# utiasSTARS/pyslam

Hardware: AMD Instinct MI355X
Metric: ms/LM-iter (Jac build + J^T J + Schur solve), stereo BA @ 500k residuals (lower is better)
Workload: dtype f64

## Files before the change

### include/pyslam_hip.h

```cpp
#ifndef PYSLAM_HIP_H
#define PYSLAM_HIP_H

#include <stdint.h>

#ifdef __cplusplus
extern "C" {
#endif

typedef struct ps_problem ps_problem;

typedef struct ps_problem_desc {
    int32_t dof;
    int32_t num_poses;
    const double*  poses;
    const int32_t* pose_rid;
    int32_t num_points;
    const double*  points;
    const int32_t* point_vid;

    int64_t num_obs;
    const int32_t* obs_pose;
    const int32_t* obs_point;
    const double*  obs_uvd;
    const int32_t* obs_grp;
// ... 81 lines not shown
int ps_step_norm2(ps_problem* h, double* norm2);

int ps_apply_update(ps_problem* h, double step);

int ps_snapshot_params(ps_problem* h);
int ps_restore_params(ps_problem* h);

int ps_get_params(ps_problem* h, double* poses, double* points);
int ps_set_params(ps_problem* h, const double* poses, const double* points);

int ps_gn_iteration(ps_problem* h, double lambda, double pcg_tol, int pcg_max_iters,
                    int linesearch, double* cost_out, double* dx_norm_out,
                    int* pcg_iters_out, double* pcg_relres_out);

typedef struct ps_solve_options {
    int32_t max_iters, allow_nondecreasing_steps, max_nondecreasing_steps, linesearch;
    double min_update_norm, min_cost, min_cost_decrease, lm_lambda;
} ps_solve_options;
int ps_motion_only_solve(ps_problem* h, const ps_solve_options* options, double* cost_history, int32_t cap,
                         int32_t* n_history, int32_t* iterations, double* last_dx_norm, double* pose12_out);

int ps_reset_solver_state(ps_problem* h);

const char* ps_build_sha(void);

int ps_solve(ps_problem* h, const ps_solve_options* options, double pcg_tol, int pcg_max_iters, double* cost_history,
             int32_t cap, int32_t* n_history, int32_t* iterations, double* last_dx_norm, int32_t* pcg_iters,
             double* pcg_relres, double* iter_ms);

int ps_lm_iteration(ps_problem* h, double lambda, double pcg_tol, int pcg_max_iters, int linesearch, double* cost_out,
                    double* dx_norm_out, double* model_decrease_out, int* pcg_iters_out, double* pcg_relres_out);

typedef struct ps_lm_options {
    int32_t max_iters, allow_nondecreasing_steps, max_nondecreasing_steps, linesearch;
    double min_update_norm, min_cost, min_cost_decrease, lm_lambda;
    double lambda0, lambda_min, lambda_max;
} ps_lm_options;
int ps_solve_lm(ps_problem* h, const ps_lm_options* options, double pcg_tol, int pcg_max_iters, double* cost_history,
                int32_t cap, int32_t* n_history, int32_t* iterations, double* last_dx_norm, int32_t* pcg_iters,
                double* pcg_relres, double* iter_ms, double* lm_rows);

int ps_gn_finish(ps_problem* h, int linesearch, double* cost_out, double* dx_pose_norm2,
                 double* dx_point_norm2);

int ps_gn_solve_finish(ps_problem* h, double pcg_tol, int pcg_max_iters, int linesearch, double* cost_out,
                       double* dx_pose_norm2, double* dx_point_norm2, int* pcg_iters_out,
                       double* pcg_relres_out);

int ps_shard_buffer(ps_problem* h, void** dev_ptr);

int ps_set_collective(ps_problem* h, void* nccl_all_reduce_fn, void* nccl_comm);
int ps_set_segment_exchange(ps_problem* h, void* nccl_all_gather_fn, int32_t world, int32_t rank, int64_t maxlen,
                            int64_t n_mine, const int64_t* mine, int64_t n_dst, const int64_t* dst, const int64_t* src_ptr,
                            const int64_t* src_off);
int ps_gn_solve_finish_enqueue(ps_problem* h, double pcg_tol, int pcg_max_iters, int linesearch, int first);
int ps_gn_result(ps_problem* h, int* done, double* shard2, double* dx_pose_norm2,
                 int* pcg_iters_out, double* pcg_relres_out);

int ps_covariance_begin(ps_problem* h);
int ps_covariance_column(ps_problem* h, int kind, int index, int comp, double tol, int max_iters,
                         int* iters_out, double* relres_out);

#define PS_COV_DENSE_MAX_UNKNOWNS 12288
int ps_covariance_marginals(ps_problem* h, double* pose_blocks ,
                            double* point_blocks );
int ps_covariance_pose_blocks(ps_problem* h, int64_t n, const int32_t* a, const int32_t* b,
                              double* out );
int ps_covariance_cross_blocks(ps_problem* h, int64_t n, const int32_t* kind_a, const int32_t* a,
                               const int32_t* kind_b, const int32_t* b, double* out );

int ps_triangulate(ps_problem* h, int64_t n, const int32_t* vids , int refine_iters, double min_parallax_deg,
                   int write_back, double* points_out , int32_t* status_out );

int ps_get_reduced_system(ps_problem* h, int32_t* row_ptr, int32_t* col_idx,
                          double* vals, double* g);
int ps_get_landmark_factors(ps_problem* h, double* cinv , double* c );
int ps_debug_reproj_blocks(ps_problem* h, double* r , double* jpose ,
                           double* jpoint );
int ps_debug_factor_blocks(ps_problem* h, double* r, double* j1, double* j2);
int ps_debug_table_checksums(ps_problem* h, uint64_t* out, int capacity, int* count);
int ps_debug_packed_runs(ps_problem* h, int32_t* nwaves, int32_t capacity_waves, int32_t* run, int32_t* first, int32_t* lm_ptr,
                         double* sq_part);
int ps_debug_pose_items(ps_problem* h, int32_t* nitems, int32_t capacity_items, int32_t* items, double* partial);

int ps_set_option(ps_problem* h, const char* name, double value);
int ps_get_option(ps_problem* h, const char* name, double* value);

int ps_set_profiling(ps_problem* h, int enabled);
int ps_get_stage_times(ps_problem* h, double* ms , int64_t* counts, int reset);

int ps_dense_normal_solve(const double* J, const double* r, int32_t m, int32_t n,
                          double* dx, double* covariance );

int ps_sparse_normal_solve(int32_t m, int32_t n, const int32_t* j_row_ptr, const int32_t* j_col, const double* j_val,
                           const int32_t* jt_row_ptr, const int32_t* jt_col, const double* jt_val,
                           const double* r, const double* rhs, double tol, int32_t max_iters,
                           double* dx, int32_t* iters_out, double* relres_out);

int ps_sparse_normal_direct(int32_t m, int32_t n, const int32_t* j_row_ptr, const int32_t* j_col, const double* j_val,
                            const int32_t* jt_row_ptr, const int32_t* jt_col, const double* jt_val,
                            const double* r, const double* rhs, int32_t refine_steps, double* dx, double* relres_out);

int ps_debug_band_inverse(const double* a, int32_t ncb, int32_t dof, int32_t bw, int32_t chunk_nodes, float* ainv_out,
                          double* elapsed_us);
int ps_debug_coarse_chol(const double* a, int32_t ncb, int32_t dof, int32_t bw, int32_t variant, double* Li, double* LiT,
                         int32_t* status, double* elapsed_us);
int ps_debug_coarse_chol_clocks(const double* a, int32_t ncb, int32_t dof, int32_t bw, int32_t variant, double* clocks);
int ps_debug_dense_factor(const double* a, int32_t n, int32_t flags, double* l_out, double* tinv_out, double* li_out, double* lit_out,
                          float* ainv_out, int32_t* diag_fail, double* elapsed_us);
int ps_debug_bchol_slab(int32_t m, int32_t w, int32_t block, int32_t* row_lo, int32_t* row_hi, int32_t* entries, int32_t* grid);
enum { PS_LDI_READ_STATE = 0, PS_LDI_READ_S32 = 1, PS_LDI_READ_X32 = 2, PS_LDI_READ_XU = 3, PS_LDI_READ_XT = 4, PS_LDI_READ_LINV = 5,
       PS_LDI_READ_COEF = 6, PS_LDI_READ_FRO = 7, PS_LDI_READ_R = 8, PS_LDI_READ_Z = 9 };
int ps_debug_ldi_gemm(int32_t M, int32_t N, int32_t K, float alpha, const float* A, int32_t lda, const float* B, int32_t ldb, float beta,
                      const float* Dm, int32_t ldd, float gamma, float* C, int32_t ldc, const int32_t* krange, int32_t upper_only,
                      const float* dev_scale, double fro_sentinel, double* fro_part);
int ps_debug_ldi_ritz(const double* rz, const double* alpha, int32_t m, float* out3);
int ps_debug_ldi_read(ps_problem* h, int32_t what, double* out, int64_t capacity);
int ps_debug_factor_stress(const double* a, int32_t ncb, int32_t dof, int32_t bw, int32_t mode, int32_t launches, int32_t lowprio,
                           int32_t aggressor, int32_t* n_diff, int32_t* n_pivot);

int ps_ransac_transforms(const double* pts_1, const double* pts_2, int32_t batch, int32_t n, double* T_out);
int ps_ransac_cost(const double* T, int32_t num_hyp, const double* pts_1, const double* obs_2, int32_t num_pts,
                   const double* cam5, double thresh, uint8_t* masks, int32_t* counts);
int ps_ransac_frame_to_frame(const double* pts_1, const double* pts_2, const double* obs_2, int32_t num_pts,
                             const int32_t* sample_idx, int32_t num_hyp, int32_t set_size, const double* cam5,
                             double thresh, double* T_all, int32_t* counts, int32_t* best_index,
                             int32_t* best_count, double* T_best, uint8_t* best_mask);

int ps_twoview_hypotheses(const double* obs_1, const double* obs_2, int32_t num_pts, const int32_t* sample_idx, int32_t num_hyp,
                          const double* cam5, double thresh, double* E_all, int32_t* counts, uint8_t* degenerate);
int ps_twoview_score(const double* E, int32_t num_hyp, const double* obs_1, const double* obs_2, int32_t num_pts,
                     const double* cam5, double thresh, uint8_t* masks, int32_t* counts);
int ps_twoview_ransac(const double* obs_1, const double* obs_2, int32_t num_pts, const int32_t* sample_idx, int32_t num_hyp,
                      const double* cam5, double thresh, int32_t refit, double* T_21, double* E_out, uint8_t* mask,
                      int32_t* info, double* parallax_deg);

int ps_pnp_hypotheses(const double* pts_w, const double* obs, int32_t num_pts, const int32_t* sample_idx, int32_t num_hyp,
                      const double* cam5, double thresh, double* T_all, int32_t* counts, uint8_t* empty);
int ps_pnp_score(const double* T, int32_t num_T, const double* pts_w, const double* obs, int32_t num_pts, const double* cam5,
                 double thresh, uint8_t* masks, int32_t* counts);
int ps_pnp_ransac(const double* pts_w, const double* obs, int32_t num_pts, const int32_t* sample_idx, int32_t num_hyp,
                  const double* cam5, double thresh, int32_t refine_iters, double* T_cw, uint8_t* mask, int32_t* info,
                  double* sq_err, double* cost_history);

int ps_sim3_hypotheses(const double* pts_1, const double* pts_2, const double* obs_1, const double* obs_2, int32_t num_pts,
                       const int32_t* sample_idx, int32_t num_hyp, const double* cam5, double thresh, int32_t fixed_scale,
                       double* S_all, double* scales, int32_t* counts, uint8_t* flags);
int ps_sim3_score(const double* S, int32_t num_S, const double* pts_1, const double* pts_2, const double* obs_1, const double* obs_2,
                  int32_t num_pts, const double* cam5, double thresh, uint8_t* masks, int32_t* counts);
int ps_sim3_ransac(const double* pts_1, const double* pts_2, const double* obs_1, const double* obs_2, int32_t num_pts,
                   const int32_t* sample_idx, int32_t num_hyp, const double* cam5, double thresh, int32_t fixed_scale,
                   int32_t refit_iters, double* S_21, double* scale, uint8_t* mask, int32_t* info, double* sq_err);

typedef struct ps_sim3pg ps_sim3pg;
int ps_sim3pg_create(int32_t num_vertices, const double* vertices13, const uint8_t* held, int32_t num_edges, const int32_t* edge_i,
                     const int32_t* edge_j, const double* edge_obs13, const double* edge_stiffness49, int32_t loss_id, double loss_k,
                     void* stream, ps_sim3pg** out);
int ps_sim3pg_destroy(ps_sim3pg* h);
int ps_sim3pg_set_vertices(ps_sim3pg* h, const double* vertices13);
int ps_sim3pg_get_vertices(ps_sim3pg* h, double* vertices13);
int ps_sim3pg_eval_cost(ps_sim3pg* h, double* cost);
int ps_sim3pg_linearize(ps_sim3pg* h, double lambda, double* H_out, double* g_out, double* cost);
int ps_sim3pg_iteration(ps_sim3pg* h, double lambda, double* cost_after, double* dx_norm, double* relres);
int ps_sim3pg_solve(ps_sim3pg* h, const ps_solve_options* options, double* cost_history, int32_t cap, int32_t* n_history,
                    int32_t* iterations, double* last_dx_norm);
int ps_sim3pg_debug_edges(ps_sim3pg* h, double* tap105);
// ... 81 lines not shown
```

### pyslam_amd/_native.py

```python
import ctypes as C
import os

import numpy as np

_HERE = os.path.dirname(os.path.abspath(__file__))
LIB_PATH = os.path.join(_HERE, 'lib', 'libpyslam_hip.so')
if os.environ.get('PYSLAM_AMD_MEASURE') == '1':
    LIB_PATH = os.path.join(_HERE, 'lib', 'libpyslam_hip_measure.so')

c_i32p = C.POINTER(C.c_int32)
c_f64p = C.POINTER(C.c_double)
c_u8p = C.POINTER(C.c_uint8)
PS_NUM_STAGES = 12
STAGE_NAMES = ['landmark_pass', 'pose_pass', 'schur_pairs', 'pose_factors', 'pcg',
               'backsub', 'update', 'cost', 'iteration_total', 'cg_kernel', 'allreduce', 'pack_unpack']


class ProblemDesc(C.Structure):
    _fields_ = [
        ('dof', C.c_int32), ('num_poses', C.c_int32), ('poses', c_f64p), ('pose_rid', c_i32p),
        ('num_points', C.c_int32), ('points', c_f64p), ('point_vid', c_i32p),
        ('num_obs', C.c_int64), ('obs_pose', c_i32p), ('obs_point', c_i32p), ('obs_uvd', c_f64p),
        ('obs_grp', c_i32p),
        ('num_cams', C.c_int32), ('cams', c_f64p), ('num_stiff3', C.c_int32), ('stiff3', c_f64p),
# ... 30 lines not shown
        ('num_obs', C.c_int64), ('num_edges', C.c_int64), ('num_priors', C.c_int64),
        ('reduced_nnzb', C.c_int64), ('num_pairs', C.c_int64), ('reduce_count', C.c_int64),
        ('device_bytes', C.c_int64), ('cg_restarts', C.c_int64), ('cg_kernel_launches', C.c_int64),
        ('ldi_solves', C.c_int64), ('ldi_fallbacks', C.c_int64), ('ldi_seeds', C.c_int64),
        ('xcg_fused_solves', C.c_int64), ('xcg_fused_fallbacks', C.c_int64),
        ('cg_persist_solves', C.c_int64), ('cg_persist_failures', C.c_int64), ('cg_persist_refused', C.c_int64),
        ('persist_cus', C.c_int32), ('persist_cus_needed', C.c_int32), ('landmark_passes_taken_over', C.c_int64),
    ]


class PhotoDesc(C.Structure):
    _fields_ = [
        ('num_pixels', C.c_int32), ('pt_ref', c_f64p), ('im_ref', c_f64p), ('im_jac', c_f64p), ('tri_jac_d', c_f64p),
        ('height', C.c_int32), ('width', C.c_int32), ('im_track', c_f64p),
        ('cam', C.c_double * 5), ('cam_type', C.c_int32), ('cam_w', C.c_int32), ('cam_h', C.c_int32),
        ('intensity_covar', C.c_double), ('depth_covar', C.c_double), ('loss_id', C.c_int32), ('loss_k', C.c_double),
    ]


class FeatParams(C.Structure):
    _fields_ = [('response_threshold', C.c_int64), ('nms_n', C.c_int32), ('max_features', C.c_int32),
                ('match_radius_u', C.c_int32), ('match_radius_v', C.c_int32), ('disp_max', C.c_int32),
                ('match_cost_max', C.c_int32), ('refinement', C.c_int32), ('reserved', C.c_int32)]


H = C.c_void_p
SIGNATURES = {
    'ps_last_error': (C.c_char_p, []),
    'ps_device_count': (C.c_int, []),
    'ps_warm_up': (C.c_int, []),
    'ps_problem_create': (C.c_int, [C.POINTER(ProblemDesc), C.c_void_p, C.POINTER(H)]),
    'ps_problem_create_hybrid': (C.c_int, [C.POINTER(ProblemDesc), C.POINTER(HostRowsDesc), C.c_void_p, C.POINTER(H)]),
    'ps_set_host_rows': (C.c_int, [H, c_f64p, C.c_int64, C.c_double]),
    'ps_problem_destroy': (C.c_int, [H]),
    'ps_get_info': (C.c_int, [H, C.POINTER(ProblemInfo)]),
    'ps_eval_cost': (C.c_int, [H, C.c_int, c_f64p]),
    'ps_linearize': (C.c_int, [H, C.c_double]),
    'ps_reduce_buffer': (C.c_int, [H, C.POINTER(C.c_void_p), C.POINTER(C.c_int64)]),
    'ps_shard_pack': (C.c_int, [H]),
    'ps_shard_unpack': (C.c_int, [H]),
    'ps_solve_reduced': (C.c_int, [H, C.c_double, C.c_int, C.POINTER(C.c_int), c_f64p]),
    'ps_backsub': (C.c_int, [H]),
    'ps_get_dx': (C.c_int, [H, c_f64p, c_f64p]),
    'ps_step_norm2': (C.c_int, [H, c_f64p]),
    'ps_apply_update': (C.c_int, [H, C.c_double]),
    'ps_snapshot_params': (C.c_int, [H]),
    'ps_restore_params': (C.c_int, [H]),
    'ps_reset_solver_state': (C.c_int, [H]),
    'ps_build_sha': (C.c_char_p, []),
    'ps_get_params': (C.c_int, [H, c_f64p, c_f64p]),
    'ps_set_params': (C.c_int, [H, c_f64p, c_f64p]),
    'ps_motion_only_solve': (C.c_int, [H, C.POINTER(SolveOptions), c_f64p, C.c_int32, C.POINTER(C.c_int32), C.POINTER(C.c_int32),
                                       C.POINTER(C.c_double), c_f64p]),
    'ps_solve': (C.c_int, [H, C.POINTER(SolveOptions), C.c_double, C.c_int, c_f64p, C.c_int32, C.POINTER(C.c_int32),
                           C.POINTER(C.c_int32), C.POINTER(C.c_double), c_i32p, c_f64p, c_f64p]),
    'ps_gn_iteration': (C.c_int, [H, C.c_double, C.c_double, C.c_int, C.c_int, c_f64p, c_f64p,
                                  C.POINTER(C.c_int), c_f64p]),
    'ps_lm_iteration': (C.c_int, [H, C.c_double, C.c_double, C.c_int, C.c_int, c_f64p, c_f64p, c_f64p,
                                  C.POINTER(C.c_int), c_f64p]),
    'ps_solve_lm': (C.c_int, [H, C.POINTER(LmOptions), C.c_double, C.c_int, c_f64p, C.c_int32, C.POINTER(C.c_int32),
                              C.POINTER(C.c_int32), C.POINTER(C.c_double), c_i32p, c_f64p, c_f64p, c_f64p]),
    'ps_gn_finish': (C.c_int, [H, C.c_int, c_f64p, c_f64p, c_f64p]),
    'ps_gn_solve_finish': (C.c_int, [H, C.c_double, C.c_int, C.c_int, c_f64p, c_f64p, c_f64p,
                                     C.POINTER(C.c_int), c_f64p]),
    'ps_set_collective': (C.c_int, [H, C.c_void_p, C.c_void_p]),
    'ps_set_segment_exchange': (C.c_int, [H, C.c_void_p, C.c_int32, C.c_int32, C.c_int64, C.c_int64, C.POINTER(C.c_int64), C.c_int64,
                                         C.POINTER(C.c_int64), C.POINTER(C.c_int64), C.POINTER(C.c_int64)]),
    'ps_shard_buffer': (C.c_int, [H, C.POINTER(C.c_void_p)]),
    'ps_gn_solve_finish_enqueue': (C.c_int, [H, C.c_double, C.c_int, C.c_int, C.c_int]),
    'ps_gn_result': (C.c_int, [H, C.POINTER(C.c_int), c_f64p, c_f64p, C.POINTER(C.c_int), c_f64p]),
    'ps_covariance_begin': (C.c_int, [H]),
    'ps_covariance_column': (C.c_int, [H, C.c_int, C.c_int, C.c_int, C.c_double, C.c_int, C.POINTER(C.c_int), c_f64p]),
    'ps_covariance_marginals': (C.c_int, [H, c_f64p, c_f64p]),
    'ps_covariance_pose_blocks': (C.c_int, [H, C.c_int64, c_i32p, c_i32p, c_f64p]),
    'ps_covariance_cross_blocks': (C.c_int, [H, C.c_int64, c_i32p, c_i32p, c_i32p, c_i32p, c_f64p]),
    'ps_triangulate': (C.c_int, [H, C.c_int64, c_i32p, C.c_int, C.c_double, C.c_int, c_f64p, c_i32p]),
    'ps_get_reduced_system': (C.c_int, [H, c_i32p, c_i32p, c_f64p, c_f64p]),
    'ps_get_landmark_factors': (C.c_int, [H, c_f64p, c_f64p]),
    'ps_debug_reproj_blocks': (C.c_int, [H, c_f64p, c_f64p, c_f64p]),
    'ps_debug_factor_blocks': (C.c_int, [H, c_f64p, c_f64p, c_f64p]),
    'ps_debug_table_checksums': (C.c_int, [H, C.POINTER(C.c_uint64), C.c_int, C.POINTER(C.c_int)]),
    'ps_debug_packed_runs': (C.c_int, [H, c_i32p, C.c_int32, c_i32p, c_i32p, c_i32p, c_f64p]),
    'ps_debug_pose_items': (C.c_int, [H, c_i32p, C.c_int32, c_i32p, c_f64p]),
    'ps_set_option': (C.c_int, [H, C.c_char_p, C.c_double]),
    'ps_get_option': (C.c_int, [H, C.c_char_p, c_f64p]),
    'ps_set_profiling': (C.c_int, [H, C.c_int]),
    'ps_get_stage_times': (C.c_int, [H, c_f64p, C.POINTER(C.c_int64), C.c_int]),
    'ps_ransac_transforms': (C.c_int, [c_f64p, c_f64p, C.c_int32, C.c_int32, c_f64p]),
    'ps_ransac_cost': (C.c_int, [c_f64p, C.c_int32, c_f64p, c_f64p, C.c_int32, c_f64p, C.c_double, c_u8p, c_i32p]),
    'ps_ransac_frame_to_frame': (C.c_int, [c_f64p, c_f64p, c_f64p, C.c_int32, c_i32p, C.c_int32, C.c_int32, c_f64p,
                                           C.c_double, c_f64p, c_i32p, c_i32p, c_i32p, c_f64p, c_u8p]),
    'ps_twoview_hypotheses': (C.c_int, [c_f64p, c_f64p, C.c_int32, c_i32p, C.c_int32, c_f64p, C.c_double, c_f64p, c_i32p, c_u8p]),
    'ps_twoview_score': (C.c_int, [c_f64p, C.c_int32, c_f64p, c_f64p, C.c_int32, c_f64p, C.c_double, c_u8p, c_i32p]),
    'ps_twoview_ransac': (C.c_int, [c_f64p, c_f64p, C.c_int32, c_i32p, C.c_int32, c_f64p, C.c_double, C.c_int32, c_f64p, c_f64p,
                                    c_u8p, c_i32p, c_f64p]),
    'ps_pnp_hypotheses': (C.c_int, [c_f64p, c_f64p, C.c_int32, c_i32p, C.c_int32, c_f64p, C.c_double, c_f64p, c_i32p, c_u8p]),
    'ps_pnp_score': (C.c_int, [c_f64p, C.c_int32, c_f64p, c_f64p, C.c_int32, c_f64p, C.c_double, c_u8p, c_i32p]),
    'ps_pnp_ransac': (C.c_int, [c_f64p, c_f64p, C.c_int32, c_i32p, C.c_int32, c_f64p, C.c_double, C.c_int32, c_f64p, c_u8p, c_i32p,
                                c_f64p, c_f64p]),
    'ps_sim3_hypotheses': (C.c_int, [c_f64p, c_f64p, c_f64p, c_f64p, C.c_int32, c_i32p, C.c_int32, c_f64p, C.c_double, C.c_int32,
                                     c_f64p, c_f64p, c_i32p, c_u8p]),
    'ps_sim3_score': (C.c_int, [c_f64p, C.c_int32, c_f64p, c_f64p, c_f64p, c_f64p, C.c_int32, c_f64p, C.c_double, c_u8p, c_i32p]),
    'ps_sim3_ransac': (C.c_int, [c_f64p, c_f64p, c_f64p, c_f64p, C.c_int32, c_i32p, C.c_int32, c_f64p, C.c_double, C.c_int32, C.c_int32,
                                 c_f64p, c_f64p, c_u8p, c_i32p, c_f64p]),
    'ps_sim3pg_create': (C.c_int, [C.c_int32, c_f64p, c_u8p, C.c_int32, c_i32p, c_i32p, c_f64p, c_f64p, C.c_int32, C.c_double, C.c_void_p,
                                   C.POINTER(H)]),
    'ps_sim3pg_destroy': (C.c_int, [H]),
    'ps_sim3pg_set_vertices': (C.c_int, [H, c_f64p]),
    'ps_sim3pg_get_vertices': (C.c_int, [H, c_f64p]),
    'ps_sim3pg_eval_cost': (C.c_int, [H, c_f64p]),
    'ps_sim3pg_linearize': (C.c_int, [H, C.c_double, c_f64p, c_f64p, c_f64p]),
    'ps_sim3pg_iteration': (C.c_int, [H, C.c_double, c_f64p, c_f64p, c_f64p]),
    'ps_sim3pg_solve': (C.c_int, [H, C.POINTER(SolveOptions), c_f64p, C.c_int32, C.POINTER(C.c_int32), C.POINTER(C.c_int32),
                                  C.POINTER(C.c_double)]),
    'ps_sim3pg_debug_edges': (C.c_int, [H, c_f64p]),
    'ps_sim3pg_debug_explog': (C.c_int, [C.c_int32, c_f64p, c_f64p, c_f64p, c_f64p]),
    'ps_sim3pg_profile': (C.c_int, [H, C.c_int32, c_f64p]),
    'ps_photometric_create': (C.c_int, [C.POINTER(PhotoDesc), C.c_void_p, C.POINTER(H)]),
    'ps_photometric_destroy': (C.c_int, [H]),
    'ps_photometric_set_pose': (C.c_int, [H, c_f64p]),
    'ps_photometric_get_pose': (C.c_int, [H, c_f64p]),
    'ps_photometric_eval_cost': (C.c_int, [H, c_f64p, C.POINTER(C.c_int64)]),
    'ps_photometric_normal_equations': (C.c_int, [H, c_f64p, c_f64p, c_f64p, C.POINTER(C.c_int64)]),
    'ps_photometric_iteration': (C.c_int, [H, C.c_int32, C.c_int32, c_f64p, c_f64p]),
    'ps_dense_create': (C.c_int, [C.c_int32, C.c_int32, C.c_int32, C.c_int32, C.c_void_p, C.POINTER(H)]),
    'ps_dense_destroy': (C.c_int, [H]),
    'ps_dense_upload': (C.c_int, [H, C.c_int32, C.c_int32, C.c_int32, C.c_int32, C.c_void_p, c_f64p]),
    'ps_dense_make_tables': (C.c_int, [H, C.c_int32, C.c_int32, c_i32p, c_f64p, C.c_double, C.c_double, C.c_double]),
    'ps_dense_track': (C.c_int, [H, C.c_int32, C.c_int32, C.c_int32, c_i32p, c_i32p, C.POINTER(SolveOptions), C.c_int32,
                                 C.c_double, c_f64p, c_f64p, c_i32p, c_f64p, C.c_int32]),
    'ps_dense_level_shape': (C.c_int, [H, C.c_int32, c_i32p, c_i32p]),
    'ps_dense_read_level': (C.c_int, [H, C.c_int32, C.c_int32, C.c_int32, c_f64p]),
    'ps_dense_num_pixels': (C.c_int, [H, C.c_int32, C.c_int32, c_i32p]),
    'ps_dense_read_tables': (C.c_int, [H, C.c_int32, C.c_int32, C.c_int32, c_f64p, c_f64p, c_f64p, c_f64p]),
    'ps_dense_device_bytes': (C.c_int, [H, C.POINTER(C.c_int64)]),
    'ps_feat_create': (C.c_int, [C.c_int32, C.c_int32, C.c_int32, C.c_void_p, C.POINTER(H)]),
    'ps_feat_destroy': (C.c_int, [H]),
    'ps_feat_push': (C.c_int, [H, C.c_int32, C.c_int32, c_u8p, c_u8p]),
    'ps_feat_match': (C.c_int, [H, C.c_int32, C.POINTER(FeatParams), c_i32p]),
    'ps_feat_read_matches': (C.c_int, [H, C.c_int32, c_f64p, c_i32p]),
    'ps_feat_read_features': (C.c_int, [H, C.c_int32, C.c_int32, c_i32p, c_i32p, C.POINTER(C.c_int64), c_u8p]),
    'ps_feat_set_map': (C.c_int, [H, C.c_int32, c_f64p, c_u8p]),
    'ps_feat_match_map': (C.c_int, [H, c_f64p, c_f64p, C.c_int32, C.POINTER(FeatParams), c_i32p]),
    'ps_feat_read_map_matches': (C.c_int, [H, C.c_int32, c_i32p, c_i32p, c_i32p, c_f64p]),
    'ps_feat_match_map_global': (C.c_int, [H, C.c_int32, C.c_int32, C.POINTER(FeatParams), c_i32p]),
    'ps_feat_read_map_second': (C.c_int, [H, C.c_int32, c_i32p]),
    'ps_feat_db_add': (C.c_int, [H, C.c_int32, c_u8p, c_i32p]),
    'ps_feat_db_clear': (C.c_int, [H]),
    'ps_feat_db_size': (C.c_int, [H, c_i32p, C.POINTER(C.c_int64)]),
    'ps_feat_db_query': (C.c_int, [H, C.c_int32, C.c_int32, C.c_int32, C.c_int32, C.POINTER(FeatParams), c_i32p]),
    'ps_feat_feature_passes': (C.c_int, [H, C.POINTER(C.c_int64)]),
    'ps_feat_device_bytes': (C.c_int, [H, C.POINTER(C.c_int64)]),
    'ps_dense_normal_solve': (C.c_int, [c_f64p, c_f64p, C.c_int32, C.c_int32, c_f64p, c_f64p]),
    'ps_sparse_normal_solve': (C.c_int, [C.c_int32, C.c_int32, c_i32p, c_i32p, c_f64p, c_i32p, c_i32p, c_f64p, c_f64p, c_f64p,
                                         C.c_double, C.c_int32, c_f64p, c_i32p, c_f64p]),
    'ps_sparse_normal_direct': (C.c_int, [C.c_int32, C.c_int32, c_i32p, c_i32p, c_f64p, c_i32p, c_i32p, c_f64p, c_f64p, c_f64p,
                                          C.c_int32, c_f64p, c_f64p]),
    'ps_debug_band_inverse': (C.c_int, [c_f64p, C.c_int32, C.c_int32, C.c_int32, C.c_int32, C.POINTER(C.c_float), c_f64p]),
    'ps_debug_coarse_chol': (C.c_int, [c_f64p, C.c_int32, C.c_int32, C.c_int32, C.c_int32, c_f64p, c_f64p, c_i32p, c_f64p]),
    'ps_debug_coarse_chol_clocks': (C.c_int, [c_f64p, C.c_int32, C.c_int32, C.c_int32, C.c_int32, c_f64p]),
    'ps_debug_dense_factor': (C.c_int, [c_f64p, C.c_int32, C.c_int32, c_f64p, c_f64p, c_f64p, c_f64p, C.POINTER(C.c_float), c_i32p, c_f64p]),
    'ps_debug_bchol_slab': (C.c_int, [C.c_int32, C.c_int32, C.c_int32, c_i32p, c_i32p, c_i32p, c_i32p]),
    'ps_debug_ldi_gemm': (C.c_int, [C.c_int32, C.c_int32, C.c_int32, C.c_float, C.POINTER(C.c_float), C.c_int32, C.POINTER(C.c_float), C.c_int32,
                                    C.c_float, C.POINTER(C.c_float), C.c_int32, C.c_float, C.POINTER(C.c_float), C.c_int32, c_i32p, C.c_int32,
                                    C.POINTER(C.c_float), C.c_double, c_f64p]),
    'ps_debug_ldi_ritz': (C.c_int, [c_f64p, c_f64p, C.c_int32, C.POINTER(C.c_float)]),
# ... 100 lines not shown
```

### pyslam_amd/csrc/ps_abi_solver.h

```cpp

int ps_get_info(ps_problem* h, ps_problem_info* info) {
    if (!h || !info) return fail("null argument");
    info->dof = h->D; info->num_poses = h->P; info->num_reduced = h->nr; info->num_points = h->L;
    info->num_var_points = h->nv; info->num_obs = h->N; info->num_edges = h->F; info->num_priors = 0;
    info->reduced_nnzb = h->nnzb; info->num_pairs = h->npairs;
    info->reduce_count = ((long)h->nnzb + h->nr) / 2 * h->D * h->D + (long)h->nr * h->D + 3;
    info->device_bytes = (int64_t)h->dev_bytes;
    info->cg_restarts = h->cg_fallbacks;
    info->cg_kernel_launches = h->cg_kernel_launches;
    info->ldi_solves = h->ldi_solves; info->ldi_fallbacks = h->ldi_fallbacks; info->ldi_seeds = h->ldi_seeds;
    info->xcg_fused_solves = h->xf_solves; info->xcg_fused_fallbacks = h->xf_fallbacks;
    info->cg_persist_solves = h->cp_launches; info->cg_persist_failures = h->cp_failures;
    info->cg_persist_refused = h->cp_refused; info->persist_cus = h->persist_cus;
    info->persist_cus_needed = h->cp_ok ? h->cp_cus_needed : (h->xp_ok ? h->xp_cus_needed : 0);
    info->landmark_passes_taken_over = h->prelm_used;
    return 0;
}

int ps_eval_cost(ps_problem* h, int include_all_constant, double* cost) {
    if (!h || !cost) return fail("null argument");
    if (include_all_constant && h->fuse_cost == 1 && lm_cost_possible(h)) { if (lm_cost_pass(h, h->lin_lambda, SC_COST)) return -1; }
    else if (cost_pass(h, include_all_constant, SC_COST)) return -1;
    if (read_scalars(h)) return -1;
    *cost = h->h_scalars[SC_COST];
// ... 751 lines not shown
    hipMemcpyAsync(jpoint, djl, (size_t)h->N * 9 * sizeof(double), hipMemcpyDeviceToHost, h->stream);
    const int rc = sync(h);
    hipFree(dr); hipFree(djp); hipFree(djl);
    return rc;
}

int ps_debug_factor_blocks(ps_problem* h, double* r, double* j1, double* j2) {
    if (!h || !r || !j1 || !j2) return fail("null argument");
    if (h->F == 0) return 0;
    const int D = h->D, DD = D * D, ROW = D + 2 * DD;
    double* dbg;
    HIP_OK(hipMalloc((void**)&dbg, (size_t)h->F * ROW * sizeof(double)));
    const int rc0 = D == 6 ? launch_factor_pass<6>(h, 0.0, dbg) : launch_factor_pass<3>(h, 0.0, dbg);
    std::vector<double> t((size_t)h->F * ROW);
    hipMemcpyAsync(t.data(), dbg, t.size() * sizeof(double), hipMemcpyDeviceToHost, h->stream);
    const int rc = sync(h);
    hipFree(dbg);
    if (rc0 || rc) return -1;
    for (long f = 0; f < h->F; ++f) {
        std::memcpy(r + f * D, &t[(size_t)f * ROW], D * sizeof(double));
        std::memcpy(j1 + f * DD, &t[(size_t)f * ROW + D], DD * sizeof(double));
        std::memcpy(j2 + f * DD, &t[(size_t)f * ROW + D + DD], DD * sizeof(double));
    }
    return 0;
}

int ps_debug_table_checksums(ps_problem* h, uint64_t* out, int capacity, int* count) {
    if (!h || !out || !count) return fail("null argument");
    if (sync(h)) return -1;
    struct Tab { const void* p; size_t bytes; };
    const bool tiled = h->schur_tiles > 1 && h->npair_items > 0;
    const Tab tabs[16] = {
        {h->point_vid, (size_t)h->L * 4}, {h->lobs, (size_t)h->N * sizeof(LObs)}, {h->lorig, (size_t)h->N * 4},
        {h->lm_ptr, ((size_t)h->nv + 1) * 4}, {h->lm_point, (size_t)h->nv * 4}, {h->pose_of_rid, (size_t)std::max(h->nr, 1) * 4},
        {h->pitems, (size_t)h->npitems * sizeof(PItem)}, {h->pitem_ptr, ((size_t)h->nr + 1) * 4}, {h->pobs, (size_t)h->Np * sizeof(LObs)},
        {h->pairs, (size_t)h->npairs * 8}, {h->pair_xitems, (size_t)8 * h->pair_per_xcd * sizeof(PairItem)},
        {tiled ? h->comb_items : nullptr, (size_t)h->ncomb * sizeof(PairItem)}, {tiled ? h->comb_tasks : nullptr, (size_t)h->npair_items * 4},
        {h->row_ptr, ((size_t)h->nr + 1) * 4}, {h->col_idx, (size_t)h->nnzb * 4}, {h->diag_slot, (size_t)h->nr * 4}};
    *count = 16;
    std::vector<unsigned char> buf;
    for (int t = 0; t < 16 && t < capacity; ++t) {
        uint64_t hsh = 0;
        if (tabs[t].p && tabs[t].bytes) {
            buf.resize(tabs[t].bytes);
            HIP_OK(hipMemcpy(buf.data(), tabs[t].p, tabs[t].bytes, hipMemcpyDeviceToHost));
            hsh = 1469598103934665603ull;
            size_t i = 0;
            for (; i + 8 <= buf.size(); i += 8) { uint64_t w; std::memcpy(&w, &buf[i], 8); hsh = (hsh ^ w) * 1099511628211ull; }
            for (; i < buf.size(); ++i) hsh = (hsh ^ buf[i]) * 1099511628211ull;
        }
        out[t] = hsh;
    }
    return 0;
}

int ps_debug_packed_runs(ps_problem* h, int32_t* nwaves, int32_t capacity_waves, int32_t* run, int32_t* first, int32_t* lm_ptr, double* sq_part) {
    if (!h || !nwaves) return fail("null argument");
    if (sync(h)) return -1;
    const int nw = h->lmw_nwaves;
    *nwaves = nw;
    if ((run || first || sq_part) && capacity_waves < nw) return fail("ps_debug_packed_runs: capacity too small");
    if (sq_part && nw) HIP_OK(hipMemcpy(sq_part, h->sq_part_l, (size_t)cdiv(nw, 4) * 8, hipMemcpyDeviceToHost));
    if (run && nw) HIP_OK(hipMemcpy(run, h->lmw_run, (size_t)nw * sizeof(LmwRun), hipMemcpyDeviceToHost));
    if (first && nw) HIP_OK(hipMemcpy(first, h->lmw_first, ((size_t)nw + 1) * 4, hipMemcpyDeviceToHost));
    if (lm_ptr && h->nv > 0) HIP_OK(hipMemcpy(lm_ptr, h->lm_ptr, ((size_t)h->nv + 1) * 4, hipMemcpyDeviceToHost));
    return 0;
}

int ps_debug_pose_items(ps_problem* h, int32_t* nitems, int32_t capacity_items, int32_t* items, double* partial) {
    if (!h || !nitems) return fail("null argument");
    if (sync(h)) return -1;
    const int ni = h->npitems;
    *nitems = ni;
    if ((items || partial) && capacity_items < ni) return fail("ps_debug_pose_items: capacity too small");
    if (items && ni) {
        std::vector<PItem> tab(ni);
        HIP_OK(hipMemcpy(tab.data(), h->pitems, (size_t)ni * sizeof(PItem), hipMemcpyDeviceToHost));
        for (int k = 0; k < ni; ++k) { items[3 * k] = tab[k].rid; items[3 * k + 1] = tab[k].start; items[3 * k + 2] = tab[k].end; }
    }
    if (partial && ni) HIP_OK(hipMemcpy(partial, h->ppartial, (size_t)ni * PS_NPOSE_ACC * sizeof(double), hipMemcpyDeviceToHost));
    return 0;
}

int ps_debug_ldi_read(ps_problem* h, int32_t what, double* out, int64_t capacity) {
    if (!h || !out) return fail("null argument");
    if (what == PS_LDI_READ_STATE) {
        if (capacity < 12) return fail("ps_debug_ldi_read: state record needs 12 doubles");
        const double rec[12] = {(double)h->ldi_state, (double)h->ldi_cur, (double)h->ldi_n, (double)h->ldi_np, (double)h->ldi_kp,
                                h->ldi_direct ? 1.0 : 0.0, h->ldi_fro_limit, (double)h->ldi_last_its, (double)h->ldi_seed_steps,
                                (double)h->nr, (double)h->D, h->ldi_ready ? 1.0 : 0.0};
        std::memcpy(out, rec, sizeof(rec));
        return 0;
    }
    if (!h->ldi_ready || h->ldi_seeds < 1) return fail("ps_debug_ldi_read: the lagged inverse has never been set up on this handle");
    HIP_OK(hipStreamSynchronize(h->stream));
    if (h->side) HIP_OK(hipStreamSynchronize(h->side));
    if (h->ldi_stream) HIP_OK(hipStreamSynchronize(h->ldi_stream));
    if (h->ev_ldi) HIP_OK(hipEventSynchronize(h->ev_ldi));
    const size_t n = (size_t)h->ldi_n, np = (size_t)h->ldi_np, kp = (size_t)h->ldi_kp;
    const void* src = nullptr; size_t count = 0; bool f32 = true;
    const bool seed_item = what == PS_LDI_READ_S32 || what == PS_LDI_READ_X32 || what == PS_LDI_READ_XT || what == PS_LDI_READ_LINV ||
                           what == PS_LDI_READ_COEF;
    if (seed_item && h->ldi_direct) return fail("ps_debug_ldi_read: the direct seed keeps no Newton-Schulz operands");
    const bool use_item = what == PS_LDI_READ_XU || what == PS_LDI_READ_R || what == PS_LDI_READ_Z;
    if (use_item && h->ldi_cur < 0) return fail("ps_debug_ldi_read: no inverse is in use");
    switch (what) {
        case PS_LDI_READ_S32: src = h->ldi_S32; count = np * np; break;
        case PS_LDI_READ_X32: src = h->ldi_X32; count = np * np; break;
        case PS_LDI_READ_XU: src = h->ldi_Xu[h->ldi_cur]; count = np * np; break;
        case PS_LDI_READ_XT: src = h->ldi_Xt; count = np * kp; break;
        case PS_LDI_READ_LINV: src = h->ldi_Linv; count = (size_t)h->nr * h->D * h->D; f32 = false; break;
        case PS_LDI_READ_COEF: src = h->ldi_coef; count = 3; break;
        case PS_LDI_READ_FRO: if (capacity < 1) return fail("ps_debug_ldi_read: capacity"); out[0] = *h->h_ldi_fro; return 0;
        case PS_LDI_READ_R: src = h->ldi_r[h->ldi_last_its & 1]; count = n; f32 = false; break;
        case PS_LDI_READ_Z: src = h->z; count = n; f32 = false; break;
        default: return fail("ps_debug_ldi_read: unknown item");
    }
    if ((size_t)capacity < count) return fail("ps_debug_ldi_read: capacity too small");
    if (!f32) { HIP_OK(hipMemcpy(out, src, count * 8, hipMemcpyDeviceToHost)); return 0; }
    std::vector<float> tmp(count);
    HIP_OK(hipMemcpy(tmp.data(), src, count * 4, hipMemcpyDeviceToHost));
    for (size_t i = 0; i < count; ++i) out[i] = (double)tmp[i];
    return 0;
}

static void relook_path(ps_problem* h) {
    const bool possible = ps_ldi_possible(*h, (long)h->nr * h->D);
    if (h->coarse_built && possible != h->xmin_auto_ldi && h->cg_explicit_min_rows < 0) h->coarse_built = false;
}

int ps_set_option(ps_problem* h, const char* name, double value) {
    if (!h || !name) return fail("null argument");
    if (!std::strcmp(name, "expect_next")) { h->expect_next = value != 0 && !h->hybrid; return 0; }
    if (!std::strcmp(name, "solve_horizon")) { h->solve_horizon = value < 0 ? -1 : (int)std::min(value, 1e6); return 0; }
    if (!std::strcmp(name, "setup_ride")) {
        h->setup_ride = value != 0 ? 1 : 0;
        h->prelin_valid = h->prelm_valid = false;
        relook_launch_gates(h);
        return 0;
    }
    if (!std::strcmp(name, "rows_regs")) {
        h->rows_regs = value != 0 ? 1 : 0;
        h->prelin_valid = h->prelm_valid = h->ride_valid = false;
        return 0;
    }
    if (!std::strcmp(name, "cg_persist_recover")) {
        h->cg_persist_recover = value != 0 ? 1 : 0;
        h->prelin_valid = h->prelm_valid = h->ride_valid = false;
        return 0;
    }
    if (!std::strcmp(name, "cg_persist_recover_lds")) {
        if (!(value >= 0 && value <= PS_CP_RECOVER_LDS_CAP)) return fail("cg_persist_recover_lds out of range (0 .. 146432 bytes)");
        h->cg_persist_recover_lds = (int)value;
        h->prelin_valid = h->prelm_valid = h->ride_valid = false;
        return 0;
    }
    if (!std::strcmp(name, "packed_prefetch")) {
        h->packed_prefetch = value != 0 ? 1 : 0;
        h->prelin_valid = h->prelm_valid = h->ride_valid = false;
        return 0;
    }
    if (!std::strcmp(name, "pose_prefetch")) {
        h->pose_prefetch = value != 0 ? 1 : 0;
        h->prelin_valid = h->prelm_valid = h->ride_valid = false;
        return 0;
    }
    if (!std::strcmp(name, "coarse_chol_band")) { h->coarse_chol_band = value != 0 ? 1 : 0; return 0; }
    if (std::strcmp(name, "cg_force_breakdown")) h->prelin_valid = h->prelm_valid = h->ride_valid = false;
    const char* refusal = nullptr;
    const int fx = ps_option_apply(*h, name, value, &refusal);
    if (fx == PS_OPT_UNKNOWN) return fail(std::string("unknown option: ") + name);
    if (fx == PS_OPT_REFUSED) return fail(refusal);
    if (fx & PS_FX_COARSE_REBUILD) h->coarse_built = false;
    if (fx & PS_FX_DROP_FACTOR) h->lci_next = -1;
    if (fx & PS_FX_DROP_SIDE) h->side_todo = false;
    if ((fx & PS_FX_LDI_OFF) && !h->ldi_enable) { h->ldi_cur = -1; if (h->ldi_state != 1) h->ldi_state = 0; }
    if (fx & PS_FX_RELOOK_PATH) relook_path(h);
    relook_launch_gates(h);
    return 0;
}

int ps_get_option(ps_problem* h, const char* name, double* value) {
    if (!h || !name || !value) return fail("null argument");
    const std::string n(name);
    if (n == "lin_zero_list") *value = h->lin_zero_gate ? 1.0 : 0.0;
    else if (n == "lin_fills") *value = (double)h->lin_fills;
    else if (n == "lin_zero_launches") *value = (double)h->lin_zero_launches;
    else if (n == "setup_ride") *value = h->ride_gate ? 1.0 : 0.0;
    else if (n == "factor_launches") *value = (double)h->bjf_launches;
    else if (n == "factors_ridden") *value = (double)h->bjf_ridden;
    else if (n == "factor_plan_mismatches") *value = (double)h->bjf_mismatches;
    else if (n == "rows_regs") *value = (double)h->rows_regs;
    else if (n == "rows_setups") *value = (double)h->rows_setups;
    else if (n == "exact_row_setups") *value = (double)h->exact_row_setups;
    else if (n == "rows_lci_in_lds") *value = h->coarse_built && h->lagx_ok && h->rows_lci_lds ? 1.0 : 0.0;
    else if (n == "packed_prefetch") *value = (double)h->packed_prefetch;
    else if (n == "pose_prefetch") *value = (double)h->pose_prefetch;
    else if (n == "cg_persist_recover") *value = (double)h->cg_persist_recover;
    else if (n == "cg_persist_recover_lds") *value = (double)h->cg_persist_recover_lds;
    else if (n == "cg_persist_recover_need") *value = h->coarse_built && h->cp_ok ? (double)h->cp_rec_lds : 0.0;
    else if (n == "cg_persist_recovered") *value = (double)h->cp_rec_inside;
    else if (n == "cg_persist_recover_fallbacks") *value = (double)h->cp_rec_behind;
    else if (n == "coarse_chol_band") *value = (double)h->coarse_chol_band;
    else if (n == "coarse_nodes") *value = h->coarse_built ? (double)h->ncb : 0.0;
    else if (n == "coarse_chol_bw") *value = h->coarse_built && h->ncb > 0 ? (double)std::min(std::max(h->coarse_chol_bw, 0), h->ncb - 1) : -1.0;
    else if (n == "cg_force_breakdown") *value = (double)h->cg_force_breakdown;
    else return fail("ps_get_option: no read-back for option: " + n);
    return 0;
}

int ps_reset_solver_state(ps_problem* h) {
    if (!h) return fail("null argument");
    h->prelin_valid = h->prelm_valid = h->ride_valid = false;
    if (!h->solver_touched) {
        static_cast<PsCostHistory&>(*h) = PsCostHistory{};
        return 0;
    }
    h->solver_touched = false;
    HIP_OK(hipStreamSynchronize(h->stream));
    if (h->side) HIP_OK(hipStreamSynchronize(h->side));
    if (h->ldi_stream) HIP_OK(hipStreamSynchronize(h->ldi_stream));
    drain_timers(h);
    static_cast<PsCarried&>(*h) = PsCarried{};
    static_cast<PsCostHistory&>(*h) = PsCostHistory{};
    if (h->lag_status) HIP_OK(hipMemsetAsync(h->lag_status, 0, ST_NWORDS * sizeof(int32_t), h->stream));
    if (h->ldi_ready && !(h->ldi_direct_ok && h->N == 0 && h->F > 0)) h->ldi_direct = false;
    h->cov_ready = false;
    return 0;
}

#ifndef PS_BUILD_SHA
#define PS_BUILD_SHA "unknown"
#endif
const char* ps_build_sha(void) { return PS_BUILD_SHA; }

int ps_set_profiling(ps_problem* h, int enabled) {
    if (!h) return fail("null argument");
    h->profiling = enabled < 0 ? 0 : (enabled > 2 ? 2 : enabled);
    return 0;
}

int ps_get_stage_times(ps_problem* h, double* ms, int64_t* counts, int reset) {
    if (!h) return fail("null argument");
    if (!h->pending.empty() && sync(h)) return -1;
    for (int i = 0; i < PS_NUM_STAGES; ++i) {
        if (ms) ms[i] = h->stage_ms[i];
        if (counts) counts[i] = h->stage_n[i];
        if (reset) { h->stage_ms[i] = 0.0; h->stage_n[i] = 0; }
    }
    return 0;
}

int ps_dense_normal_solve(const double* J, const double* r, int32_t m, int32_t n, double* dx, double* covariance) {
    if (!J || !r || !dx || m <= 0 || n <= 0) return fail("bad argument");
    if (n > 2048) return fail("generic (host-evaluated) path supports at most 2048 unknowns");
    if (need_device()) return -1;
    const int nrhs = covariance ? n + 1 : 1;
    DevBuf bJ, br, bH, bB, bst, bg;
    if (bJ.put(J, (size_t)m * n) || br.put(r, (size_t)m) || bH.get((size_t)n * n * sizeof(double)) ||
        bst.get(ST_NWORDS * sizeof(int32_t)) || bg.get((size_t)n * sizeof(double))) return -1;
    HIP_OK(hipMemset(bst.p, 0, ST_NWORDS * sizeof(int32_t)));
    hipLaunchKernelGGL(k_dense_normal, dim3(cdiv((long)n * n, 256)), dim3(256), 0, 0, m, n, bJ.as<double>(), br.as<double>(), bH.as<double>(),
                       bg.as<double>());
    std::vector<double> B((size_t)n * nrhs, 0.0), gh(n);
    if (bg.fetch(gh.data(), gh.size())) return -1;
    for (int i = 0; i < n; ++i) { B[(size_t)i * nrhs] = gh[i]; if (covariance) B[(size_t)i * nrhs + 1 + i] = 1.0; }
    if (bB.put(B.data(), B.size())) return -1;
    hipLaunchKernelGGL(k_dense_chol_solve, dim3(1), dim3(256), 0, 0, n, nrhs, bH.as<double>(), bB.as<double>(), bst.as<int32_t>());
    int32_t st[ST_NWORDS];
    if (bB.fetch(B.data(), B.size()) || bst.fetch(st, (size_t)ST_NWORDS)) return -1;
    if (st[ST_DIAG_FAIL]) return fail("normal matrix is not positive definite");
    for (int i = 0; i < n; ++i) {
        dx[i] = B[(size_t)i * nrhs];
        if (covariance) for (int j = 0; j < n; ++j) covariance[(size_t)i * n + j] = B[(size_t)i * nrhs + 1 + j];
    }
    return 0;
}
```

### pyslam_amd/csrc/ps_core.hip

```cpp
#include <hip/hip_runtime.h>

#include <algorithm>
#include <array>
#include <map>
#include <atomic>
#include <chrono>
#include <thread>
#include <climits>
#include <cmath>
#include <cstdio>
#include <cstring>
#include <memory>
#include <mutex>
#include <string>
#include <vector>

#include "pyslam_hip.h"
#include "ps_kernels.h"
#include "ps_ransac_core.h"
#include "ps_ransac.h"
#include "ps_k_twoview.h"
#include "ps_k_pnp.h"
#include "ps_k_sim3.h"
#include "ps_k_sim3pg.h"
// ... 287 lines not shown
    int cg_persist_recover = 1;
    int cg_persist_recover_lds = PS_CP_RECOVER_LDS_CAP;
    int cp_rec_pp = 0, cp_rec_cols = 0;
    size_t cp_rec_lds = 0;
    long cp_rec_inside = 0, cp_rec_behind = 0;
    int persist_dev = 0, persist_cus = 0;
    bool persist_masked = false;
    int cp_cus_needed = 0, xp_cus_needed = 0;
    int persist_held = 0;
    bool params_moved_since_lin = false;
    bool z_foreign = false;
    bool no_repeat = false;
    long cp_refused = 0;
    void persist_release() { if (persist_held) { ps_persist_ledger().release(persist_dev, persist_held); persist_held = 0; } }
    int persist_capacity() const { return persist_masked ? persist_cus / 2 : persist_cus; }
    bool persist_reserve(int need) {
        if (need <= 0 || persist_cus <= 0) return false;
        if (persist_held) return true;
        if (!ps_persist_ledger().reserve(persist_dev, need, persist_capacity())) { ++cp_refused; return false; }
        persist_held = need; return true;
    }
    bool xp_ok = false;
    int32_t* xf_cnt = nullptr;
    unsigned long long* xp_exch = nullptr;
    size_t xp_words = 0;
    unsigned xp_salt = 0;
    bool xp_defer = false;
    long long* cp_dbg = nullptr;
    long long* xp_dbg = nullptr;
    long prof_tick = 0;
    int cg_fallbacks = 0;
    bool cg_two_level_reduce = false, cg_short_rows = false;
    double* cg_tot = nullptr;
    bool cg_split = false;
    bool xmin_auto_ldi = false;
    double *cg_U = nullptr, *cg_cgd[2] = {}, *cg_ab = nullptr;
    int cg_launched = 0;
    long cg_kernel_launches = 0;
    bool cov_ready = false;
    std::vector<int32_t> h_slot_of_vid;
    double* cov_buf = nullptr;
    double* cov_xbuf = nullptr;
    long long cov_epoch = 0, cov_sigma_epoch = -1;
    double* tri_buf = nullptr;
    size_t tri_cap = 0;
    int ell_wf = 0, ell_wc = 0;
    double *cost_partials = nullptr, *scalars = nullptr, *h_scalars = nullptr;
    int32_t *status = nullptr, *h_status = nullptr;
    double* h_scalars_dev = nullptr;
    int32_t* h_status_dev = nullptr;
    double *h_shard = nullptr, *h_shard_dev = nullptr;
    long long *h_seq = nullptr, *h_seq_dev = nullptr;
    long long seq = 0;
    long long *h_setup = nullptr, *h_setup_dev = nullptr;
    long long setup_seq = 0;
    int32_t* arrivals = nullptr;
    double *h_mo_hist = nullptr, *h_mo_hist_dev = nullptr;
    int ncost_obs = 0, ncost_fac = 0;
    typedef int (*allreduce_fn)(const void*, void*, size_t, int, int, void*, hipStream_t);
    allreduce_fn nccl_allreduce = nullptr;
    void* nccl_comm = nullptr;
    typedef int (*allgather_fn)(const void*, void*, size_t, int, void*, hipStream_t);
    allgather_fn seg_allgather = nullptr;
    int seg_world = 0;
    long seg_maxlen = 0, seg_nmine = 0, seg_ndst = 0;
    int32_t *seg_mine = nullptr, *seg_dst = nullptr, *seg_src_off = nullptr, *seg_src_ptr = nullptr;
    double *seg_in = nullptr, *seg_all = nullptr;
    double* shard_pack = nullptr;
    int32_t *up_slot = nullptr, *upT_slot = nullptr;
    long nup = 0, pack_count = 0;
    double* shard_buf = nullptr;
    bool shard_out = false;
    double *sq_part_l = nullptr, *sq_part_p = nullptr;
    bool lm_md = false;
    double *md_part_p = nullptr, *md_part_l = nullptr;
    int nmd_p = 0;
    int nsq_l = 0 , nsq_l16 = 0 , nsq_p = 0;
    int32_t* lmw_first = nullptr;
    int lmw_nwaves = 0;
    LmwRun* lmw_run = nullptr;
    int packed_prefetch = 1;
    int pose_prefetch = 1;
    int pose_chunk = 256;
    int coarse_chol_band = 1;
    int coarse_chol_bw = 0;
    bool ldi_ready = false;
    int ldi_n = 0, ldi_np = 0, ldi_kp = 0;
    float *ldi_S32 = nullptr, *ldi_X32 = nullptr, *ldi_R32 = nullptr, *ldi_T32 = nullptr, *ldi_Xt = nullptr, *ldi_XtT = nullptr;
    float* ldi_Xu[2] = {};
    double *ldi_x64 = nullptr, *ldi_Linv = nullptr, *ldi_r[2] = {}, *ldi_part = nullptr, *ldi_fro_part = nullptr;
    double *h_ldi_fro = nullptr, *h_ldi_fro_dev = nullptr;
    double ldi_fro_limit = 0.1;
    int2* ldi_krange = nullptr;
    bool side_poolable = false;
    hipStream_t ldi_stream = nullptr;
    double *ldi_A64 = nullptr, *ldi_Li = nullptr, *ldi_LiT = nullptr, *ldi_Tinv = nullptr; int32_t* ldi_stat = nullptr;
    float* ldi_coef = nullptr;
    long ldi_solves = 0, ldi_fallbacks = 0, ldi_seeds = 0;
    hipEvent_t ev_ldi = nullptr, ev_ldi_sread = nullptr;
    bool snap_valid = false;
    long long *h_early = nullptr, *h_early_dev = nullptr;
    long long early_seq = 0;
    bool spec_next = false, spec_enqueued = false, early_armed = false, prelin_valid = false;
    double prelin_lambda = 0.0;
    bool prelm_pending = false, prelm_valid = false;
    double prelm_lambda = 0.0;
    long long prelm_tag = 0, prelm_seq = 0, lmfail_check = 0, lin_lmfail_tag = 0;
    long long *h_lmfail = nullptr, *h_lmfail_dev = nullptr;
    long prelm_used = 0;
    bool start_cost_pending = false;
    bool solver_touched = false;
    int profiling = 0;
    std::vector<std::pair<int, int>> pending;
    double stage_ms[PS_NUM_STAGES] = {};
    int64_t stage_n[PS_NUM_STAGES] = {};
    std::vector<hipEvent_t> ev_pool;
    size_t ev_used = 0;

    char *arena_dev = nullptr, *arena_host = nullptr;
    void* words_host = nullptr;
    size_t arena_used = 0;
    bool arena_open = false, arena_poisoned = false;

    template <typename T>
    int alloc(T** out, size_t n, bool device_written = false ) {
        *out = nullptr;
        const size_t bytes = std::max<size_t>(n, 1) * sizeof(T);
        if (arena_open && bytes <= PS_ARENA_SMALL && !device_written) {
            const size_t off = (arena_used + 255) & ~(size_t)255;
            if (off + bytes <= PS_ARENA_BYTES) {
                std::memset(arena_host + off, 0, bytes);
                arena_used = off + bytes;
                dev_bytes += bytes;
                *out = (T*)(arena_dev + off);
                return 0;
            }
        }
        void* p = nullptr;
        static const bool guard_on = ps_env("PS_ALLOC_GUARD") != nullptr;
        const size_t padded = (bytes + 255) & ~(size_t)255;
        if (slab_left >= padded) {
            *out = (T*)slab; slab += padded; slab_left -= padded; dev_bytes += bytes;
            return 0;
        }
        hipError_t e = hipMalloc(&p, guard_on ? padded + 4096 : bytes);
        if (e != hipSuccess) return fail(std::string("hipMalloc: ") + hipGetErrorString(e));
        if (guard_on) {
            if (hipMemset((char*)p + bytes, 0xA5, padded - bytes + 4096) != hipSuccess) return fail("hipMemset (guard) failed");
            guards.push_back({(char*)p + padded, bytes, (int)guards.size()});
            fprintf(stderr, "GUARD %p table #%d = %zu bytes (%s)\n", (void*)this, (int)guards.size() - 1, bytes, __PRETTY_FUNCTION__);
        }
        static const bool poison_all = ps_env("PS_ARENA_POISON") != nullptr;
        if (poison_all && hipMemset(p, 0xFF, bytes) != hipSuccess) return fail("hipMemset (poison) failed");
        allocs.push_back(p);
        dev_bytes += bytes;
        *out = (T*)p;
        return 0;
    }
    char* slab = nullptr; size_t slab_left = 0;
    int slab_reserve(size_t bytes) {
        if (ps_env("PS_ALLOC_GUARD")) return 0;
        void* p = nullptr;
        hipError_t e = hipMalloc(&p, bytes);
        if (e != hipSuccess) return fail(std::string("hipMalloc: ") + hipGetErrorString(e));
        if (ps_env("PS_ARENA_POISON") && hipMemset(p, 0xFF, bytes) != hipSuccess) return fail("hipMemset (poison) failed");
        allocs.push_back(p);
// ... 101 lines not shown
```

### pyslam_amd/csrc/ps_host_cg.h

```cpp

namespace {

struct StageTimer {
    ps_problem* h;
    int stage;
    hipEvent_t a = nullptr, b = nullptr;
    int slot = -1;
    StageTimer(ps_problem* h_, int st, int level = 2) : h(h_), stage(st) {
        if (h->profiling < level) return;
        if (h->profiling == 1 && h->prof_every > 1 &&
            h->prof_tick % h->prof_every != (st == PS_ST_CG_KERNEL ? h->prof_every / 2 : 0)) return;
        if (h->ev_used + 2 > h->ev_pool.size()) {
            for (int i = 0; i < 64; ++i) { hipEvent_t e; hipEventCreate(&e); h->ev_pool.push_back(e); }
        }
        slot = (int)h->ev_used;
        a = h->ev_pool[h->ev_used++];
        b = h->ev_pool[h->ev_used++];
        hipEventRecord(a, h->stream);
    }
    void stop() {
        if (!a) return;
        hipEventRecord(b, h->stream);
        h->pending.push_back({stage, slot});
        a = nullptr;
    }
    ~StageTimer() { stop(); }
};

void drain_timers(ps_problem* h) {
    for (auto& pr : h->pending) {
        float ms = 0.f;
        if (hipEventElapsedTime(&ms, h->ev_pool[pr.second], h->ev_pool[pr.second + 1]) == hipSuccess) {
            h->stage_ms[pr.first] += ms;
            h->stage_n[pr.first] += 1;
        }
    }
    h->pending.clear();
    h->ev_used = 0;
}

int side_kick(ps_problem* h);
int ldi_side_kick(ps_problem* h);
int linearize(ps_problem* h, double lambda, bool allow_prelm = false);
bool use_direct(const ps_problem* h);

void drain_timers_ready(ps_problem* h) {
    std::vector<std::pair<int, int>> keep;
    for (auto& pr : h->pending) {
        float ms = 0.f;
        if (hipEventQuery(h->ev_pool[pr.second + 1]) != hipSuccess) { keep.push_back(pr); continue; }
        if (hipEventElapsedTime(&ms, h->ev_pool[pr.second], h->ev_pool[pr.second + 1]) == hipSuccess) {
            h->stage_ms[pr.first] += ms;
            h->stage_n[pr.first] += 1;
        }
    }
    h->pending.swap(keep);
    if (h->pending.empty()) h->ev_used = 0;
}

int sync(ps_problem* h) {
    HIP_OK(hipStreamSynchronize(h->stream));
    h->persist_release();
    drain_timers(h);
    if (h->side_todo) h->side_ready = true;
    return 0;
}

int wait_published(ps_problem* h) {
    volatile long long* w = h->h_seq;
    struct WaitClock {
        ps_problem* h; std::chrono::steady_clock::time_point t0 = std::chrono::steady_clock::now();
        ~WaitClock() { h->host_wait_ns += std::chrono::duration<double, std::nano>(std::chrono::steady_clock::now() - t0).count(); ++h->host_waits; }
    } wc{h};
    static const int kick_mode = ps_env("PS_SIDE_KICK") ? atoi(ps_env("PS_SIDE_KICK")) : 2;
    volatile long long* ws = h->h_setup;
    for (long spins = 0; spins < 400000000L; ++spins) {
        if (kick_mode == 2 && h->side_todo && !h->side_ready && *ws == h->setup_seq) { h->side_ready = true; if (side_kick(h)) return -1; }
        if (h->ldi_side_todo && *ws == h->setup_seq) { if (ldi_side_kick(h)) return -1; }
        if (h->early_armed && *reinterpret_cast<volatile long long*>(h->h_early) == h->early_seq) {
            h->early_armed = false; h->spec_enqueued = true;
            if (h->prelm_pending) { h->prelm_pending = false; h->prelm_valid = true; }
            if (linearize(h, h->lin_lambda, true)) return -1;
        }
        if (*w == h->seq) {
            h->persist_release();
            if (h->lmfail_check && *reinterpret_cast<volatile long long*>(h->h_lmfail + (h->lmfail_check & 1)) == h->lmfail_check) h->h_status[ST_LM_FAIL] += 1;
            if (h->h_status[ST_PERSIST_FAIL] && (h->cg_persist || h->xcg_persist)) { h->cg_persist = 0; h->xcg_persist = 0; ++h->cp_failures; }
            if (h->start_cost_pending) {
                h->start_cost_pending = false;
                h->last_cost = h->ldi_call_start_cost = h->h_scalars[SC_STARTCOST];
            }
            if (h->side_todo) { h->side_ready = true; if (kick_mode >= 1 && side_kick(h)) return -1; }
            if (h->ldi_side_todo) { if (h->spec_enqueued) h->ldi_side_todo = false; else if (ldi_side_kick(h)) return -1; }
            h->early_armed = false;
            if (h->pending.empty()) return 0;
            if (h->spec_enqueued) { drain_timers_ready(h); return 0; }
            HIP_OK(hipEventSynchronize(h->ev_pool[h->pending.back().second + 1]));
            drain_timers(h);
            return 0;
        }
        __builtin_ia32_pause();
    }
    return sync(h);
}

int read_scalars(ps_problem* h) {
    HIP_OK(hipMemcpyAsync(h->h_scalars, h->scalars, SC_NWORDS * sizeof(double), hipMemcpyDeviceToHost, h->stream));
    HIP_OK(hipMemcpyAsync(h->h_status, h->status, ST_NWORDS * sizeof(int32_t), hipMemcpyDeviceToHost, h->stream));
    return sync(h);
}

template <int D>
int launch_factor_pass(ps_problem* h, double lambda, double* dbg = nullptr) {
    if (h->F == 0 && h->FH == 0) return 0;
    if (h->F > 0)
        hipLaunchKernelGGL(k_factor_pass<D>, dim3(cdiv(h->F, PS_FP_FACTORS)), dim3(256), 0, h->stream, (int)h->F, h->f_i,
                           h->f_j, h->f_Tinv, h->f_grp, h->fgroups, h->poses, h->fscratch, dbg);
    if (dbg) return 0;
    const long threads = (long)h->nes * D * D + (long)h->nr * D;
    hipLaunchKernelGGL(k_factor_assemble<D>, dim3(cdiv(threads, 256)), dim3(256), 0, h->stream, h->nes,
                       h->eslots, h->eptr, h->eitems, h->eslot_diag, h->nr, h->gptr, h->gitems,
                       h->fscratch, lambda, h->S, h->g);
    return 0;
}

template <int D>
int pcg_run(ps_problem* h, double tol, int max_iters, int* iters_out, double* relres_out) {
    const int nr = h->nr;
    if (max_iters + 2 > h->hist_cap) return fail("pcg max_iters exceeds the history buffer (4096)");
    hipLaunchKernelGGL(k_block_jacobi<D>, dim3(cdiv(nr, 256)), dim3(256), 0, h->stream, nr, h->diag_slot,
                       h->S, h->Minv, h->status);
    hipLaunchKernelGGL(k_pcg_init<D>, dim3(h->npartB), dim3(256), 0, h->stream, nr, h->g, h->Minv, h->x,
                       h->r, h->z, h->rz_part, h->rr_part, h->status);
    const double tol2 = tol * tol;
    int k = 0;
    int chunk = std::max(4, h->last_pcg_iters + 1);
    bool done = false;
    while (!done) {
        const int n = std::min(chunk, max_iters + 1 - k);
        h->cg_kernel_launches += 2L * n;
        for (int i = 0; i < n; ++i, ++k) {
            double* pold = (k & 1) ? h->p1 : h->p0;
            double* pnew = (k & 1) ? h->p0 : h->p1;
            hipLaunchKernelGGL(k_pcg_spmv<D>, dim3(h->npartA), dim3(256), 0, h->stream, nr, h->row_ptr,
                               h->col_idx, h->S, h->z, pold, pnew, h->q, h->rz_part, h->rr_part, h->npartB,
                               h->pq_part, h->hist, k, tol2, h->status, h->scalars);
            if (k < max_iters)
                hipLaunchKernelGGL(k_pcg_update<D>, dim3(h->npartB), dim3(256), 0, h->stream, nr, h->Minv,
                                   pnew, h->q, h->x, h->r, h->z, h->pq_part, h->npartA, h->hist, k,
                                   h->rz_part, h->rr_part, h->status);
        }
        HIP_OK(hipMemcpyAsync(h->h_status, h->status, ST_NWORDS * sizeof(int32_t), hipMemcpyDeviceToHost, h->stream));
        HIP_OK(hipMemcpyAsync(h->h_scalars, h->scalars, SC_NWORDS * sizeof(double), hipMemcpyDeviceToHost, h->stream));
        HIP_OK(hipStreamSynchronize(h->stream));
        done = h->h_status[ST_PCG_DONE] != 0 || k > max_iters;
        chunk = 8;
    }
    h->last_pcg_iters = h->h_status[ST_PCG_ITERS];
    if (iters_out) *iters_out = h->h_status[ST_PCG_ITERS];
    const double rr0 = h->h_scalars[SC_RR0], rrf = h->h_scalars[SC_RRFINAL];
    if (relres_out) *relres_out = rr0 > 0.0 ? std::sqrt(rrf / rr0) : 0.0;
// ... 705 lines not shown
        if (cg_fused_setup<D>(h, max_iters, false, rhs)) return -1;
        int chunk = std::max(h->pcg_chunk, h->last_pcg_iters + 2);
        bool done = false;
        while (!done) {
            const int m = std::min(chunk, max_iters + 2 - h->cg_launched);
            cg_fused_launch<D>(h, tol_pass, m);
            HIP_OK(hipMemcpyAsync(h->h_status, h->status, ST_NWORDS * sizeof(int32_t), hipMemcpyDeviceToHost, h->stream));
            HIP_OK(hipMemcpyAsync(h->h_scalars, h->scalars, SC_NWORDS * sizeof(double), hipMemcpyDeviceToHost, h->stream));
            HIP_OK(hipStreamSynchronize(h->stream));
            h->persist_release();
            if (h->h_status[ST_PERSIST_FAIL] && h->cg_persist) { h->cg_persist = 0; ++h->cp_failures; }
            done = h->h_status[ST_PCG_DONE] != 0 || h->cg_launched >= max_iters + 2;
            chunk = h->pcg_chunk;
        }
        total_its += h->h_status[ST_PCG_ITERS];
        const bool pretend = forced && h->h_status[ST_PCG_DONE] == 1 && tol_pass > tol;
        if ((h->h_status[ST_PCG_DONE] != 2 && !pretend) || h->h_status[ST_DIAG_FAIL] || h->h_status[ST_LM_FAIL]) break;
        const double rr0 = h->h_scalars[SC_RR0], rrf = h->h_scalars[SC_RRFINAL];
        const double rho = rr0 > 0.0 ? std::sqrt(rrf / rr0) : 1.0;
        ++h->cg_fallbacks;
        if (restarts == 3 || !(rho < 0.5)) {
            if (restarts) copy_doubles(h->stream, h->g, gsaved, (size_t)nvec);
            return pcg_run<D>(h, tol, max_iters, iters_out, relres_out);
        }
        cg_fused_recover<D>(h, nullptr);
        if (restarts == 0) copy_doubles(h->stream, gsaved, h->g, (size_t)nvec);
        hipLaunchKernelGGL(k_vec_accumulate, dim3(cdiv(nvec, 256)), dim3(256), 0, h->stream, nvec, (const double*)h->x, xacc, restarts == 0);
        hipLaunchKernelGGL(k_bsr_residual<D>, dim3(cdiv(nvec, 256)), dim3(256), 0, h->stream, h->nr, h->row_ptr, h->col_idx, h->S,
                           (const double*)xacc, (const double*)gsaved, h->g);
        reduced *= rho;
        rhs = true;
        ++restarts;
    }
    cg_fused_recover<D>(h, nullptr);
    if (restarts) {
        hipLaunchKernelGGL(k_vec_accumulate, dim3(cdiv(nvec, 256)), dim3(256), 0, h->stream, nvec, (const double*)xacc, h->x, 0);
        copy_doubles(h->stream, h->g, gsaved, (size_t)nvec);
    }
    int its = 0; double rel = 0.0;
    const int rc = cg_report(h, &its, &rel);
    if (iters_out) *iters_out = total_its;
    if (relres_out) *relres_out = rel * reduced;
    h->last_pcg_iters = total_its;
    return rc;
}

int linearize(ps_problem* h, double lambda, bool allow_prelm) {
    h->solver_touched = true;
    h->prelin_valid = false;
    const bool lm_done = allow_prelm && h->prelm_valid && h->prelm_lambda == lambda && h->nv > 0;
    h->prelm_valid = false;
    h->lin_lmfail_tag = lm_done ? h->prelm_tag : 0;
    if (lm_done) ++h->prelm_used;
    h->lin_lambda = lambda;
    h->params_moved_since_lin = false; h->z_foreign = false;
    ++h->prof_tick;
    h->cov_ready = false;
    cov_release(h);
    h->status_clean = false;
    if (h->ldi_sread_pending) {
        HIP_OK(hipStreamWaitEvent(h->stream, h->ev_ldi_sread, 0));
        h->ldi_sread_pending = false;
    }
    const bool zero_by_list = h->lin_zero_gate;
    const bool lm_here = h->nv > 0 && !lm_done;
    BjFactorOut ride{};
    h->ride_valid = false;
    if (h->ride_gate && h->nr > 0 && h->pcg_variant == 1 && !use_direct(h)) {
        if (!h->coarse_built && build_coarse(h)) return -1;
        if (h->cg_explicit) h->ride_gate = false;
        else {
            const int lci = (h->side_todo && h->side_ready) ? h->side_buf : h->lci_next;
            const CgSetupPlan plan = cg_setup_plan(h, allow_prelm, lci);
            const CgSetupPlan lag = cg_setup_plan(h, true, lci);
            const bool held = plan.basis_out && ((lag.lagged && plan.basis_out == h->Bmat2[lag.use]) ||
                                                 (h->side_todo && plan.basis_out == h->Bmat2[h->side_buf]));
            if (!held) {
                ride = BjFactorOut{h->Linv, h->status, h->cg_r[0], h->cg_w[0], h->cg_s[0], h->cg_p, h->cg_xh, h->poses, h->pose_of_rid,
                                   h->coarse_basis, plan.basis_out, h->bgv};
                h->ride_lagged = plan.lagged; h->ride_use = plan.use; h->ride_basis = plan.basis_out;
            }
        }
    }
    if (!zero_by_list) {
        HIP_OK(hipMemsetAsync(h->red, 0, h->red_count * sizeof(double) + ST_NWORDS * sizeof(int32_t), h->stream));
        ++h->lin_fills;
    } else {
        if (lm_here) HIP_OK(hipMemsetAsync(h->status, 0, ST_NWORDS * sizeof(int32_t), h->stream));
        ++h->lin_zero_launches;
    }
    if (lm_here) {
        StageTimer t(h, PS_ST_LANDMARK);
        const ObsWide wl{h->sidx_l, h->stiff_tab};
#define PS_LM_LAUNCH(W) hipLaunchKernelGGL(k_landmark_pass<W>, dim3(cdiv(h->nv, 256 / PS_LM_GROUP)), dim3(256), 0, h->stream, h->nv, h->lm_ptr, \
                           h->lm_point, h->lobs, h->poses, h->points, h->pose_rid, h->ogroups, lambda, h->Z,                       \
                           h->Cinv, h->cvec, h->status, h->lm_ablate, wl)
#define PS_LMP_LAUNCH(W, PF) hipLaunchKernelGGL((k_landmark_pass_packed<W, false, PF>), dim3(cdiv(h->lmw_nwaves, 4)), dim3(256), 0, h->stream, h->lmw_nwaves, \
                           h->lmw_first, h->lmw_run, h->lm_ptr, h->lm_point, h->lobs, h->poses, h->points, h->pose_rid, h->ogroups, lambda, h->Z,      \
                           h->Cinv, h->cvec, h->status, wl, (const int32_t*)nullptr, (double*)nullptr, (long long*)nullptr, 0LL)
        if (h->lm_packed && h->lmw_nwaves > 0 && !h->lm_ablate) {
            if (h->packed_prefetch) { if (h->wide_obs) PS_LMP_LAUNCH(true, true); else PS_LMP_LAUNCH(false, true); }
            else if (h->wide_obs) PS_LMP_LAUNCH(true, false); else PS_LMP_LAUNCH(false, false);
        }
        else if (h->wide_obs) PS_LM_LAUNCH(true); else PS_LM_LAUNCH(false);
#undef PS_LMP_LAUNCH
#undef PS_LM_LAUNCH
    }
    bool fin_in_combine = false, fin_in_pairs = false;
    static const bool schur_split_env = ps_env("PS_SCHUR_SPLIT") != nullptr;
    if (h->npitems > 0) {
        StageTimer t(h, PS_ST_POSE);
        const ObsWide wp{h->sidx_p, h->stiff_tab};
        const int per_xcd = h->pose_xcd ? cdiv(h->npitems, 8) : 0;
        const int nblk = per_xcd ? 8 * per_xcd : h->npitems;
        static_assert(ST_NWORDS % 2 == 0, "the status words are cleared as doubles");
        const int ntail = zero_by_list ? h->nr * 6 + 2 + (lm_here ? 0 : ST_NWORDS / 2) : 0;
        const int nzs = zero_by_list ? h->nzero_slots : 0;
        const int nzblk = zero_by_list ? cdiv((long)nzs * 36 + ntail, 256) : 0;
#define PS_PPF_LAUNCH(W, D) hipLaunchKernelGGL((k_pose_pass_pf<W, D>), dim3(nblk + nzblk), dim3(256), 0, h->stream, h->pitems, h->pobs,       \
                               h->poses, h->points, h->ogroups, h->Cinv, h->cvec, h->ppartial, wp, h->npitems, per_xcd,                  \
                               nblk, (const int32_t*)h->zero_slots, nzs, h->S, h->g, ntail)
        if (h->pose_prefetch && h->pose_chunk <= PS_POSE_PF_OBS) {
            if (h->wide_obs) { if (lambda != 0.0) PS_PPF_LAUNCH(true, true); else PS_PPF_LAUNCH(true, false); }
            else if (lambda != 0.0) PS_PPF_LAUNCH(false, true); else PS_PPF_LAUNCH(false, false);
        }
        else if (h->wide_obs)
            hipLaunchKernelGGL(k_pose_pass<true>, dim3(nblk + nzblk), dim3(256), 0, h->stream, h->pitems, h->pobs,
                               h->poses, h->points, h->ogroups, h->Cinv, h->cvec, h->ppartial, lambda != 0.0 ? 1 : 0, wp, h->npitems, per_xcd,
                               nblk, (const int32_t*)h->zero_slots, nzs, h->S, h->g, ntail);
        else
            hipLaunchKernelGGL(k_pose_pass<false>, dim3(nblk + nzblk), dim3(256), 0, h->stream, h->pitems, h->pobs,
                               h->poses, h->points, h->ogroups, h->Cinv, h->cvec, h->ppartial, lambda != 0.0 ? 1 : 0, wp, h->npitems, per_xcd,
                               nblk, (const int32_t*)h->zero_slots, nzs, h->S, h->g, ntail);
#undef PS_PPF_LAUNCH
        fin_in_combine = h->Spart && h->npair_items > 0 && !h->has_diag_tasks && h->D == 6;
        fin_in_pairs = !h->Spart && h->schur_pipeline && h->npair_items > 0 && !h->has_diag_tasks && h->D == 6 && !schur_split_env;
        if (!fin_in_combine && !fin_in_pairs)
            hipLaunchKernelGGL(k_pose_finalize, dim3(h->nr), dim3(64), 0, h->stream, h->nr, h->pitem_ptr,
                               h->ppartial, h->diag_slot, lambda, h->S, h->g);
    }
    if (h->npair_items > 0) {
        StageTimer t(h, PS_ST_SCHUR, 1);
        const bool split2 = schur_split_env;
        const int halfp = split2 ? (h->pair_per_xcd / 2 + 3) / 4 * 4 : h->pair_per_xcd;
        static const int lds_pad = ps_env("PS_SCHUR_LDS_PAD") ? atoi(ps_env("PS_SCHUR_LDS_PAD")) : 0;
        auto launch_pairs = [&](int nblk, int lds, int from, int to) {
            if (!h->schur_pipeline)
                hipLaunchKernelGGL(k_schur_pairs, dim3(nblk), dim3(256), lds, h->stream, h->pair_per_xcd, h->pair_xitems, h->pairs,
                                   h->Z, h->S, h->Spart, h->schur_ablate, from, to);
            else {
#ifdef PS_MEASURE
                auto k = h->schur_ablate == 0 ? k_schur_pairs_db<0> : h->schur_ablate == 1 ? k_schur_pairs_db<1> :
                         h->schur_ablate == 2 ? k_schur_pairs_db<2> : h->schur_ablate == 3 ? k_schur_pairs_db<3> :
                         h->schur_ablate == 4 ? k_schur_pairs_db<4> : k_schur_pairs_db<5>;
#else
                auto k = k_schur_pairs_db<0>;
#endif
                const int nfin = fin_in_pairs ? cdiv(h->nr, 4) : 0;
                const int lead = (fin_in_pairs && ride.Linv) ? (nfin + 7) / 8 * 8 : 0;
                hipLaunchKernelGGL(k, dim3(nblk + (lead ? lead : nfin)), dim3(256), lds, h->stream, h->pair_per_xcd,
                                   h->pair_xitems, h->pairs, h->Z, h->S, h->Spart, from, to, nblk, fin_in_pairs ? h->nr : 0,
                                   h->pitem_ptr, h->ppartial, h->diag_slot, lambda, h->g, fin_in_pairs ? ride : BjFactorOut{}, lead);
                if (fin_in_pairs && ride.Linv) { h->ride_valid = true; ++h->bjf_ridden; }
            }
        };
        launch_pairs(8 * (halfp / 4), lds_pad, 0, halfp);
        if (split2 && halfp < h->pair_per_xcd) launch_pairs(8 * ((h->pair_per_xcd - halfp + 3) / 4), 0, halfp, h->pair_per_xcd);
        if (h->Spart)
            hipLaunchKernelGGL(k_schur_combine, dim3(cdiv(h->ncomb, 4) + (fin_in_combine ? cdiv(h->nr, 4) : 0)), dim3(256), 0,
                               h->stream, h->ncomb, h->comb_items, h->comb_tasks, h->Spart, h->S,
                               fin_in_combine ? h->nr : 0, h->pitem_ptr, h->ppartial, h->diag_slot, lambda, h->g);
    }
    if ((h->F > 0 || h->FH > 0) && h->nr > 0) {
        StageTimer t(h, PS_ST_EDGES);
        if (h->D == 6) launch_factor_pass<6>(h, lambda); else launch_factor_pass<3>(h, lambda);
    }
    return side_kick(h);
}

inline bool cost_packed_possible(const ps_problem* h) {
    return h->fuse_cost != 0 && h->lm_packed && h->lmw_nwaves > 0 && !h->lm_ablate && h->Nl == h->N && h->nv > 0 && h->D == 6;
}
int cost_partials_pass(ps_problem* h, int include_all, const int32_t* gate) {
    int n = 0;
    if (h->N > 0 && include_all && cost_packed_possible(h)) {
        const ObsWide wl{h->sidx_l, h->stiff_tab};
        const int nbl = cdiv(h->lmw_nwaves, 4);
#define PS_CSP_LAUNCH(W, PF) hipLaunchKernelGGL((k_cost_packed<W, PF>), dim3(nbl), dim3(256), 0, h->stream, h->lmw_nwaves, h->lmw_first, h->lmw_run, \
                           h->lm_ptr, h->lm_point, h->lobs, h->poses, h->points, h->ogroups, h->cost_partials, gate, wl)
        if (h->packed_prefetch) { if (h->wide_obs) PS_CSP_LAUNCH(true, true); else PS_CSP_LAUNCH(false, true); }
        else if (h->wide_obs) PS_CSP_LAUNCH(true, false); else PS_CSP_LAUNCH(false, false);
#undef PS_CSP_LAUNCH
        n += nbl;
    } else if (h->N > 0) {
        const ObsWide wl{h->sidx_l, h->stiff_tab};
        if (h->wide_obs)
            hipLaunchKernelGGL(k_cost_reproj<true>, dim3(h->ncost_obs), dim3(256), 0, h->stream, h->N, h->lobs, h->poses,
                               h->points, h->pose_rid, h->point_vid, h->ogroups, include_all, h->cost_partials, gate, wl);
        else
            hipLaunchKernelGGL(k_cost_reproj<false>, dim3(h->ncost_obs), dim3(256), 0, h->stream, h->N, h->lobs, h->poses,
                               h->points, h->pose_rid, h->point_vid, h->ogroups, include_all, h->cost_partials, gate, wl);
        n += h->ncost_obs;
    }
    if (h->F > 0) {
        if (h->D == 6)
            hipLaunchKernelGGL(k_cost_factors<6>, dim3(h->ncost_fac), dim3(256), 0, h->stream, (int)h->F, h->f_i,
                               h->f_j, h->f_Tinv, h->f_grp, h->fgroups, h->poses, h->pose_rid, include_all,
                               h->cost_partials + n, gate);
        else
            hipLaunchKernelGGL(k_cost_factors<3>, dim3(h->ncost_fac), dim3(256), 0, h->stream, (int)h->F, h->f_i,
                               h->f_j, h->f_Tinv, h->f_grp, h->fgroups, h->poses, h->pose_rid, include_all,
                               h->cost_partials + n, gate);
        n += h->ncost_fac;
    }
    return n;
}
// ... 49 lines not shown
}

int lm_md_enqueue(ps_problem* h, const int32_t* gate) {
    const int32_t* pip = h->npitems > 0 ? h->pitem_ptr : nullptr;
#define PS_LMP_SUMS(DD) hipLaunchKernelGGL(k_lm_pose_sums<DD>, dim3(h->nmd_p), dim3(256), 0, h->stream, h->nr, h->x, h->g, pip, h->ppartial, h->nes,   \
                               h->eslots, h->eptr, h->eitems, h->eslot_diag, h->brow_of, h->fscratch, h->lin_lambda, gate, h->md_part_p)
    if (h->D == 6) PS_LMP_SUMS(6); else PS_LMP_SUMS(3);
#undef PS_LMP_SUMS
    hipLaunchKernelGGL(k_lm_total, dim3(1), dim3(256), 0, h->stream, h->nmd_p, h->md_part_p, h->nv > 0 ? nsq_l_now(h) : 0, h->md_part_l, gate,
                       h->scalars + SC_MODELDEC);
    return 0;
}

int step_norm(ps_problem* h) {
    double* part = h->cost_partials;
    HIP_OK(hipMemsetAsync(h->scalars + SC_DXP2, 0, sizeof(double), h->stream));
    HIP_OK(hipMemsetAsync(h->scalars + SC_DXL2, 0, sizeof(double), h->stream));
    if (h->nr > 0) {
        const int b = std::min(256, cdiv((long)h->nr * h->D, 256));
        hipLaunchKernelGGL(k_sumsq_partials, dim3(b), dim3(256), 0, h->stream, (long)h->nr * h->D, h->x, 1.0, part);
        hipLaunchKernelGGL(k_reduce_partials, dim3(1), dim3(256), 0, h->stream, b, part, h->scalars + SC_DXP2);
    }
    if (h->nv > 0) {
        const int b = std::min(256, cdiv((long)h->nv * 3, 256));
        hipLaunchKernelGGL(k_sumsq_partials, dim3(b), dim3(256), 0, h->stream, (long)h->nv * 3, h->dxl, 1.0, part + 256);
        hipLaunchKernelGGL(k_reduce_partials, dim3(1), dim3(256), 0, h->stream, b, part + 256, h->scalars + SC_DXL2);
    }
    return 0;
}

int apply_update(ps_problem* h, double step, const int32_t* gate = nullptr, bool with_norm = false, long long* hearly = nullptr, long long eseq = 0) {
    h->params_moved_since_lin = true;
    h->prelin_valid = h->prelm_valid = h->ride_valid = false;
    StageTimer t(h, PS_ST_UPDATE);
    if (h->nr > 0) {
        double* sq = with_norm ? h->sq_part_p : nullptr;
        if (h->D == 6)
            hipLaunchKernelGGL(k_update_poses<6>, dim3(cdiv(h->P, 256)), dim3(256), 0, h->stream, h->P, h->pose_rid, h->x, step, h->poses, sq, gate, hearly, eseq);
        else
            hipLaunchKernelGGL(k_update_poses<3>, dim3(cdiv(h->P, 256)), dim3(256), 0, h->stream, h->P, h->pose_rid, h->x, step, h->poses, sq, gate, hearly, eseq);
    }
    if (h->nv > 0)
        hipLaunchKernelGGL(k_update_points, dim3(cdiv((long)h->nv * 3, 256)), dim3(256), 0, h->stream, h->nv,
                           h->lm_point, h->dxl, step, h->points, gate);
    return 0;
}

inline bool lm_cost_possible(const ps_problem* h) {
    return cost_packed_possible(h) && (!h->shard_out || (h->nccl_allreduce && h->nccl_comm));
}
int lm_cost_enqueue(ps_problem* h, double lambda, const int32_t* gate) {
    const int nbl = cdiv(h->lmw_nwaves, 4);
    if (h->params_moved_since_lin || lambda != h->lin_lambda) h->z_foreign = true;
    h->prelm_tag = ++h->prelm_seq;
    {
        StageTimer t(h, PS_ST_LANDMARK);
        const ObsWide wl{h->sidx_l, h->stiff_tab};
#define PS_LMC_LAUNCH(W, PF) hipLaunchKernelGGL((k_landmark_pass_packed<W, true, PF>), dim3(nbl), dim3(256), 0, h->stream, h->lmw_nwaves, h->lmw_first,    \
                           h->lmw_run, h->lm_ptr, h->lm_point, h->lobs, h->poses, h->points, h->pose_rid, h->ogroups, lambda, h->Z, h->Cinv, h->cvec,        \
                           h->status, wl, gate, h->cost_partials, h->h_lmfail_dev + (h->prelm_tag & 1), h->prelm_tag)
        if (h->packed_prefetch) { if (h->wide_obs) PS_LMC_LAUNCH(true, true); else PS_LMC_LAUNCH(false, true); }
        else if (h->wide_obs) PS_LMC_LAUNCH(true, false); else PS_LMC_LAUNCH(false, false);
#undef PS_LMC_LAUNCH
    }
    int n = nbl;
    if (h->F > 0) {
        StageTimer t(h, PS_ST_COST);
        hipLaunchKernelGGL(k_cost_factors<6>, dim3(h->ncost_fac), dim3(256), 0, h->stream, (int)h->F, h->f_i, h->f_j, h->f_Tinv, h->f_grp,
                           h->fgroups, h->poses, h->pose_rid, 1, h->cost_partials + nbl, gate);
        n += h->ncost_fac;
    }
    h->prelm_lambda = lambda;
    return n;
}
int lm_cost_pass(ps_problem* h, double lambda, int scalar_slot) {
    h->prelin_valid = h->ride_valid = false;
    const int n = lm_cost_enqueue(h, lambda, nullptr);
    hipLaunchKernelGGL(k_reduce_partials, dim3(1), dim3(256), 0, h->stream, n, h->cost_partials, h->scalars + scalar_slot);
    h->prelm_pending = false; h->prelm_valid = true;
    return 0;
}

int gn_tail(ps_problem* h, int linesearch, const int32_t* gate, bool publish = false) {
    h->params_moved_since_lin = true;
    h->prelin_valid = h->prelm_valid = h->ride_valid = false;
    h->prelm_pending = false;
    const bool fused = linesearch && h->nv > 0 && h->nr > 0 && h->D == 6;
    long long* const hearly = (publish && h->spec_next && !h->spec_enqueued && gate) ? h->h_early_dev : nullptr;
    const long long eseq = hearly ? ++h->early_seq : 0;
    h->early_armed = hearly != nullptr;
    const bool stamp_in_backsub = h->nv > 0;
    if (h->lm_md && lm_md_ensure(h)) return -1;
    if (backsub(h, gate, fused, stamp_in_backsub ? hearly : nullptr, eseq)) return -1;
    if (h->lm_md && lm_md_enqueue(h, gate)) return -1;
    int ncost = 0;
    if (!linesearch) { StageTimer t(h, PS_ST_COST); ncost = cost_partials_pass(h, 0, gate); }
    if (!fused && apply_update(h, 1.0, gate, true, stamp_in_backsub ? nullptr : hearly, eseq)) return -1;
    if (!stamp_in_backsub && (fused || h->nr == 0)) h->early_armed = false;
    const bool lm_cost = fused && (publish || (h->shard_out && h->nccl_allreduce && h->nccl_comm)) && h->expect_next && lm_cost_possible(h);
    if (lm_cost) {
        ncost = lm_cost_enqueue(h, h->lin_lambda, gate);
        h->prelm_pending = true;
    } else if (linesearch) { StageTimer t(h, PS_ST_COST); ncost = cost_partials_pass(h, 1, gate); }
    double* o_cost = h->shard_out ? h->shard_buf : h->scalars + (linesearch ? SC_COST : SC_LINCOST);
    double* o_dxl = h->shard_out ? h->shard_buf + 1 : h->scalars + SC_DXL2;
    hipLaunchKernelGGL(k_reduce3, dim3(3), dim3(256), 0, h->stream,
                       ncost, h->cost_partials, o_cost,
                       h->nsq_p, h->sq_part_p, h->nr > 0 ? h->scalars + SC_DXP2 : nullptr,
                       nsq_l_now(h), h->sq_part_l, (h->nv > 0 || h->shard_out) ? o_dxl : nullptr, gate,
                       h->status, h->scalars, publish ? h->h_status_dev : nullptr, publish ? h->h_scalars_dev : nullptr,
                       h->arrivals, publish ? h->h_seq_dev : nullptr, publish ? ++h->seq : 0LL);
    return 0;
}

}
```

### pyslam_amd/csrc/ps_k_linearize.h

```cpp
#pragma once

#define PS_LM_GROUP 16

PS_DEV double group16_sum(double v) {
    v = dpp_shift_add<0x111, 0xf, 0xf>(v);
    v = dpp_shift_add<0x112, 0xf, 0xf>(v);
    v = dpp_shift_add<0x114, 0xf, 0xe>(v);
    v = dpp_shift_add<0x118, 0xf, 0xc>(v);
    return __shfl(v, (int)(threadIdx.x & 63) | 15, 64);
}

#define PS_ZROW 16

PS_DEV void lm_emit_m(const ReprojEval& ev, double M00, double M10, double M11, double M20, double M21,
                      double M22, double* __restrict__ m) {
#pragma unroll
    for (int a = 0; a < 3; ++a) {
        const double w0 = ev.Jp[a] * ev.Jl[0] + ev.Jp[6 + a] * ev.Jl[3] + ev.Jp[12 + a] * ev.Jl[6];
        const double w1 = ev.Jp[a] * ev.Jl[1] + ev.Jp[6 + a] * ev.Jl[4] + ev.Jp[12 + a] * ev.Jl[7];
        const double w2 = ev.Jp[a] * ev.Jl[2] + ev.Jp[6 + a] * ev.Jl[5] + ev.Jp[12 + a] * ev.Jl[8];
        m[3 * a] = w0 * M00;
        m[3 * a + 1] = w0 * M10 + w1 * M11;
        m[3 * a + 2] = w0 * M20 + w1 * M21 + w2 * M22;
    }
}

PS_DEV void zrow_cross(const double* __restrict__ m, const double* __restrict__ pc, double* __restrict__ l) {
#pragma unroll
    for (int k = 0; k < 3; ++k) {
        l[k] = pc[1] * m[6 + k] - pc[2] * m[3 + k];
        l[3 + k] = pc[2] * m[k] - pc[0] * m[6 + k];
        l[6 + k] = pc[0] * m[3 + k] - pc[1] * m[k];
    }
}

PS_DEV void zrow_expand(const double* __restrict__ m, const double* __restrict__ pc, double* __restrict__ z) {
#pragma unroll
    for (int k = 0; k < 9; ++k) z[k] = m[k];
    zrow_cross(m, pc, z + 9);
}

#ifndef PS_LM_WAVES
#define PS_LM_WAVES 3
#endif
template <bool WIDE>
__global__ __launch_bounds__(256) __attribute__((amdgpu_waves_per_eu(PS_LM_WAVES, 8))) void k_landmark_pass(
    int nv, const int32_t* __restrict__ lm_ptr, const int32_t* __restrict__ lm_point,
    const LObs* __restrict__ lobs, const double* __restrict__ poses,
    const double* __restrict__ points, const int32_t* __restrict__ pose_rid,
    const ObsGroup* __restrict__ groups, double lambda,
    double* __restrict__ Z, double* __restrict__ Cinv, double* __restrict__ cvec,
    int32_t* __restrict__ status, int ablate, ObsWide wide)
{
    const int v = blockIdx.x * (blockDim.x / PS_LM_GROUP) + threadIdx.x / PS_LM_GROUP;
    const int sub = threadIdx.x & (PS_LM_GROUP - 1);
    const bool live = v < nv;
    int b = 0, e = 0;
    double pw[3] = {0.0, 0.0, 0.0};
    if (live) {
        b = lm_ptr[v]; e = lm_ptr[v + 1];
        const int pt = lm_point[v];
        pw[0] = points[3 * pt]; pw[1] = points[3 * pt + 1]; pw[2] = points[3 * pt + 2];
    }
    const bool single = (e - b) <= PS_LM_GROUP;

    double H00 = 0, H10 = 0, H11 = 0, H20 = 0, H21 = 0, H22 = 0, b0 = 0, b1 = 0, b2 = 0;
    ReprojEval ev;
    bool have = false, variable_pose = false;
    int rid_of_obs = -1;
    for (int i = b + sub; i < e; i += PS_LM_GROUP) {
        const LObs o = lobs[i];
        const int pose = PS_POSE_OF(o);
        const Se3 T = se3_load(poses + 12 * pose);
        rid_of_obs = pose_rid[pose];
        variable_pose = rid_of_obs >= 0;
        reproj_eval_obs<true, true, WIDE>(T, pw, &o.u, groups, PS_GRP_OF(o), wide, i, ev);
        have = true;
        const double* J = ev.Jl;
#pragma unroll
        for (int k = 0; k < 3; ++k) {
            H00 += J[3 * k] * J[3 * k];
            H10 += J[3 * k + 1] * J[3 * k];
            H11 += J[3 * k + 1] * J[3 * k + 1];
            H20 += J[3 * k + 2] * J[3 * k];
            H21 += J[3 * k + 2] * J[3 * k + 1];
            H22 += J[3 * k + 2] * J[3 * k + 2];
            b0 -= J[3 * k] * ev.r[k];
            b1 -= J[3 * k + 1] * ev.r[k];
            b2 -= J[3 * k + 2] * ev.r[k];
        }
    }
    H00 = group16_sum(H00); H10 = group16_sum(H10); H11 = group16_sum(H11);
    H20 = group16_sum(H20); H21 = group16_sum(H21); H22 = group16_sum(H22);
    b0 = group16_sum(b0); b1 = group16_sum(b1); b2 = group16_sum(b2);

    const double damp = 1.0 + lambda;
    H00 *= damp; H11 *= damp; H22 *= damp;
    const double M00 = ps_rsqrt(H00);
    const double l10 = H10 * M00, l20 = H20 * M00;
    const double d1 = H11 - l10 * l10;
    const double M11 = ps_rsqrt(d1);
    const double l21 = (H21 - l20 * l10) * M11;
    const double d2 = H22 - l20 * l20 - l21 * l21;
    const double M22 = ps_rsqrt(d2);
    const double M10 = -l10 * M00 * M11;
    const double M21 = -l21 * M11 * M22;
    const double M20 = -(l20 * M00 + l21 * M10) * M22;
    if (live && sub == 0) {
        if (!(H00 > 0.0) || !(d1 > 0.0) || !(d2 > 0.0)) atomicAdd(&status[ST_LM_FAIL], 1);
        double* ci = Cinv + 6 * (size_t)v;
        ci[0] = M00; ci[1] = M10; ci[2] = M11; ci[3] = M20; ci[4] = M21; ci[5] = M22;
        double* cv = cvec + 3 * (size_t)v;
        cv[0] = M00 * b0;
        cv[1] = M10 * b0 + M11 * b1;
        cv[2] = M20 * b0 + M21 * b1 + M22 * b2;
    }
    __shared__ __attribute__((aligned(16))) double zst[4][64 * PS_ZROW];
    const int lane = threadIdx.x & 63, wv = threadIdx.x >> 6;
    if (__ballot(single || !live) == ~0ull && !(ablate & 2)) {
        const int row0 = __shfl(b, 0, 64);
        const int eend = max(max(__shfl(e, 0, 64), __shfl(e, 16, 64)), max(__shfl(e, 32, 64), __shfl(e, 48, 64)));
        const int nrows = eend - row0;
        if (have) {
            double z[PS_ZROW];
#pragma unroll
            for (int k = 0; k < PS_ZROW; ++k) z[k] = 0.0;
            z[12] = -1.0;
            if (variable_pose) {
                lm_emit_m(ev, M00, M10, M11, M20, M21, M22, z);
                z[9] = ev.pc[0]; z[10] = ev.pc[1]; z[11] = ev.pc[2];
                z[12] = (double)rid_of_obs;
            }
            double2* dst = reinterpret_cast<double2*>(&zst[wv][PS_ZROW * (b + sub - row0)]);
#pragma unroll
            for (int k = 0; k < PS_ZROW / 2; ++k) dst[k] = make_double2(z[2 * k], z[2 * k + 1]);
        }
        __builtin_amdgcn_wave_barrier();
        if (!(ablate & 1)) {
            const double2* src = reinterpret_cast<const double2*>(zst[wv]);
            double2* out = reinterpret_cast<double2*>(Z + PS_ZROW * (size_t)row0);
            for (int k = lane; k < nrows * (PS_ZROW / 2); k += 64) out[k] = src[k];
        }
        return;
    }
    if (!live) return;
    for (int i = b + sub; i < e; i += PS_LM_GROUP) {
        const LObs o = lobs[i];
        const int pose = PS_POSE_OF(o);
        double* z = Z + PS_ZROW * (size_t)i;
        const int rid = pose_rid[pose];
        z[12] = (double)rid;
        if (rid < 0 || (ablate & 1)) continue;
        if (!single) {
            const Se3 T = se3_load(poses + 12 * pose);
            reproj_eval_obs<true, true, WIDE>(T, pw, &o.u, groups, PS_GRP_OF(o), wide, i, ev);
        }
        lm_emit_m(ev, M00, M10, M11, M20, M21, M22, z);
        z[9] = ev.pc[0]; z[10] = ev.pc[1]; z[11] = ev.pc[2];
    }
}

PS_DEV void pose_sandwich(const double* __restrict__ e, const double* __restrict__ pc, double* __restrict__ acc) {
    const double x = pc[0], y = pc[1], z = pc[2];
    const double E[3][3] = {{e[0], e[1], e[2]}, {e[1], e[3], e[4]}, {e[2], e[4], e[5]}};
    double F[3][3];
#pragma unroll
    for (int i = 0; i < 3; ++i) {
        F[i][0] = E[i][2] * y - E[i][1] * z;
        F[i][1] = E[i][0] * z - E[i][2] * x;
        F[i][2] = E[i][1] * x - E[i][0] * y;
    }
    acc[0] += e[0]; acc[1] += e[1]; acc[2] += e[2]; acc[3] += F[0][0]; acc[4] += F[0][1]; acc[5] += F[0][2];
    acc[6] += e[3]; acc[7] += e[4]; acc[8] += F[1][0]; acc[9] += F[1][1]; acc[10] += F[1][2];
    acc[11] += e[5]; acc[12] += F[2][0]; acc[13] += F[2][1]; acc[14] += F[2][2];
    acc[15] += y * F[2][0] - z * F[1][0];
    acc[16] += y * F[2][1] - z * F[1][1];
    acc[17] += y * F[2][2] - z * F[1][2];
    acc[18] += z * F[0][1] - x * F[2][1];
    acc[19] += z * F[0][2] - x * F[2][2];
    acc[20] += x * F[1][2] - y * F[0][2];
}

#define PS_NPOSE_ACC 33
#ifndef PS_POSE_TRANSPOSE
#define PS_POSE_TRANSPOSE 1
#endif
typedef const __attribute__((address_space(1))) void* ps_gptr_t;
typedef __attribute__((address_space(3))) void* ps_lptr_t;

#ifndef PS_POSE_WAVES
#define PS_POSE_WAVES 3
#endif
template <bool WIDE>
__global__ __launch_bounds__(256) __attribute__((amdgpu_waves_per_eu(PS_POSE_WAVES, 8))) void k_pose_pass(
    const PItem* __restrict__ items,
    const LObs* __restrict__ pobs ,
    const double* __restrict__ poses, const double* __restrict__ points,
    const ObsGroup* __restrict__ groups, const double* __restrict__ Cinv,
    const double* __restrict__ cvec, double* __restrict__ partial, int want_diag ,
    ObsWide wide, int nitems, int per_xcd ,
    int zero_first, const int32_t* __restrict__ zero_slots, int nzero_slots, double* __restrict__ S, double* __restrict__ ztail, int ntail)
{
    __shared__ double red[4][PS_NPOSE_ACC];
#if PS_POSE_TRANSPOSE
    __shared__ double tr[4][64 * 17];
#endif
    if ((int)blockIdx.x >= zero_first) {
        const int e = ((int)blockIdx.x - zero_first) * 256 + (int)threadIdx.x, ns = 36 * nzero_slots;
        if (e < ns) { const int k = e / 36; S[(size_t)zero_slots[k] * 36 + (e - 36 * k)] = 0.0; }
        else if (e - ns < ntail) ztail[e - ns] = 0.0;
        return;
    }
    const int item = per_xcd > 0 ? (int)(blockIdx.x & 7) * per_xcd + (int)(blockIdx.x >> 3) : (int)blockIdx.x;
    if (item >= nitems) return;
    const PItem it = items[item];
    const int w = threadIdx.x >> 6, lane = threadIdx.x & 63;
    const Se3 T = se3_load(poses + 12 * (size_t)it.pad);
    double acc[PS_NPOSE_ACC];
#pragma unroll
    for (int k = 0; k < PS_NPOSE_ACC; ++k) acc[k] = 0.0;
    for (int i = it.start + threadIdx.x; i < it.end; i += 256) {
        const LObs o = pobs[i];
        const int v = PS_POSE_OF(o) - 1;
        const double pw[3] = {points[3 * (size_t)o.point], points[3 * (size_t)o.point + 1], points[3 * (size_t)o.point + 2]};
        double m[6] = {0, 0, 0, 0, 0, 0}, c0 = 0.0, c1 = 0.0, c2 = 0.0;
        if (v >= 0) {
            const double* ci = Cinv + 6 * (size_t)v;
#pragma unroll
            for (int k = 0; k < 6; ++k) m[k] = ci[k];
            c0 = cvec[3 * (size_t)v]; c1 = cvec[3 * (size_t)v + 1]; c2 = cvec[3 * (size_t)v + 2];
        }
        ReprojEval ev;
        reproj_eval_obs<true, true, WIDE>(T, pw, &o.u, groups, PS_GRP_OF(o), wide, i, ev);
        double G[6], t3[3];
        {
            const double* J = ev.Jp;
            G[0] = J[0] * J[0] + J[6] * J[6] + J[12] * J[12];
            G[1] = J[0] * J[1] + J[6] * J[7] + J[12] * J[13];
            G[2] = J[0] * J[2] + J[6] * J[8] + J[12] * J[14];
            G[3] = J[1] * J[1] + J[7] * J[7] + J[13] * J[13];
            G[4] = J[1] * J[2] + J[7] * J[8] + J[13] * J[14];
            G[5] = J[2] * J[2] + J[8] * J[8] + J[14] * J[14];
#pragma unroll
            for (int a = 0; a < 3; ++a) t3[a] = J[a] * ev.r[0] + J[6 + a] * ev.r[1] + J[12 + a] * ev.r[2];
        }
        if (want_diag) {
            double d21[21];
#pragma unroll
            for (int k = 0; k < 21; ++k) d21[k] = 0.0;
            pose_sandwich(G, ev.pc, d21);
            acc[27] += d21[0]; acc[28] += d21[6]; acc[29] += d21[11]; acc[30] += d21[15]; acc[31] += d21[18]; acc[32] += d21[20];
        }
        if (v >= 0) {
            double m9[9];
            lm_emit_m(ev, m[0], m[1], m[2], m[3], m[4], m[5], m9);
            G[0] -= m9[0] * m9[0] + m9[1] * m9[1] + m9[2] * m9[2];
            G[1] -= m9[0] * m9[3] + m9[1] * m9[4] + m9[2] * m9[5];
            G[2] -= m9[0] * m9[6] + m9[1] * m9[7] + m9[2] * m9[8];
            G[3] -= m9[3] * m9[3] + m9[4] * m9[4] + m9[5] * m9[5];
            G[4] -= m9[3] * m9[6] + m9[4] * m9[7] + m9[5] * m9[8];
            G[5] -= m9[6] * m9[6] + m9[7] * m9[7] + m9[8] * m9[8];
#pragma unroll
            for (int a = 0; a < 3; ++a) t3[a] += m9[3 * a] * c0 + m9[3 * a + 1] * c1 + m9[3 * a + 2] * c2;
        }
        pose_sandwich(G, ev.pc, acc);
        acc[21] -= t3[0]; acc[22] -= t3[1]; acc[23] -= t3[2];
        acc[24] -= ev.pc[1] * t3[2] - ev.pc[2] * t3[1];
        acc[25] -= ev.pc[2] * t3[0] - ev.pc[0] * t3[2];
        acc[26] -= ev.pc[0] * t3[1] - ev.pc[1] * t3[0];
    }
#if PS_POSE_TRANSPOSE
    {
        double* trw = tr[w];
#pragma unroll
        for (int h2 = 0; h2 < 2; ++h2) {
            const int k0 = 17 * h2, nk = h2 ? PS_NPOSE_ACC - 17 : 17;
#pragma unroll
            for (int k = 0; k < 17; ++k) if (k < nk) trw[lane * 17 + k] = acc[k0 + k];
            __builtin_amdgcn_wave_barrier();
            if (lane < nk) {
                double s = 0.0;
#pragma unroll 8
                for (int l = 0; l < 64; ++l) s += trw[l * 17 + lane];
                red[w][k0 + lane] = s;
            }
            __builtin_amdgcn_wave_barrier();
        }
    }
#else
#pragma unroll
    for (int k = 0; k < PS_NPOSE_ACC; ++k) {
        const double s = wave_sum(acc[k]);
        if (lane == 0) red[w][k] = s;
    }
#endif
    __syncthreads();
// ... 3 lines not shown
}

template <bool WIDE, bool DIAG>
PS_DEV void pose_obs_compact(const Se3& T, const LObs& o, const double* __restrict__ pw, const double* __restrict__ m,
                             double c0, double c1, double c2, int v, const ObsGroup* __restrict__ groups, int gfirst_id,
                             const ObsGroup& gfirst, const double* __restrict__ Sl,
                             double* __restrict__ G, double* __restrict__ t3, double* __restrict__ pc, double* __restrict__ dg) {
    ReprojEval ev;
    reproj_eval_obs_fetched<true, true, WIDE>(T, pw, &o.u, groups, PS_GRP_OF(o), gfirst_id, gfirst, Sl, ev);
    {
        const double* J = ev.Jp;
        G[0] = J[0] * J[0] + J[6] * J[6] + J[12] * J[12];
        G[1] = J[0] * J[1] + J[6] * J[7] + J[12] * J[13];
        G[2] = J[0] * J[2] + J[6] * J[8] + J[12] * J[14];
        G[3] = J[1] * J[1] + J[7] * J[7] + J[13] * J[13];
        G[4] = J[1] * J[2] + J[7] * J[8] + J[13] * J[14];
        G[5] = J[2] * J[2] + J[8] * J[8] + J[14] * J[14];
#pragma unroll
        for (int a = 0; a < 3; ++a) t3[a] = J[a] * ev.r[0] + J[6 + a] * ev.r[1] + J[12 + a] * ev.r[2];
    }
    if (DIAG) {
        double d21[21];
#pragma unroll
        for (int k = 0; k < 21; ++k) d21[k] = 0.0;
        pose_sandwich(G, ev.pc, d21);
        dg[0] = d21[0]; dg[1] = d21[6]; dg[2] = d21[11]; dg[3] = d21[15]; dg[4] = d21[18]; dg[5] = d21[20];
    }
    if (v >= 0) {
        double m9[9];
        lm_emit_m(ev, m[0], m[1], m[2], m[3], m[4], m[5], m9);
        G[0] -= m9[0] * m9[0] + m9[1] * m9[1] + m9[2] * m9[2];
        G[1] -= m9[0] * m9[3] + m9[1] * m9[4] + m9[2] * m9[5];
        G[2] -= m9[0] * m9[6] + m9[1] * m9[7] + m9[2] * m9[8];
        G[3] -= m9[3] * m9[3] + m9[4] * m9[4] + m9[5] * m9[5];
        G[4] -= m9[3] * m9[6] + m9[4] * m9[7] + m9[5] * m9[8];
        G[5] -= m9[6] * m9[6] + m9[7] * m9[7] + m9[8] * m9[8];
#pragma unroll
        for (int a = 0; a < 3; ++a) t3[a] += m9[3 * a] * c0 + m9[3 * a + 1] * c1 + m9[3 * a + 2] * c2;
    }
    pc[0] = ev.pc[0]; pc[1] = ev.pc[1]; pc[2] = ev.pc[2];
}

PS_DEV double pose_cross_sub(double acc, double a, double b, double c, double d) {
#pragma clang fp contract(off)
    return acc - __builtin_fma(a, b, -(c * d));
}

template <bool DIAG>
PS_DEV void pose_acc_add(const double* __restrict__ G, const double* __restrict__ t3, const double* __restrict__ pc,
                         const double* __restrict__ dg, double* __restrict__ acc) {
    if (DIAG) { acc[27] += dg[0]; acc[28] += dg[1]; acc[29] += dg[2]; acc[30] += dg[3]; acc[31] += dg[4]; acc[32] += dg[5]; }
    pose_sandwich(G, pc, acc);
    acc[21] -= t3[0]; acc[22] -= t3[1]; acc[23] -= t3[2];
    acc[24] = pose_cross_sub(acc[24], pc[1], t3[2], pc[2], t3[1]);
    acc[25] = pose_cross_sub(acc[25], pc[2], t3[0], pc[0], t3[2]);
    acc[26] = pose_cross_sub(acc[26], pc[0], t3[1], pc[1], t3[0]);
}

template <bool WIDE>
PS_DEV void pose_obs_gather(const LObs& o, int si, const double* __restrict__ points, const double* __restrict__ Cinv,
                            const double* __restrict__ cvec, const ObsWide& wide, double* __restrict__ pw, double* __restrict__ m,
                            double* __restrict__ c, double* __restrict__ Sl) {
    const int v = PS_POSE_OF(o) - 1;
    pw[0] = points[3 * (size_t)o.point]; pw[1] = points[3 * (size_t)o.point + 1]; pw[2] = points[3 * (size_t)o.point + 2];
    if (v >= 0) {
        const double* ci = Cinv + 6 * (size_t)v;
#pragma unroll
        for (int k = 0; k < 6; ++k) m[k] = ci[k];
        c[0] = cvec[3 * (size_t)v]; c[1] = cvec[3 * (size_t)v + 1]; c[2] = cvec[3 * (size_t)v + 2];
    }
    if (WIDE) {
        const double* sp = wide.stiff + 9 * (size_t)si;
#pragma unroll
        for (int k = 0; k < 9; ++k) Sl[k] = sp[k];
    }
}

#define PS_POSE_PF_OBS 512
template <bool WIDE, bool DIAG>
__global__ __launch_bounds__(256) __attribute__((amdgpu_waves_per_eu((WIDE || DIAG) ? 3 : 4, 8))) void k_pose_pass_pf(
    const PItem* __restrict__ items, const LObs* __restrict__ pobs, const double* __restrict__ poses,
    const double* __restrict__ points, const ObsGroup* __restrict__ groups, const double* __restrict__ Cinv,
    const double* __restrict__ cvec, double* __restrict__ partial, ObsWide wide, int nitems, int per_xcd,
    int zero_first, const int32_t* __restrict__ zero_slots, int nzero_slots, double* __restrict__ S, double* __restrict__ ztail, int ntail)
{
    __shared__ double red[4][PS_NPOSE_ACC];
    __shared__ double tr[4][64 * 17];
    if ((int)blockIdx.x >= zero_first) {
        const int e = ((int)blockIdx.x - zero_first) * 256 + (int)threadIdx.x, ns = 36 * nzero_slots;
        if (e < ns) { const int k = e / 36; S[(size_t)zero_slots[k] * 36 + (e - 36 * k)] = 0.0; }
        else if (e - ns < ntail) ztail[e - ns] = 0.0;
        return;
    }
    const int item = per_xcd > 0 ? (int)(blockIdx.x & 7) * per_xcd + (int)(blockIdx.x >> 3) : (int)blockIdx.x;
    if (item >= nitems) return;
    const PItem it = items[item];
    const int w = threadIdx.x >> 6, lane = threadIdx.x & 63;
    const int ia = it.start + (int)threadIdx.x, ib = ia + 256;
    const bool ha = ia < it.end, hb = ib < it.end;
    const Se3 T = se3_load(poses + 12 * (size_t)it.pad);
    LObs oa = {0.0, 0.0, 0.0, 0, 0}, ob = {0.0, 0.0, 0.0, 0, 0};
    int sa = 0, sb = 0;
    if (ha) { oa = pobs[ia]; if (WIDE) sa = wide.sidx[ia]; }
    if (hb) { ob = pobs[ib]; if (WIDE) sb = wide.sidx[ib]; }
    double pwa[3], ma[6] = {0, 0, 0, 0, 0, 0}, ca[3] = {0.0, 0.0, 0.0}, Sla[9];
    double pwb[3], mb[6] = {0, 0, 0, 0, 0, 0}, cb[3] = {0.0, 0.0, 0.0}, Slb[9];
    double Ga[6], ta[3], pca[3], da[6], Gb[6], tb[3], pcb[3], db[6];
    if (ha) {
        pose_obs_gather<WIDE>(oa, sa, points, Cinv, cvec, wide, pwa, ma, ca, Sla);
        if (hb) pose_obs_gather<WIDE>(ob, sb, points, Cinv, cvec, wide, pwb, mb, cb, Slb);
        const int g0 = __builtin_amdgcn_readfirstlane((int)PS_GRP_OF(oa));
        const ObsGroup g = obs_group_fetch(groups, g0);
        pose_obs_compact<WIDE, DIAG>(T, oa, pwa, ma, ca[0], ca[1], ca[2], PS_POSE_OF(oa) - 1, groups, g0, g, Sla, Ga, ta, pca, da);
        if (hb) pose_obs_compact<WIDE, DIAG>(T, ob, pwb, mb, cb[0], cb[1], cb[2], PS_POSE_OF(ob) - 1, groups, g0, g, Slb, Gb, tb, pcb, db);
    }
    double acc[PS_NPOSE_ACC];
#pragma unroll
    for (int k = 0; k < PS_NPOSE_ACC; ++k) acc[k] = 0.0;
    if (ha) pose_acc_add<DIAG>(Ga, ta, pca, da, acc);
    if (hb) pose_acc_add<DIAG>(Gb, tb, pcb, db, acc);
    {
        double* trw = tr[w];
#pragma unroll
        for (int h2 = 0; h2 < 2; ++h2) {
            const int k0 = 17 * h2, nk = h2 ? PS_NPOSE_ACC - 17 : 17;
#pragma unroll
            for (int k = 0; k < 17; ++k) if (k < nk) trw[lane * 17 + k] = acc[k0 + k];
            __builtin_amdgcn_wave_barrier();
            if (lane < nk) {
                double s = 0.0;
#pragma unroll 8
                for (int l = 0; l < 64; ++l) s += trw[l * 17 + lane];
                red[w][k0 + lane] = s;
            }
            __builtin_amdgcn_wave_barrier();
        }
    }
    __syncthreads();
    if (threadIdx.x < PS_NPOSE_ACC)
        partial[(size_t)item * PS_NPOSE_ACC + threadIdx.x] =
            ((red[0][threadIdx.x] + red[1][threadIdx.x]) + red[2][threadIdx.x]) + red[3][threadIdx.x];
}

PS_DEV void pose_finalize_wave(int rid, int lane, const int32_t* __restrict__ pitem_ptr,
                               const double* __restrict__ partial, const int32_t* __restrict__ diag_slot,
                               double lambda, double* __restrict__ S, double* __restrict__ g, double* v ,
                               double* s_new = nullptr, double* g_new = nullptr)
{
    if (lane < PS_NPOSE_ACC) {
        double s = 0.0;
        for (int it = pitem_ptr[rid]; it < pitem_ptr[rid + 1]; ++it) s += partial[(size_t)it * PS_NPOSE_ACC + lane];
        v[lane] = s;
    }
    __builtin_amdgcn_wave_barrier();
    double sn = 0.0, gn = 0.0;
    if (lane < 36) {
        const int r = lane / 6, c = lane % 6;
        const int a = r < c ? r : c, b = r < c ? c : r;
        const int idx = a * 6 - (a * (a - 1)) / 2 + (b - a);
        double val = v[idx];
        if (r == c) val += lambda * v[27 + r];
        const size_t o = (size_t)diag_slot[rid] * 36 + lane;
        sn = S[o] + val;
        S[o] = sn;
    }
    if (lane < 6) { const size_t o = (size_t)rid * 6 + lane; gn = g[o] + v[21 + lane]; g[o] = gn; }
    if (s_new) *s_new = sn;
    if (g_new) *g_new = gn;
}

__global__ __launch_bounds__(64) void k_pose_finalize(
    int nr, const int32_t* __restrict__ pitem_ptr, const double* __restrict__ partial,
    const int32_t* __restrict__ diag_slot, double lambda,
    double* __restrict__ S, double* __restrict__ g)
{
    __shared__ double v[PS_NPOSE_ACC];
    pose_finalize_wave(blockIdx.x, threadIdx.x, pitem_ptr, partial, diag_slot, lambda, S, g, v);
// ... 261 lines not shown
```

### pyslam_amd/csrc/ps_k_packed.h

```cpp
#pragma once

#define PS_LMW_MAXOBS 16

__global__ __launch_bounds__(256) void k_lmw_maxobs(int nv, const int32_t* __restrict__ lm_ptr, int32_t* __restrict__ out) {
    const int v = blockIdx.x * blockDim.x + threadIdx.x;
    const int n = v < nv ? lm_ptr[v + 1] - lm_ptr[v] : -1;
    int mx = n, mn = n < 0 ? INT_MAX : n;
    for (int off = 32; off; off >>= 1) { mx = max(mx, __shfl_xor(mx, off, 64)); mn = min(mn, __shfl_xor(mn, off, 64)); }
    if ((threadIdx.x & 63) == 0 && mx >= 0) { atomicMax(out, mx); atomicMin(out + 1, mn); }
}

struct __attribute__((aligned(16))) LmwRun { int32_t v0, v1, row0, nrows; };

PS_DEV int lmw_first_landmark(int nv, int target, const int32_t* __restrict__ lm_ptr) {
    int lo = 0, hi = nv;
    while (lo < hi) { const int mid = (lo + hi) >> 1; if (lm_ptr[mid] < target) lo = mid + 1; else hi = mid; }
    return lo;
}

__global__ __launch_bounds__(256) void k_lmw_items(int nv, int nwaves, int W, const int32_t* __restrict__ lm_ptr, int32_t* __restrict__ first,
                                                   LmwRun* __restrict__ run) {
    const int w = blockIdx.x * blockDim.x + threadIdx.x;
    if (w > nwaves) return;
    if (w == nwaves) { first[w] = nv; return; }
    const int v0 = lmw_first_landmark(nv, W * w, lm_ptr);
    const int v1 = w + 1 == nwaves ? nv : lmw_first_landmark(nv, W * (w + 1), lm_ptr);
    first[w] = v0;
    const int row0 = lm_ptr[v0];
    run[w] = LmwRun{v0, v1, row0, lm_ptr[v1] - row0};
}

struct LmwSeg { int v, lane0, lane1, nrows, row0; bool valid, head; };
PS_DEV LmwSeg lmw_segment_of(int v0, int nlm, int row0, int nrows, int start, int lane, volatile int32_t* flags ) {
    LmwSeg s;
    s.row0 = row0;
    s.nrows = nrows;
    flags[lane] = 0;
    __builtin_amdgcn_wave_barrier();
    if (lane < nlm) flags[start - s.row0] = 1;
    __builtin_amdgcn_wave_barrier();
    const unsigned long long hm = __ballot(flags[lane] != 0);
    const unsigned long long le = (lane == 63) ? ~0ull : ((2ull << lane) - 1ull);
    const unsigned long long below = hm & le, above = hm & ~le;
    s.valid = lane < s.nrows;
    s.v = v0 + __popcll(below) - 1;
    s.lane0 = below ? 63 - __clzll(below) : 0;
    s.lane1 = above ? __ffsll((long long)above) - 1 : s.nrows;
    s.lane1 = min(s.lane1, s.nrows);
    s.head = s.valid && lane == s.lane0;
    return s;
}
PS_DEV LmwSeg lmw_segment(int v0, int v1, const int32_t* __restrict__ lm_ptr, int lane, volatile int32_t* flags ) {
    const int nlm = v1 - v0;
    const int start = (lane < nlm) ? lm_ptr[v0 + lane] : 0;
    const int row0 = lm_ptr[v0];
    return lmw_segment_of(v0, nlm, row0, lm_ptr[v1] - row0, start, lane, flags);
}

PS_DEV LmwRun lmw_run_and_gate(const LmwRun* __restrict__ lmw_run, int nwaves, int gw , const int32_t* __restrict__ gate,
                               int& gate_word) {
    int4 r = make_int4(0, 0, 0, 0);
    if (gw < nwaves) r = reinterpret_cast<const int4*>(lmw_run)[gw];
    int g = 1;
    if (gate) g = gate[ST_PCG_DONE];
    asm volatile("" : "+s"(r.x), "+s"(r.y), "+s"(r.z), "+s"(r.w), "+s"(g));
    gate_word = g;
    return LmwRun{r.x, r.y, r.z, r.w};
}

template <bool WIDE, bool COST, bool PF>
__global__ __launch_bounds__(256) __attribute__((amdgpu_waves_per_eu(PS_LM_WAVES, 8))) void k_landmark_pass_packed(
    int nwaves, const int32_t* __restrict__ lmw_first, const LmwRun* __restrict__ lmw_run, const int32_t* __restrict__ lm_ptr,
    const int32_t* __restrict__ lm_point,
    const LObs* __restrict__ lobs, const double* __restrict__ poses,
    const double* __restrict__ points, const int32_t* __restrict__ pose_rid,
    const ObsGroup* __restrict__ groups, double lambda,
    double* __restrict__ Z, double* __restrict__ Cinv, double* __restrict__ cvec,
    int32_t* __restrict__ status, ObsWide wide,
    const int32_t* __restrict__ gate = nullptr, double* __restrict__ cost_part = nullptr,
    long long* __restrict__ fail_word = nullptr, long long fail_tag = 0)
{
    __shared__ __attribute__((aligned(16))) double zst[4][64 * PS_ZROW];
    __shared__ int32_t flags[4][64];
    __shared__ double csum[16];
    const int lane = threadIdx.x & 63;
    int wv, v0, v1;
    LmwRun rn = {0, 0, 0, 0};
    if (PF) {
        wv = __builtin_amdgcn_readfirstlane(threadIdx.x >> 6);
        int gate_word;
        rn = lmw_run_and_gate(lmw_run, nwaves, blockIdx.x * 4 + wv, COST ? gate : nullptr, gate_word);
        if (COST && gate_word != 1) return;
        v0 = rn.v0; v1 = rn.v1;
    } else {
        if (COST && gate && gate[ST_PCG_DONE] != 1) return;
        wv = threadIdx.x >> 6;
        const int gw = blockIdx.x * 4 + wv;
        v0 = gw < nwaves ? lmw_first[gw] : 0; v1 = gw < nwaves ? lmw_first[gw + 1] : 0;
    }
    double obs_cost = 0.0;
    if (v1 > v0) {
    double* sm = zst[wv];
    ReprojEval ev;
    bool variable_pose = false;
    int rid_of_obs = -1;
    double hb[9] = {0, 0, 0, 0, 0, 0, 0, 0, 0};
    LmwSeg sg;
    if (PF) {
        const int nlm = v1 - v0, i = rn.row0 + lane;
        const int start = (lane < nlm) ? lm_ptr[v0 + lane] : 0;
        if (lane < rn.nrows) {
            const LObs o = lobs[i];
            const int si = WIDE ? wide.sidx[i] : 0;
            const int pose = PS_POSE_OF(o), grp = PS_GRP_OF(o);
            const Se3 T = se3_load(poses + 12 * pose);
            const double pw[3] = {points[3 * (size_t)o.point], points[3 * (size_t)o.point + 1], points[3 * (size_t)o.point + 2]};
            rid_of_obs = pose_rid[pose];
            double Sl[9];
            if (WIDE) {
                const double* sp = wide.stiff + 9 * (size_t)si;
#pragma unroll
                for (int k = 0; k < 9; ++k) Sl[k] = sp[k];
            }
            const int g0 = __builtin_amdgcn_readfirstlane(grp);
            const ObsGroup g = obs_group_fetch(groups, g0);
            reproj_eval_obs_fetched<true, true, WIDE>(T, pw, &o.u, groups, grp, g0, g, Sl, ev);
        }
        sg = lmw_segment_of(v0, nlm, rn.row0, rn.nrows, start, lane, flags[wv]);
    } else {
        sg = lmw_segment(v0, v1, lm_ptr, lane, flags[wv]);
        const int i = sg.row0 + lane;
        if (sg.valid) {
            const int pt = lm_point[sg.v];
            const double pw[3] = {points[3 * (size_t)pt], points[3 * (size_t)pt + 1], points[3 * (size_t)pt + 2]};
            const LObs o = lobs[i];
            const int pose = PS_POSE_OF(o);
            const Se3 T = se3_load(poses + 12 * pose);
            rid_of_obs = pose_rid[pose];
            reproj_eval_obs<true, true, WIDE>(T, pw, &o.u, groups, PS_GRP_OF(o), wide, i, ev);
        }
    }
    if (sg.valid) {
        variable_pose = rid_of_obs >= 0;
        if (COST) obs_cost = ev.cost;
        const double* J = ev.Jl;
#pragma unroll
        for (int k = 0; k < 3; ++k) {
            hb[0] += J[3 * k] * J[3 * k];
            hb[1] += J[3 * k + 1] * J[3 * k];
            hb[2] += J[3 * k + 1] * J[3 * k + 1];
            hb[3] += J[3 * k + 2] * J[3 * k];
            hb[4] += J[3 * k + 2] * J[3 * k + 1];
            hb[5] += J[3 * k + 2] * J[3 * k + 2];
            hb[6] -= J[3 * k] * ev.r[k];
            hb[7] -= J[3 * k + 1] * ev.r[k];
            hb[8] -= J[3 * k + 2] * ev.r[k];
        }
    }
#pragma unroll
    for (int k = 0; k < 9; ++k) sm[9 * lane + k] = hb[k];
    __builtin_amdgcn_wave_barrier();
    {
        const int jpos = lane - sg.lane0, nseg = sg.lane1 - sg.lane0;
        double part[9];
#pragma unroll
        for (int it = 0; it < 9; ++it) {
            const int q = jpos + it * nseg;
            part[it] = 0.0;
            if (sg.valid && q < 9) {
                double acc = 0.0;
                for (int l = sg.lane0; l < sg.lane1; ++l) acc += sm[9 * l + q];
                part[it] = acc;
            }
        }
        __builtin_amdgcn_wave_barrier();
#pragma unroll
        for (int it = 0; it < 9; ++it) {
            const int q = jpos + it * nseg;
            if (sg.valid && q < 9) sm[9 * sg.lane0 + q] = part[it];
        }
        __builtin_amdgcn_wave_barrier();
    }
    if (sg.head) {
        double a[9];
#pragma unroll
        for (int k = 0; k < 9; ++k) a[k] = sm[9 * lane + k];
        const double damp = 1.0 + lambda;
        const double H00 = a[0] * damp, H10 = a[1], H11 = a[2] * damp, H20 = a[3], H21 = a[4], H22 = a[5] * damp;
        const double M00 = ps_rsqrt(H00);
        const double l10 = H10 * M00, l20 = H20 * M00;
        const double d1 = H11 - l10 * l10;
        const double M11 = ps_rsqrt(d1);
        const double l21 = (H21 - l20 * l10) * M11;
        const double d2 = H22 - l20 * l20 - l21 * l21;
        const double M22 = ps_rsqrt(d2);
        const double M10 = -l10 * M00 * M11;
        const double M21 = -l21 * M11 * M22;
        const double M20 = -(l20 * M00 + l21 * M10) * M22;
        if (!(H00 > 0.0) || !(d1 > 0.0) || !(d2 > 0.0)) {
            if (COST && fail_word) *reinterpret_cast<volatile long long*>(fail_word) = fail_tag;
            else atomicAdd(&status[ST_LM_FAIL], 1);
        }
        double* ci = Cinv + 6 * (size_t)sg.v;
        ci[0] = M00; ci[1] = M10; ci[2] = M11; ci[3] = M20; ci[4] = M21; ci[5] = M22;
        double* cv = cvec + 3 * (size_t)sg.v;
        cv[0] = M00 * a[6];
        cv[1] = M10 * a[6] + M11 * a[7];
        cv[2] = M20 * a[6] + M21 * a[7] + M22 * a[8];
        double* mo = sm + 9 * lane;
        mo[0] = M00; mo[1] = M10; mo[2] = M11; mo[3] = M20; mo[4] = M21; mo[5] = M22;
    }
    __builtin_amdgcn_wave_barrier();
    double M[6] = {0, 0, 0, 0, 0, 0};
    if (sg.valid) {
#pragma unroll
        for (int k = 0; k < 6; ++k) M[k] = sm[9 * sg.lane0 + k];
    }
    __builtin_amdgcn_wave_barrier();
    if (sg.valid) {
        double z[PS_ZROW];
#pragma unroll
        for (int k = 0; k < PS_ZROW; ++k) z[k] = 0.0;
        z[12] = -1.0;
        if (variable_pose) {
            lm_emit_m(ev, M[0], M[1], M[2], M[3], M[4], M[5], z);
            z[9] = ev.pc[0]; z[10] = ev.pc[1]; z[11] = ev.pc[2];
            z[12] = (double)rid_of_obs;
        }
        double2* dst = reinterpret_cast<double2*>(sm + PS_ZROW * lane);
#pragma unroll
        for (int k = 0; k < PS_ZROW / 2; ++k) dst[k] = make_double2(z[2 * k], z[2 * k + 1]);
    }
    __builtin_amdgcn_wave_barrier();
    const double2* src = reinterpret_cast<const double2*>(sm);
    double2* out = reinterpret_cast<double2*>(Z + PS_ZROW * (size_t)sg.row0);
    for (int k = lane; k < sg.nrows * (PS_ZROW / 2); k += 64) out[k] = src[k];
    }
    if (COST) {
        obs_cost = block_sum(obs_cost, csum);
        if (threadIdx.x == 0) cost_part[blockIdx.x] = obs_cost;
    }
}

template <bool WIDE, bool PF>
__global__ __launch_bounds__(256) void k_cost_packed(
    int nwaves, const int32_t* __restrict__ lmw_first, const LmwRun* __restrict__ lmw_run, const int32_t* __restrict__ lm_ptr,
    const int32_t* __restrict__ lm_point,
    const LObs* __restrict__ lobs, const double* __restrict__ poses, const double* __restrict__ points,
    const ObsGroup* __restrict__ groups, double* __restrict__ cost_part, const int32_t* __restrict__ gate, ObsWide wide)
{
    __shared__ double csum[16];
    if (PF) {
        const int lane = threadIdx.x & 63, gw = blockIdx.x * 4 + __builtin_amdgcn_readfirstlane(threadIdx.x >> 6);
        int gate_word;
        const LmwRun rn = lmw_run_and_gate(lmw_run, nwaves, gw, gate, gate_word);
        if (gate_word != 1) return;
        double c = 0.0;
        if (lane < rn.nrows) {
            const int i = rn.row0 + lane;
            const LObs o = lobs[i];
            const int si = WIDE ? wide.sidx[i] : 0;
            const int grp = PS_GRP_OF(o);
            const Se3 T = se3_load(poses + 12 * PS_POSE_OF(o));
            const double pw[3] = {points[3 * (size_t)o.point], points[3 * (size_t)o.point + 1], points[3 * (size_t)o.point + 2]};
            double Sl[9];
            if (WIDE) {
                const double* sp = wide.stiff + 9 * (size_t)si;
#pragma unroll
                for (int k = 0; k < 9; ++k) Sl[k] = sp[k];
            }
            const int g0 = __builtin_amdgcn_readfirstlane(grp);
            const ObsGroup g = obs_group_fetch(groups, g0);
            ReprojEval ev;
            reproj_eval_obs_fetched<false, false, WIDE>(T, pw, &o.u, groups, grp, g0, g, Sl, ev);
            c = ev.cost;
        }
        c = block_sum(c, csum);
        if (threadIdx.x == 0) cost_part[blockIdx.x] = c;
        return;
    }
    if (gate && gate[ST_PCG_DONE] != 1) return;
    const int lane = threadIdx.x & 63, wv = threadIdx.x >> 6, gw = blockIdx.x * 4 + wv;
    double c = 0.0;
    const int v0 = gw < nwaves ? lmw_first[gw] : 0, v1 = gw < nwaves ? lmw_first[gw + 1] : 0;
    if (v1 > v0) {
        const int row0 = lm_ptr[v0], nrows = lm_ptr[v1] - row0;
        if (lane < nrows) {
            const int i = row0 + lane;
            const LObs o = lobs[i];
            const Se3 T = se3_load(poses + 12 * PS_POSE_OF(o));
            const double pw[3] = {points[3 * (size_t)o.point], points[3 * (size_t)o.point + 1], points[3 * (size_t)o.point + 2]};
            ReprojEval ev;
            reproj_eval_obs<false, false, WIDE>(T, pw, &o.u, groups, PS_GRP_OF(o), wide, i, ev);
            c = ev.cost;
        }
    }
    c = block_sum(c, csum);
    if (threadIdx.x == 0) cost_part[blockIdx.x] = c;
}

template <bool MD, bool PF>
__global__ __launch_bounds__(256) void k_backsub_packed(
    int nwaves, const int32_t* __restrict__ lmw_first, const LmwRun* __restrict__ lmw_run, const int32_t* __restrict__ lm_ptr,
    const double* __restrict__ Z, const double* __restrict__ Cinv, const double* __restrict__ cvec,
    const double* __restrict__ xp, double* __restrict__ dxl,
    double* __restrict__ sq_part ,
    const int32_t* __restrict__ gate,
    int nblk_l, const int32_t* __restrict__ lm_point, double* __restrict__ points,
    int P, const int32_t* __restrict__ pose_rid, double* __restrict__ poses, double* __restrict__ sq_part_p,
    long long* __restrict__ hearly, long long eseq, double* __restrict__ md_part = nullptr, double lam_ratio = 0.0)
{
    __shared__ double lds[16];
    __shared__ double sm3[4][64 * 3];
    __shared__ int32_t flags[4][64];
    LmwRun rn = {0, 0, 0, 0};
    bool closed;
    if (PF) {
        int gate_word;
        rn = lmw_run_and_gate(lmw_run, nwaves, blockIdx.x * 4 + __builtin_amdgcn_readfirstlane(threadIdx.x >> 6), gate, gate_word);
// ... 133 lines not shown
```

### pyslam_amd/csrc/ps_k_tail.h

```cpp
#pragma once
#include "ps_stop_rule.h"

PS_DEV bool mo_solve6(const double* __restrict__ tot, double lambda, double* __restrict__ x) {
    double H[6][6], il[6];
    bool ok = true;
    int n = 0;
#pragma unroll
    for (int a = 0; a < 6; ++a)
#pragma unroll
        for (int b = a; b < 6; ++b) { H[a][b] = tot[n]; H[b][a] = tot[n]; ++n; }
#pragma unroll
    for (int a = 0; a < 6; ++a) H[a][a] += lambda * tot[27 + a];
#pragma unroll
    for (int j = 0; j < 6; ++j) {
        double d = H[j][j];
#pragma unroll
        for (int k = 0; k < j; ++k) d -= H[j][k] * H[j][k];
        ok = ok && (d > 0.0);
        il[j] = ps_rsqrt(d);
#pragma unroll
        for (int i = j + 1; i < 6; ++i) {
            double v = H[i][j];
#pragma unroll
            for (int k = 0; k < j; ++k) v -= H[i][k] * H[j][k];
// ... 404 lines not shown
template <bool WIDE>
__global__ __launch_bounds__(256) void k_cost_reproj(
    long n, const LObs* __restrict__ lobs, const double* __restrict__ poses,
    const double* __restrict__ points, const int32_t* __restrict__ pose_rid,
    const int32_t* __restrict__ point_vid, const ObsGroup* __restrict__ groups,
    int include_all, double* __restrict__ partials, const int32_t* __restrict__ gate, ObsWide wide)
{
    __shared__ double lds[16];
    if (gate && gate[ST_PCG_DONE] != 1) return;
    double c = 0.0;
    for (long i = (long)blockIdx.x * blockDim.x + threadIdx.x; i < n; i += (long)gridDim.x * blockDim.x) {
        const LObs o = lobs[i];
        const int pose = PS_POSE_OF(o);
        if (!include_all && pose_rid[pose] < 0 && point_vid[o.point] < 0) continue;
        const Se3 T = se3_load(poses + 12 * pose);
        const double pw[3] = {points[3 * o.point], points[3 * o.point + 1], points[3 * o.point + 2]};
        ReprojEval ev;
        reproj_eval_obs<false, false, WIDE>(T, pw, &o.u, groups, PS_GRP_OF(o), wide, i, ev);
        c += ev.cost;
    }
    c = block_sum(c, lds);
    if (threadIdx.x == 0) partials[blockIdx.x] = c;
}

template <int D>
__global__ __launch_bounds__(256) void k_cost_factors(
    int nf, const int32_t* __restrict__ f_i, const int32_t* __restrict__ f_j,
    const double* __restrict__ f_Tinv, const int32_t* __restrict__ f_grp,
    const FactorGroup* __restrict__ groups, const double* __restrict__ poses,
    const int32_t* __restrict__ pose_rid, int include_all, double* __restrict__ partials,
    const int32_t* __restrict__ gate)
{
    typedef PoseOps<D> G;
    __shared__ double lds[16];
    if (gate && gate[ST_PCG_DONE] != 1) return;
    double cst = 0.0;
    for (int f = blockIdx.x * blockDim.x + threadIdx.x; f < nf; f += gridDim.x * blockDim.x) {
        const int i = f_i[f], j = f_j[f];
        if (!include_all && pose_rid[j] < 0 && (i < 0 || pose_rid[i] < 0)) continue;
        const FactorGroup& grp = groups[f_grp[f]];
        const typename G::T T2 = G::load(poses + G::W * (size_t)j);
        const typename G::T To = G::load(f_Tinv + G::W * (size_t)f);
        typename G::T E;
        if (i >= 0) E = G::mul(T2, G::mul(G::inv(G::load(poses + G::W * (size_t)i)), To));
        else E = G::mul(T2, To);
        double xi[D];
        G::log(E, xi);
#pragma unroll
        for (int k = 0; k < D; ++k) {
            double rk = 0.0;
#pragma unroll
            for (int m = 0; m < D; ++m) rk += grp.S[k * D + m] * xi[m];
            cst += ps_loss_rho(grp.loss_id, grp.loss_k, rk);
        }
    }
    cst = block_sum(cst, lds);
    if (threadIdx.x == 0) partials[blockIdx.x] = cst;
}

__global__ __launch_bounds__(256) void k_sumsq_partials(
    long n, const double* __restrict__ v, double scale, double* __restrict__ partials)
{
    __shared__ double lds[16];
    double s = 0.0;
    for (long i = (long)blockIdx.x * blockDim.x + threadIdx.x; i < n; i += (long)gridDim.x * blockDim.x) {
        const double a = scale * v[i];
        s += a * a;
    }
    s = block_sum(s, lds);
    if (threadIdx.x == 0) partials[blockIdx.x] = s;
}

PS_DEV double strided_sum8(const double* __restrict__ p, int n) {
    double a[8] = {0.0, 0.0, 0.0, 0.0, 0.0, 0.0, 0.0, 0.0};
    int i = threadIdx.x;
    for (; i + 7 * 256 < n; i += 8 * 256) {
#pragma unroll
        for (int k = 0; k < 8; ++k) a[k] += p[i + k * 256];
    }
    for (int k = 0; i < n; i += 256, ++k) a[k] += p[i];
    return ((a[0] + a[1]) + (a[2] + a[3])) + ((a[4] + a[5]) + (a[6] + a[7]));
}

__global__ __launch_bounds__(256) void k_reduce3(
    int n0, const double* __restrict__ p0, double* __restrict__ o0,
    int n1, const double* __restrict__ p1, double* __restrict__ o1,
    int n2, const double* __restrict__ p2, double* __restrict__ o2, const int32_t* __restrict__ gate,
    const int32_t* __restrict__ status, const double* __restrict__ scalars,
    int32_t* __restrict__ hst, double* __restrict__ hsc,
    int32_t* __restrict__ arrivals , long long* __restrict__ hseq, long long seq)
{
    __shared__ double lds[16];
    const bool open = !(gate && gate[ST_PCG_DONE] != 1);
    if (hst && blockIdx.x == 0) {
        const int t = threadIdx.x;
        if (t < ST_NWORDS) hst[t] = status[t];
        else if (t < ST_NWORDS + SC_NWORDS) {
            const int k = t - ST_NWORDS;
            if (!open || (o0 != scalars + k && o1 != scalars + k && o2 != scalars + k)) hsc[k] = scalars[k];
        }
    }
    const int n = blockIdx.x == 0 ? n0 : (blockIdx.x == 1 ? n1 : n2);
    const double* p = blockIdx.x == 0 ? p0 : (blockIdx.x == 1 ? p1 : p2);
    double* o = blockIdx.x == 0 ? o0 : (blockIdx.x == 1 ? o1 : o2);
    if (open && o) {
        double s = strided_sum8(p, n);
        s = block_sum(s, lds);
        if (threadIdx.x == 0) {
            o[0] = s;
            if (hsc && o >= scalars && o < scalars + SC_NWORDS) hsc[o - scalars] = s;
        }
    }
    if (hseq) {
        __syncthreads();
        if (threadIdx.x == 0) {
            __threadfence_system();
            if (atomicAdd(arrivals, 1) == (int)gridDim.x - 1) {
                *arrivals = 0;
                __threadfence_system();
                *reinterpret_cast<volatile long long*>(hseq) = seq;
            }
        }
    }
}

__global__ __launch_bounds__(64) void k_publish(
    const int32_t* __restrict__ status, const double* __restrict__ scalars, const double* __restrict__ shard,
    int32_t* __restrict__ hst, double* __restrict__ hsc, double* __restrict__ hshard,
    long long* __restrict__ hseq, long long seq)
{
    const int t = threadIdx.x;
    if (t < ST_NWORDS) hst[t] = status[t];
    else if (t < ST_NWORDS + SC_NWORDS) hsc[t - ST_NWORDS] = scalars[t - ST_NWORDS];
    else if (t < ST_NWORDS + SC_NWORDS + 2) hshard[t - ST_NWORDS - SC_NWORDS] = shard[t - ST_NWORDS - SC_NWORDS];
    __syncthreads();
    if (t == 0) {
        __threadfence_system();
        *reinterpret_cast<volatile long long*>(hseq) = seq;
    }
}

__global__ __launch_bounds__(256) void k_reduce_partials(int n, const double* __restrict__ partials,
                                                          double* __restrict__ out)
{
    __shared__ double lds[16];
    double s = strided_sum8(partials, n);
    s = block_sum(s, lds);
    if (threadIdx.x == 0) out[0] = s;
}

template <bool WIDE>
__global__ __launch_bounds__(256) void k_debug_reproj(
    long n, const LObs* __restrict__ lobs, const int32_t* __restrict__ lorig,
    const double* __restrict__ poses, const double* __restrict__ points,
    const ObsGroup* __restrict__ groups, double* __restrict__ r, double* __restrict__ jp,
    double* __restrict__ jl, ObsWide wide)
{
    const long i = (long)blockIdx.x * blockDim.x + threadIdx.x;
    if (i >= n) return;
    const LObs o = lobs[i];
    const Se3 T = se3_load(poses + 12 * PS_POSE_OF(o));
    const double pw[3] = {points[3 * o.point], points[3 * o.point + 1], points[3 * o.point + 2]};
    ReprojEval ev;
    reproj_eval_obs<true, true, WIDE>(T, pw, &o.u, groups, PS_GRP_OF(o), wide, i, ev);
    const size_t k = (size_t)lorig[i];
    for (int a = 0; a < 3; ++a) r[3 * k + a] = ev.r[a];
    for (int a = 0; a < 18; ++a) jp[18 * k + a] = ev.Jp[a];
    for (int a = 0; a < 9; ++a) jl[9 * k + a] = ev.Jl[a];
}

__global__ __launch_bounds__(256) void k_dense_normal(int m, int n, const double* __restrict__ J,
                                                       const double* __restrict__ r,
                                                       double* __restrict__ H, double* __restrict__ g)
{
    const int t = blockIdx.x * blockDim.x + threadIdx.x;
    if (t < n * n) {
        const int a = t / n, b = t % n;
        double s = 0.0;
        for (int k = 0; k < m; ++k) s += J[(size_t)k * n + a] * J[(size_t)k * n + b];
        H[t] = s;
    }
    if (t < n) {
        double s = 0.0;
        for (int k = 0; k < m; ++k) s -= J[(size_t)k * n + t] * r[k];
        g[t] = s;
    }
}

__global__ __launch_bounds__(256) void k_dense_chol_solve(int n, int nrhs, double* __restrict__ H,
                                                           double* __restrict__ B, int32_t* __restrict__ status)
{
    const int t = threadIdx.x;
    for (int j = 0; j < n; ++j) {
        __syncthreads();
        if (t == 0) {
            double d = H[(size_t)j * n + j];
            for (int k = 0; k < j; ++k) d -= H[(size_t)j * n + k] * H[(size_t)j * n + k];
            if (!(d > 0.0)) atomicAdd(&status[ST_DIAG_FAIL], 1);
            H[(size_t)j * n + j] = sqrt(d);
        }
        __syncthreads();
        const double l = H[(size_t)j * n + j];
        for (int i = j + 1 + t; i < n; i += 256) {
            double v = H[(size_t)i * n + j];
            for (int k = 0; k < j; ++k) v -= H[(size_t)i * n + k] * H[(size_t)j * n + k];
            H[(size_t)i * n + j] = v / l;
// ... 127 lines not shown
```

### pyslam_amd/csrc/ps_math.h

```cpp
#pragma once
#include <hip/hip_runtime.h>

#define PS_DEV __device__ __forceinline__

__device__ __forceinline__ double ps_rsqrt(double x) {
    double y = __builtin_amdgcn_rsq(x);
    const double hx = 0.5 * x;
    y = y * (1.5 - hx * y * y);
    y = y * (1.5 - hx * y * y);
    return y;
}
#define PS_SMALL_ANGLE 1e-8

enum { PS_LOSS_L2 = 0, PS_LOSS_L1 = 1, PS_LOSS_CAUCHY = 2, PS_LOSS_HUBER = 3,
       PS_LOSS_TUKEY = 4, PS_LOSS_TDIST = 5 };

PS_DEV double ps_loss_rho(int id, double k, double x) {
#pragma clang fp contract(off)
    const double a = fabs(x);
    switch (id) {
    case PS_LOSS_L2: return 0.5 * x * x;
    case PS_LOSS_L1: return a;
    case PS_LOSS_CAUCHY: { const double q = x / k; return (0.5 * k * k) * log(1.0 + q * q); }
    case PS_LOSS_HUBER: return (a <= k) ? 0.5 * x * x : k * (a - 0.5 * k);
// ... 180 lines not shown
    return o;
}

PS_DEV Se2 se2_mul(const Se2& A, const Se2& B) {
    Se2 o;
    o.R[0] = A.R[0] * B.R[0] + A.R[1] * B.R[2]; o.R[1] = A.R[0] * B.R[1] + A.R[1] * B.R[3];
    o.R[2] = A.R[2] * B.R[0] + A.R[3] * B.R[2]; o.R[3] = A.R[2] * B.R[1] + A.R[3] * B.R[3];
    o.t[0] = A.R[0] * B.t[0] + A.R[1] * B.t[1] + A.t[0];
    o.t[1] = A.R[2] * B.t[0] + A.R[3] * B.t[1] + A.t[1];
    return o;
}

PS_DEV void se2_log(const Se2& T, double* __restrict__ xi) {
    const double phi = atan2(T.R[2], T.R[0]);
    double a, b;
    if (fabs(phi) <= PS_SMALL_ANGLE) { a = 1.0; b = 0.5 * phi; }
    else { const double half = 0.5 * phi; a = half / tan(half); b = half; }
    xi[0] = a * T.t[0] + b * T.t[1];
    xi[1] = -b * T.t[0] + a * T.t[1];
    xi[2] = phi;
}

PS_DEV Se2 se2_exp(const double* __restrict__ xi) {
    Se2 T;
    const double phi = xi[2];
    const double c = cos(phi), s = sin(phi);
    T.R[0] = c; T.R[1] = -s; T.R[2] = s; T.R[3] = c;
    double a, b;
    if (fabs(phi) <= PS_SMALL_ANGLE) { a = 1.0; b = 0.5 * phi; }
    else { a = s / phi; b = (1.0 - c) / phi; }
    T.t[0] = a * xi[0] - b * xi[1];
    T.t[1] = b * xi[0] + a * xi[1];
    return T;
}

PS_DEV double se2_adjoint_entry_mem(const double* __restrict__ p, int r, int c) {
    if (r == 2) return (c == 2) ? 1.0 : 0.0;
    if (c < 2) return p[2 * r + c];
    return (r == 0) ? p[5] : -p[4];
}

PS_DEV double se2_adjoint_entry(const Se2& T, int r, int c) {
    if (r == 2) return (c == 2) ? 1.0 : 0.0;
    if (c < 2) return T.R[2 * r + c];
    return (r == 0) ? T.t[1] : -T.t[0];
}

template <int D> struct PoseOps;
template <> struct PoseOps<6> {
    typedef Se3 T;
    static constexpr int W = 12;
    static PS_DEV T load(const double* p) { return se3_load(p); }
    static PS_DEV void store(double* p, const T& x) { se3_store(p, x); }
    static PS_DEV T inv(const T& x) { return se3_inv(x); }
    static PS_DEV T mul(const T& a, const T& b) { return se3_mul(a, b); }
    static PS_DEV void log(const T& x, double* xi) { se3_log(x, xi); }
    static PS_DEV T exp(const double* xi) { return se3_exp(xi); }
    static PS_DEV double adj(const T& x, int r, int c) { return se3_adjoint_entry(x, r, c); }
    static PS_DEV double adj_mem(const double* p, int r, int c) { return se3_adjoint_entry_mem(p, r, c); }
};
template <> struct PoseOps<3> {
    typedef Se2 T;
    static constexpr int W = 6;
    static PS_DEV T load(const double* p) { return se2_load(p); }
    static PS_DEV void store(double* p, const T& x) { se2_store(p, x); }
    static PS_DEV T inv(const T& x) { return se2_inv(x); }
    static PS_DEV T mul(const T& a, const T& b) { return se2_mul(a, b); }
    static PS_DEV void log(const T& x, double* xi) { se2_log(x, xi); }
    static PS_DEV T exp(const double* xi) { return se2_exp(xi); }
    static PS_DEV double adj(const T& x, int r, int c) { return se2_adjoint_entry(x, r, c); }
    static PS_DEV double adj_mem(const double* p, int r, int c) { return se2_adjoint_entry_mem(p, r, c); }
};

struct ObsGroup { double cu, cv, fu, fv, b; double S[9]; int loss_id; int cam_type; double loss_k; };

struct ReprojEval {
    double r[3];
    double Jp[18];
    double Jl[9];
    double cost;
    double pc[3];
};

template <bool WITH_JP, bool WITH_JL>
PS_DEV void reproj_eval_s(const Se3& T, const double* __restrict__ pw, const double* __restrict__ uvd,
                          const ObsGroup& g, const double* __restrict__ Sv, ReprojEval& o) {
    double pc[3], rr[3], iz;
    const bool rgbd = g.cam_type == 1, mono = g.cam_type == 2;
    {
#pragma clang fp contract(off)
#pragma unroll
        for (int i = 0; i < 3; ++i)
            pc[i] = __builtin_fma(T.R[3 * i + 2], pw[2], __builtin_fma(T.R[3 * i + 1], pw[1], __builtin_fma(T.R[3 * i], pw[0], T.t[i])));
        iz = 1.0 / pc[2];
        const double e0 = __builtin_fma(g.fu * pc[0], iz, g.cu - uvd[0]);
        const double e1 = __builtin_fma(g.fv * pc[1], iz, g.cv - uvd[1]);
        const double e2 = mono ? 0.0 : (rgbd ? pc[2] - uvd[2] : __builtin_fma(g.fu * g.b, iz, -uvd[2]));
#pragma unroll
        for (int i = 0; i < 3; ++i) rr[i] = __builtin_fma(Sv[3 * i + 2], e2, __builtin_fma(Sv[3 * i + 1], e1, Sv[3 * i] * e0));
        o.cost = 0.0;
#pragma unroll
        for (int i = 0; i < 3; ++i) o.cost += ps_loss_rho(g.loss_id, g.loss_k, rr[i]);
    }
    o.pc[0] = pc[0]; o.pc[1] = pc[1]; o.pc[2] = pc[2];
    double s[3];
#pragma unroll
    for (int i = 0; i < 3; ++i) {
        const double ri = rr[i];
        s[i] = (i == 2 && mono) ? 1.0 : ps_loss_sqrt_weight(g.loss_id, g.loss_k, ri);
        o.r[i] = s[i] * ri;
    }
    if (!WITH_JP && !WITH_JL) return;
    const double iz2 = iz * iz;
    const double j00 = g.fu * iz, j02 = -g.fu * pc[0] * iz2;
    const double j11 = g.fv * iz, j12 = -g.fv * pc[1] * iz2;
    const double j22 = mono ? 0.0 : (rgbd ? 1.0 : -g.fu * g.b * iz2);
    double SJ[9];
    {
#pragma clang fp contract(off)
#pragma unroll
        for (int i = 0; i < 3; ++i) {
            SJ[3 * i] = s[i] * (Sv[3 * i] * j00);
            SJ[3 * i + 1] = s[i] * (Sv[3 * i + 1] * j11);
            SJ[3 * i + 2] = s[i] * __builtin_fma(Sv[3 * i + 2], j22, __builtin_fma(Sv[3 * i], j02, Sv[3 * i + 1] * j12));
        }
        if (WITH_JP) {
#pragma unroll
            for (int i = 0; i < 3; ++i) {
                const double a = SJ[3 * i], b = SJ[3 * i + 1], c = SJ[3 * i + 2];
                o.Jp[6 * i] = a; o.Jp[6 * i + 1] = b; o.Jp[6 * i + 2] = c;
                o.Jp[6 * i + 3] = __builtin_fma(c, pc[1], -(b * pc[2]));
                o.Jp[6 * i + 4] = __builtin_fma(a, pc[2], -(c * pc[0]));
                o.Jp[6 * i + 5] = __builtin_fma(b, pc[0], -(a * pc[1]));
            }
        }
        if (WITH_JL) {
#pragma unroll
            for (int i = 0; i < 3; ++i)
#pragma unroll
                for (int j = 0; j < 3; ++j)
                    o.Jl[3 * i + j] = __builtin_fma(SJ[3 * i + 2], T.R[6 + j], __builtin_fma(SJ[3 * i], T.R[j], SJ[3 * i + 1] * T.R[3 + j]));
        }
    }
}

template <bool WITH_JP, bool WITH_JL>
PS_DEV void reproj_eval(const Se3& T, const double* __restrict__ pw, const double* __restrict__ uvd,
                        const ObsGroup& g, ReprojEval& o) {
    reproj_eval_s<WITH_JP, WITH_JL>(T, pw, uvd, g, g.S, o);
}

template <bool WITH_JP, bool WITH_JL>
PS_DEV void reproj_eval_grp(const Se3& T, const double* __restrict__ pw, const double* __restrict__ uvd,
                            const ObsGroup* __restrict__ groups, int grp, ReprojEval& o) {
    for (;;) {
        const int g0 = __builtin_amdgcn_readfirstlane(grp);
        if (grp == g0) { reproj_eval<WITH_JP, WITH_JL>(T, pw, uvd, groups[g0], o); break; }
    }
}

struct ObsWide { const int32_t* sidx; const double* stiff; };

template <bool WITH_JP, bool WITH_JL, bool WIDE>
PS_DEV void reproj_eval_obs(const Se3& T, const double* __restrict__ pw, const double* __restrict__ uvd,
                            const ObsGroup* __restrict__ groups, int grp, const ObsWide& wide, long i, ReprojEval& o) {
    if (!WIDE) { reproj_eval_grp<WITH_JP, WITH_JL>(T, pw, uvd, groups, grp, o); return; }
    double Sl[9];
    const double* sp = wide.stiff + 9 * (size_t)wide.sidx[i];
#pragma unroll
    for (int k = 0; k < 9; ++k) Sl[k] = sp[k];
    for (;;) {
        const int g0 = __builtin_amdgcn_readfirstlane(grp);
        if (grp == g0) { reproj_eval_s<WITH_JP, WITH_JL>(T, pw, uvd, groups[g0], Sl, o); break; }
    }
}

PS_DEV ObsGroup obs_group_fetch(const ObsGroup* __restrict__ groups, int g0 ) {
    ObsGroup g = groups[g0];
    asm volatile("" : "+s"(g.cu), "+s"(g.cv), "+s"(g.fu), "+s"(g.fv), "+s"(g.b), "+s"(g.loss_k), "+s"(g.loss_id), "+s"(g.cam_type));
    asm volatile("" : "+s"(g.S[0]), "+s"(g.S[1]), "+s"(g.S[2]), "+s"(g.S[3]), "+s"(g.S[4]), "+s"(g.S[5]), "+s"(g.S[6]), "+s"(g.S[7]), "+s"(g.S[8]));
    return g;
}

template <bool WITH_JP, bool WITH_JL, bool WIDE>
PS_DEV void reproj_eval_obs_fetched(const Se3& T, const double* __restrict__ pw, const double* __restrict__ uvd,
                                    const ObsGroup* __restrict__ groups, int grp, int gfirst_id, const ObsGroup& gfirst,
                                    const double* __restrict__ Sl, ReprojEval& o) {
    for (;;) {
        const int g0 = __builtin_amdgcn_readfirstlane(grp);
        if (grp == g0) {
            ObsGroup g = gfirst;
            if (g0 != gfirst_id) g = groups[g0];
            reproj_eval_s<WITH_JP, WITH_JL>(T, pw, uvd, g, WIDE ? Sl : g.S, o);
            break;
        }
    }
}
```

### pyslam_amd/device.py

```python
import ctypes as C

import numpy as np

from pyslam_amd import _native as nat


COVARIANCE_MARGINALS_LIMIT = 12288


def _solve_options(o, opt, linesearch=None):
    o.max_iters, o.allow_nondecreasing_steps = int(opt.max_iters), int(bool(opt.allow_nondecreasing_steps))
    o.max_nondecreasing_steps = int(opt.max_nondecreasing_steps)
    o.linesearch = int(bool(opt.linesearch_max_iters > 0 if linesearch is None else linesearch))
    o.min_update_norm, o.min_cost = float(opt.min_update_norm), float(opt.min_cost)
    o.min_cost_decrease, o.lm_lambda = float(opt.min_cost_decrease), float(getattr(opt, 'lm_lambda', 0.))
    return o


class DeviceProblem:
    def __init__(self, lp, stream=None, extra_pairs=None):
        lib = nat.require_gpu()
        self._lib = lib
        self.lp = lp
        self.dof = lp.dof
# ... 286 lines not shown
        if vids is not None:
            vids = np.ascontiguousarray(vids, dtype=np.int32).reshape(-1)
        n = self.nv if vids is None else vids.shape[0]
        pts, status = np.zeros((n, 3)), np.zeros(n, dtype=np.int32)
        if n:
            nat.check(self._lib.ps_triangulate(self._h, n, nat.i32p(vids) if vids is not None else None, int(refine_iters),
                                               float(min_parallax_deg), int(bool(write_back)), nat.f64p(pts), nat.i32p(status)))
        return pts, status

    def get_dx(self):
        xp = np.zeros((self.nr, self.dof))
        xl = np.zeros((self.nv, 3))
        nat.check(self._lib.ps_get_dx(self._h, nat.f64p(xp), nat.f64p(xl)))
        return xp, xl

    def get_params(self, poses_out=None, points_out=None):
        if poses_out is not None or points_out is not None:
            nat.check(self._lib.ps_get_params(self._h, nat.f64p(poses_out), nat.f64p(points_out)))
            return poses_out, points_out
        poses = np.zeros((self.lp.num_poses, self.lp.pose_width))
        points = np.zeros((self.lp.num_points, 3))
        nat.check(self._lib.ps_get_params(self._h, nat.f64p(poses), nat.f64p(points)))
        return poses, points

    def set_params(self, poses=None, points=None):
        p = poses if poses is None or nat.is_resident(poses) else np.ascontiguousarray(poses, dtype=np.float64)
        q = points if points is None or nat.is_resident(points) else np.ascontiguousarray(points, dtype=np.float64)
        nat.check(self._lib.ps_set_params(self._h, nat.f64p(p), nat.f64p(q)))
        if self.host is not None and poses is not None:
            self._hposes = self._read_poses()

    def reduce_buffer(self):
        ptr, n = C.c_void_p(), C.c_int64()
        nat.check(self._lib.ps_reduce_buffer(self._h, C.byref(ptr), C.byref(n)))
        return ptr.value, n.value

    def shard_pack(self):
        nat.check(self._lib.ps_shard_pack(self._h))

    def shard_unpack(self):
        nat.check(self._lib.ps_shard_unpack(self._h))

    def reduced_system(self):
        nnzb, d = self.info['reduced_nnzb'], self.dof
        rp = np.zeros(self.nr + 1, dtype=np.int32)
        ci = np.zeros(max(nnzb, 1), dtype=np.int32)
        vals = np.zeros((max(nnzb, 1), d, d))
        g = np.zeros(max(self.nr * d, 1))
        nat.check(self._lib.ps_get_reduced_system(self._h, nat.i32p(rp), nat.i32p(ci), nat.f64p(vals), nat.f64p(g)))
        return rp, ci[:nnzb], vals[:nnzb], g[:self.nr * d]

    def reduced_dense(self):
        rp, ci, vals, g = self.reduced_system()
        d, n = self.dof, self.nr * self.dof
        S = np.zeros((n, n))
        for r in range(self.nr):
            for k in range(rp[r], rp[r + 1]):
                S[r * d:(r + 1) * d, ci[k] * d:(ci[k] + 1) * d] = vals[k]
        return S, g

    def landmark_factors(self):
        cinv, c = np.zeros((self.nv, 6)), np.zeros((self.nv, 3))
        nat.check(self._lib.ps_get_landmark_factors(self._h, nat.f64p(cinv), nat.f64p(c)))
        return cinv, c

    def packed_runs(self):
        nw = C.c_int32(0)
        nat.check(self._lib.ps_debug_packed_runs(self._h, C.byref(nw), 0, None, None, None, None))
        n = nw.value
        run, first, lm_ptr = np.zeros((n, 4), dtype=np.int32), np.zeros(n + 1, dtype=np.int32), np.zeros(self.nv + 1, dtype=np.int32)
        sq = np.zeros((n + 3) // 4)
        i32 = lambda a: a.ctypes.data_as(C.POINTER(C.c_int32))
        nat.check(self._lib.ps_debug_packed_runs(self._h, C.byref(nw), n, i32(run), i32(first), i32(lm_ptr), nat.f64p(sq)))
        return run, first, lm_ptr, sq

    def pose_items(self):
        ni = C.c_int32(0)
        nat.check(self._lib.ps_debug_pose_items(self._h, C.byref(ni), 0, None, None))
        n = ni.value
        items, partial = np.zeros((n, 3), dtype=np.int32), np.zeros((n, 33))
        nat.check(self._lib.ps_debug_pose_items(self._h, C.byref(ni), n, items.ctypes.data_as(C.POINTER(C.c_int32)), nat.f64p(partial)))
        return items, partial

    def debug_reproj_blocks(self):
        n = self.lp.num_obs
        r, jp, jl = np.zeros((n, 3)), np.zeros((n, 3, 6)), np.zeros((n, 3, 3))
        nat.check(self._lib.ps_debug_reproj_blocks(self._h, nat.f64p(r), nat.f64p(jp), nat.f64p(jl)))
        return r, jp, jl

    def debug_factor_blocks(self):
        f, d = self.lp.num_edges + self.lp.num_priors, self.lp.dof
        r, j1, j2 = np.zeros((f, d)), np.zeros((f, d, d)), np.zeros((f, d, d))
        nat.check(self._lib.ps_debug_factor_blocks(self._h, nat.f64p(r), nat.f64p(j1), nat.f64p(j2)))
        return r, j1, j2

    def debug_ldi_state(self):
        rec = np.zeros(12)
        nat.check(self._lib.ps_debug_ldi_read(self._h, 0, nat.f64p(rec), rec.size))
        keys = ('state', 'cur', 'n', 'np', 'kp', 'direct', 'fro_limit', 'last_its', 'seed_steps', 'nr', 'dof', 'ready')
        return {k: (float(v) if k == 'fro_limit' else int(v)) for k, v in zip(keys, rec)}

    def debug_ldi_read(self, what):
        s = self.debug_ldi_state()
        n, npad, kp, nr, d = s['n'], s['np'], s['kp'], s['nr'], s['dof']
        code, shape = {'S32': (1, (npad, npad)), 'X32': (2, (npad, npad)), 'Xu': (3, (npad, npad)), 'Xt': (4, (npad, kp)),
                       'Linv': (5, (nr, d, d)), 'coef': (6, (3,)), 'fro': (7, (1,)), 'r': (8, (n,)), 'z': (9, (n,))}[what]
        out = np.zeros(max(int(np.prod(shape)), 1))
        nat.check(self._lib.ps_debug_ldi_read(self._h, code, nat.f64p(out), out.size))
        return out[:int(np.prod(shape))].reshape(shape)

    def get_info(self):
        info = nat.ProblemInfo()
        nat.check(self._lib.ps_get_info(self._h, C.byref(info)))
        return {k: getattr(info, k) for k, _ in nat.ProblemInfo._fields_}

    def cg_restarts(self):
        info = nat.ProblemInfo()
        nat.check(self._lib.ps_get_info(self._h, C.byref(info)))
        return int(info.cg_restarts)

    def cg_kernel_launches(self):
        info = nat.ProblemInfo()
        nat.check(self._lib.ps_get_info(self._h, C.byref(info)))
        return int(info.cg_kernel_launches)

    def cg_persist_counts(self):
        info = nat.ProblemInfo()
        nat.check(self._lib.ps_get_info(self._h, C.byref(info)))
        return int(info.cg_persist_solves), int(info.cg_persist_failures)

    def cg_persist_recover_counts(self):
        return int(self.get_option('cg_persist_recovered')), int(self.get_option('cg_persist_recover_fallbacks'))

    def set_option(self, name, value):
        nat.check(self._lib.ps_set_option(self._h, name.encode(), float(value)))

    def get_option(self, name):
        v = C.c_double()
        nat.check(self._lib.ps_get_option(self._h, name.encode(), C.byref(v)))
        return v.value

    def set_profiling(self, level=2):
        nat.check(self._lib.ps_set_profiling(self._h, int(level)))

    def stage_times(self, reset=False):
        ms = (C.c_double * nat.PS_NUM_STAGES)()
        cnt = (C.c_int64 * nat.PS_NUM_STAGES)()
        nat.check(self._lib.ps_get_stage_times(self._h, ms, cnt, int(reset)))
        return {n: (ms[i], cnt[i]) for i, n in enumerate(nat.STAGE_NAMES)}


def dense_normal_solve(J, r, want_covariance=False):
    lib = nat.require_gpu()
    J = np.ascontiguousarray(J, dtype=np.float64)
    r = np.ascontiguousarray(r, dtype=np.float64).reshape(-1)
    m, n = J.shape
    dx = np.zeros(n)
    cov = np.zeros((n, n)) if want_covariance else None
    nat.check(lib.ps_dense_normal_solve(nat.f64p(J), nat.f64p(r), m, n, nat.f64p(dx), nat.f64p(cov)))
    return (dx, cov) if want_covariance else dx


def band_inverse(A, ncb, dof, bw, chunk_nodes=0):
    lib = nat.require_gpu()
    A = np.ascontiguousarray(A, dtype=np.float64)
    n = ncb * dof
# ... 349 lines not shown
```

Before: 0.2588.

## Fold end-of-step reduction into next pose-pass launch and shrink Z staging in LDS

Defers the k_reduce3 launch at the end of a GN/LM step and, when the next linearization zeroes by list, runs the three reduction blocks as leading blocks of the pose-pass kernel, which also clears the status words. This removes a separate small kernel launch per iteration. The landmark kernel's LDS staging for Z rows is shrunk from 16 to 14 doubles, with zero padding on the global write, and the prefetch variant's waves-per-EU hint is raised to 5. An asm barrier around the loss evaluation keeps the compiler from interleaving the rho computation. The deferred reduce adds flush points in sync, the spin loop and gn_tail, which brings ordering risk around status clearing and host publication.

New measurement: 0.2545, median of 3. No clear change (-1.7%).

```diff
diff --git a/include/pyslam_hip.h b/include/pyslam_hip.h
--- a/include/pyslam_hip.h
+++ b/include/pyslam_hip.h
@@ -187,6 +187,7 @@
 int ps_debug_packed_runs(ps_problem* h, int32_t* nwaves, int32_t capacity_waves, int32_t* run, int32_t* first, int32_t* lm_ptr,
                          double* sq_part);
 int ps_debug_pose_items(ps_problem* h, int32_t* nitems, int32_t capacity_items, int32_t* items, double* partial);
+int ps_debug_z_rows(ps_problem* h, int64_t* nrows, int64_t capacity_rows, double* z);
 
 int ps_set_option(ps_problem* h, const char* name, double value);
 int ps_get_option(ps_problem* h, const char* name, double* value);
diff --git a/pyslam_amd/_native.py b/pyslam_amd/_native.py
--- a/pyslam_amd/_native.py
+++ b/pyslam_amd/_native.py
@@ -136,6 +136,7 @@
     'ps_debug_table_checksums': (C.c_int, [H, C.POINTER(C.c_uint64), C.c_int, C.POINTER(C.c_int)]),
     'ps_debug_packed_runs': (C.c_int, [H, c_i32p, C.c_int32, c_i32p, c_i32p, c_i32p, c_f64p]),
     'ps_debug_pose_items': (C.c_int, [H, c_i32p, C.c_int32, c_i32p, c_f64p]),
+    'ps_debug_z_rows': (C.c_int, [H, C.POINTER(C.c_int64), C.c_int64, c_f64p]),
     'ps_set_option': (C.c_int, [H, C.c_char_p, C.c_double]),
     'ps_get_option': (C.c_int, [H, C.c_char_p, c_f64p]),
     'ps_set_profiling': (C.c_int, [H, C.c_int]),
diff --git a/pyslam_amd/csrc/ps_abi_solver.h b/pyslam_amd/csrc/ps_abi_solver.h
--- a/pyslam_amd/csrc/ps_abi_solver.h
+++ b/pyslam_amd/csrc/ps_abi_solver.h
@@ -857,6 +857,17 @@
     return 0;
 }
 
+int ps_debug_z_rows(ps_problem* h, int64_t* nrows, int64_t capacity_rows, double* z) {
+    if (!h || !nrows) return fail("null argument");
+    if (sync(h)) return -1;
+    int32_t nl = 0;
+    if (h->nv > 0) HIP_OK(hipMemcpy(&nl, h->lm_ptr + h->nv, 4, hipMemcpyDeviceToHost));
+    *nrows = nl;
+    if (z && capacity_rows < nl) return fail("ps_debug_z_rows: capacity too small");
+    if (z && nl) HIP_OK(hipMemcpy(z, h->Z, (size_t)nl * PS_ZROW * sizeof(double), hipMemcpyDeviceToHost));
+    return 0;
+}
+
 int ps_debug_ldi_read(ps_problem* h, int32_t what, double* out, int64_t capacity) {
     if (!h || !out) return fail("null argument");
     if (what == PS_LDI_READ_STATE) {
@@ -940,6 +951,7 @@
         h->prelin_valid = h->prelm_valid = h->ride_valid = false;
         return 0;
     }
+    if (!std::strcmp(name, "reduce_ride")) { h->reduce_ride = value != 0 ? 1 : 0; return 0; }
     if (!std::strcmp(name, "coarse_chol_band")) { h->coarse_chol_band = value != 0 ? 1 : 0; return 0; }
     if (std::strcmp(name, "cg_force_breakdown")) h->prelin_valid = h->prelm_valid = h->ride_valid = false;
     const char* refusal = nullptr;
@@ -971,6 +983,9 @@
     else if (n == "rows_lci_in_lds") *value = h->coarse_built && h->lagx_ok && h->rows_lci_lds ? 1.0 : 0.0;
     else if (n == "packed_prefetch") *value = (double)h->packed_prefetch;
     else if (n == "pose_prefetch") *value = (double)h->pose_prefetch;
+    else if (n == "reduce_ride") *value = (double)h->reduce_ride;
+    else if (n == "reduce_ridden") *value = (double)h->reduce_ridden;
+    else if (n == "reduce_launched") *value = (double)h->reduce_launched;
     else if (n == "cg_persist_recover") *value = (double)h->cg_persist_recover;
     else if (n == "cg_persist_recover_lds") *value = (double)h->cg_persist_recover_lds;
     else if (n == "cg_persist_recover_need") *value = h->coarse_built && h->cp_ok ? (double)h->cp_rec_lds : 0.0;
diff --git a/pyslam_amd/csrc/ps_core.hip b/pyslam_amd/csrc/ps_core.hip
--- a/pyslam_amd/csrc/ps_core.hip
+++ b/pyslam_amd/csrc/ps_core.hip
@@ -393,6 +393,10 @@
     int packed_prefetch = 1;
     int pose_prefetch = 1;
     int pose_chunk = 256;
+    int reduce_ride = 1;
+    bool reduce_pending = false;
+    ReduceRide red_ride{};
+    long reduce_ridden = 0, reduce_launched = 0;
     int coarse_chol_band = 1;
     int coarse_chol_bw = 0;
     bool ldi_ready = false;
diff --git a/pyslam_amd/csrc/ps_host_cg.h b/pyslam_amd/csrc/ps_host_cg.h
--- a/pyslam_amd/csrc/ps_host_cg.h
+++ b/pyslam_amd/csrc/ps_host_cg.h
@@ -58,7 +58,16 @@
     if (h->pending.empty()) h->ev_used = 0;
 }
 
+int flush_reduce(ps_problem* h) {
+    if (!h->reduce_pending) return 0;
+    h->reduce_pending = false;
+    hipLaunchKernelGGL(k_reduce3, dim3(3), dim3(256), 0, h->stream, h->red_ride);
+    ++h->reduce_launched;
+    return 0;
+}
+
 int sync(ps_problem* h) {
+    if (flush_reduce(h)) return -1;
     HIP_OK(hipStreamSynchronize(h->stream));
     h->persist_release();
     drain_timers(h);
@@ -77,6 +86,10 @@
     for (long spins = 0; spins < 400000000L; ++spins) {
         if (kick_mode == 2 && h->side_todo && !h->side_ready && *ws == h->setup_seq) { h->side_ready = true; if (side_kick(h)) return -1; }
         if (h->ldi_side_todo && *ws == h->setup_seq) { if (ldi_side_kick(h)) return -1; }
+        if (h->early_armed && h->reduce_pending && *reinterpret_cast<volatile long long*>(h->h_early) == -h->early_seq) {
+            h->early_armed = false;
+            if (flush_reduce(h)) return -1;
+        }
         if (h->early_armed && *reinterpret_cast<volatile long long*>(h->h_early) == h->early_seq) {
             h->early_armed = false; h->spec_enqueued = true;
             if (h->prelm_pending) { h->prelm_pending = false; h->prelm_valid = true; }
@@ -948,6 +961,13 @@
             }
         }
     }
+    ReduceRide red_ride{};
+    if (h->reduce_pending) {
+        if (zero_by_list && !lm_here && h->npitems > 0) {
+            red_ride = h->red_ride; red_ride.lead = 8; red_ride.clear_status = h->status;
+            h->reduce_pending = false; ++h->reduce_ridden;
+        } else if (flush_reduce(h)) return -1;
+    }
     if (!zero_by_list) {
         HIP_OK(hipMemsetAsync(h->red, 0, h->red_count * sizeof(double) + ST_NWORDS * sizeof(int32_t), h->stream));
         ++h->lin_fills;
@@ -980,24 +1000,24 @@
         const int per_xcd = h->pose_xcd ? cdiv(h->npitems, 8) : 0;
         const int nblk = per_xcd ? 8 * per_xcd : h->npitems;
         static_assert(ST_NWORDS % 2 == 0, "the status words are cleared as doubles");
-        const int ntail = zero_by_list ? h->nr * 6 + 2 + (lm_here ? 0 : ST_NWORDS / 2) : 0;
+        const int ntail = zero_by_list ? h->nr * 6 + 2 + ((lm_here || red_ride.lead) ? 0 : ST_NWORDS / 2) : 0;
         const int nzs = zero_by_list ? h->nzero_slots : 0;
         const int nzblk = zero_by_list ? cdiv((long)nzs * 36 + ntail, 256) : 0;
-#define PS_PPF_LAUNCH(W, D) hipLaunchKernelGGL((k_pose_pass_pf<W, D>), dim3(nblk + nzblk), dim3(256), 0, h->stream, h->pitems, h->pobs,       \
+#define PS_PPF_LAUNCH(W, D) hipLaunchKernelGGL((k_pose_pass_pf<W, D>), dim3(red_ride.lead + nblk + nzblk), dim3(256), 0, h->stream, h->pitems, h->pobs, \
                                h->poses, h->points, h->ogroups, h->Cinv, h->cvec, h->ppartial, wp, h->npitems, per_xcd,                  \
-                               nblk, (const int32_t*)h->zero_slots, nzs, h->S, h->g, ntail)
+                               nblk, (const int32_t*)h->zero_slots, nzs, h->S, h->g, ntail, red_ride)
         if (h->pose_prefetch && h->pose_chunk <= PS_POSE_PF_OBS) {
             if (h->wide_obs) { if (lambda != 0.0) PS_PPF_LAUNCH(true, true); else PS_PPF_LAUNCH(true, false); }
             else if (lambda != 0.0) PS_PPF_LAUNCH(false, true); else PS_PPF_LAUNCH(false, false);
         }
         else if (h->wide_obs)
-            hipLaunchKernelGGL(k_pose_pass<true>, dim3(nblk + nzblk), dim3(256), 0, h->stream, h->pitems, h->pobs,
+            hipLaunchKernelGGL(k_pose_pass<true>, dim3(red_ride.lead + nblk + nzblk), dim3(256), 0, h->stream, h->pitems, h->pobs,
                                h->poses, h->points, h->ogroups, h->Cinv, h->cvec, h->ppartial, lambda != 0.0 ? 1 : 0, wp, h->npitems, per_xcd,
-                               nblk, (const int32_t*)h->zero_slots, nzs, h->S, h->g, ntail);
+                               nblk, (const int32_t*)h->zero_slots, nzs, h->S, h->g, ntail, red_ride);
         else
-            hipLaunchKernelGGL(k_pose_pass<false>, dim3(nblk + nzblk), dim3(256), 0, h->stream, h->pitems, h->pobs,
+            hipLaunchKernelGGL(k_pose_pass<false>, dim3(red_ride.lead + nblk + nzblk), dim3(256), 0, h->stream, h->pitems, h->pobs,
                                h->poses, h->points, h->ogroups, h->Cinv, h->cvec, h->ppartial, lambda != 0.0 ? 1 : 0, wp, h->npitems, per_xcd,
-                               nblk, (const int32_t*)h->zero_slots, nzs, h->S, h->g, ntail);
+                               nblk, (const int32_t*)h->zero_slots, nzs, h->S, h->g, ntail, red_ride);
 #undef PS_PPF_LAUNCH
         fin_in_combine = h->Spart && h->npair_items > 0 && !h->has_diag_tasks && h->D == 6;
         fin_in_pairs = !h->Spart && h->schur_pipeline && h->npair_items > 0 && !h->has_diag_tasks && h->D == 6 && !schur_split_env;
@@ -1213,6 +1233,7 @@
 }
 
 int gn_tail(ps_problem* h, int linesearch, const int32_t* gate, bool publish = false) {
+    if (flush_reduce(h)) return -1;
     h->params_moved_since_lin = true;
     h->prelin_valid = h->prelm_valid = h->ride_valid = false;
     h->prelm_pending = false;
@@ -1235,13 +1256,18 @@
     } else if (linesearch) { StageTimer t(h, PS_ST_COST); ncost = cost_partials_pass(h, 1, gate); }
     double* o_cost = h->shard_out ? h->shard_buf : h->scalars + (linesearch ? SC_COST : SC_LINCOST);
     double* o_dxl = h->shard_out ? h->shard_buf + 1 : h->scalars + SC_DXL2;
-    hipLaunchKernelGGL(k_reduce3, dim3(3), dim3(256), 0, h->stream,
-                       ncost, h->cost_partials, o_cost,
-                       h->nsq_p, h->sq_part_p, h->nr > 0 ? h->scalars + SC_DXP2 : nullptr,
-                       nsq_l_now(h), h->sq_part_l, (h->nv > 0 || h->shard_out) ? o_dxl : nullptr, gate,
-                       h->status, h->scalars, publish ? h->h_status_dev : nullptr, publish ? h->h_scalars_dev : nullptr,
-                       h->arrivals, publish ? h->h_seq_dev : nullptr, publish ? ++h->seq : 0LL);
-    return 0;
-}
-
-}
+    const ReduceRide rr{0, ncost, h->cost_partials, o_cost,
+                        h->nsq_p, h->sq_part_p, h->nr > 0 ? h->scalars + SC_DXP2 : nullptr,
+                        nsq_l_now(h), h->sq_part_l, (h->nv > 0 || h->shard_out) ? o_dxl : nullptr, gate,
+                        h->status, h->scalars, publish ? h->h_status_dev : nullptr, publish ? h->h_scalars_dev : nullptr,
+                        h->arrivals, publish ? h->h_seq_dev : nullptr, publish ? ++h->seq : 0LL, nullptr};
+    if (h->reduce_ride && publish && h->early_armed && lm_cost && h->npitems > 0 && !h->lm_md && !h->shard_out && h->lin_zero_gate) {
+        h->red_ride = rr; h->reduce_pending = true;
+    } else {
+        hipLaunchKernelGGL(k_reduce3, dim3(3), dim3(256), 0, h->stream, rr);
+        ++h->reduce_launched;
+    }
+    return 0;
+}
+
+}
diff --git a/pyslam_amd/csrc/ps_k_linearize.h b/pyslam_amd/csrc/ps_k_linearize.h
--- a/pyslam_amd/csrc/ps_k_linearize.h
+++ b/pyslam_amd/csrc/ps_k_linearize.h
@@ -11,6 +11,7 @@
 }
 
 #define PS_ZROW 16
+#define PS_ZST 14
 
 PS_DEV void lm_emit_m(const ReprojEval& ev, double M00, double M10, double M11, double M20, double M21,
                       double M22, double* __restrict__ m) {
@@ -160,6 +161,17 @@
     }
 }
 
+struct ReduceRide {
+    int lead;
+    int n0; const double* p0; double* o0;
+    int n1; const double* p1; double* o1;
+    int n2; const double* p2; double* o2;
+    const int32_t* gate; const int32_t* status; const double* scalars;
+    int32_t* hst; double* hsc; int32_t* arrivals; long long* hseq; long long seq;
+    int32_t* clear_status;
+};
+PS_DEV void reduce3_block(const ReduceRide& rr, int b, double* lds );
+
 PS_DEV void pose_sandwich(const double* __restrict__ e, const double* __restrict__ pc, double* __restrict__ acc) {
     const double x = pc[0], y = pc[1], z = pc[2];
     const double E[3][3] = {{e[0], e[1], e[2]}, {e[1], e[3], e[4]}, {e[2], e[4], e[5]}};
@@ -199,19 +211,25 @@
     const ObsGroup* __restrict__ groups, const double* __restrict__ Cinv,
     const double* __restrict__ cvec, double* __restrict__ partial, int want_diag ,
     ObsWide wide, int nitems, int per_xcd ,
-    int zero_first, const int32_t* __restrict__ zero_slots, int nzero_slots, double* __restrict__ S, double* __restrict__ ztail, int ntail)
+    int zero_first, const int32_t* __restrict__ zero_slots, int nzero_slots, double* __restrict__ S, double* __restrict__ ztail, int ntail,
+    ReduceRide rr)
 {
     __shared__ double red[4][PS_NPOSE_ACC];
 #if PS_POSE_TRANSPOSE
     __shared__ double tr[4][64 * 17];
 #endif
-    if ((int)blockIdx.x >= zero_first) {
-        const int e = ((int)blockIdx.x - zero_first) * 256 + (int)threadIdx.x, ns = 36 * nzero_slots;
+    int bid = (int)blockIdx.x;
+    if (rr.lead) {
+        if (bid < rr.lead) { if (bid < 3) reduce3_block(rr, bid, red[0]); return; }
+        bid -= rr.lead;
+    }
+    if (bid >= zero_first) {
+        const int e = (bid - zero_first) * 256 + (int)threadIdx.x, ns = 36 * nzero_slots;
         if (e < ns) { const int k = e / 36; S[(size_t)zero_slots[k] * 36 + (e - 36 * k)] = 0.0; }
         else if (e - ns < ntail) ztail[e - ns] = 0.0;
         return;
     }
-    const int item = per_xcd > 0 ? (int)(blockIdx.x & 7) * per_xcd + (int)(blockIdx.x >> 3) : (int)blockIdx.x;
+    const int item = per_xcd > 0 ? (bid & 7) * per_xcd + (bid >> 3) : bid;
     if (item >= nitems) return;
     const PItem it = items[item];
     const int w = threadIdx.x >> 6, lane = threadIdx.x & 63;
@@ -381,17 +399,23 @@
     const PItem* __restrict__ items, const LObs* __restrict__ pobs, const double* __restrict__ poses,
     const double* __restrict__ points, const ObsGroup* __restrict__ groups, const double* __restrict__ Cinv,
     const double* __restrict__ cvec, double* __restrict__ partial, ObsWide wide, int nitems, int per_xcd,
-    int zero_first, const int32_t* __restrict__ zero_slots, int nzero_slots, double* __restrict__ S, double* __restrict__ ztail, int ntail)
+    int zero_first, const int32_t* __restrict__ zero_slots, int nzero_slots, double* __restrict__ S, double* __restrict__ ztail, int ntail,
+    ReduceRide rr)
 {
     __shared__ double red[4][PS_NPOSE_ACC];
     __shared__ double tr[4][64 * 17];
-    if ((int)blockIdx.x >= zero_first) {
-        const int e = ((int)blockIdx.x - zero_first) * 256 + (int)threadIdx.x, ns = 36 * nzero_slots;
+    int bid = (int)blockIdx.x;
+    if (rr.lead) {
+        if (bid < rr.lead) { if (bid < 3) reduce3_block(rr, bid, red[0]); return; }
+        bid -= rr.lead;
+    }
+    if (bid >= zero_first) {
+        const int e = (bid - zero_first) * 256 + (int)threadIdx.x, ns = 36 * nzero_slots;
         if (e < ns) { const int k = e / 36; S[(size_t)zero_slots[k] * 36 + (e - 36 * k)] = 0.0; }
         else if (e - ns < ntail) ztail[e - ns] = 0.0;
         return;
     }
-    const int item = per_xcd > 0 ? (int)(blockIdx.x & 7) * per_xcd + (int)(blockIdx.x >> 3) : (int)blockIdx.x;
+    const int item = per_xcd > 0 ? (bid & 7) * per_xcd + (bid >> 3) : bid;
     if (item >= nitems) return;
     const PItem it = items[item];
     const int w = threadIdx.x >> 6, lane = threadIdx.x & 63;
diff --git a/pyslam_amd/csrc/ps_k_packed.h b/pyslam_amd/csrc/ps_k_packed.h
--- a/pyslam_amd/csrc/ps_k_packed.h
+++ b/pyslam_amd/csrc/ps_k_packed.h
@@ -69,7 +69,7 @@
 }
 
 template <bool WIDE, bool COST, bool PF>
-__global__ __launch_bounds__(256) __attribute__((amdgpu_waves_per_eu(PS_LM_WAVES, 8))) void k_landmark_pass_packed(
+__global__ __launch_bounds__(256) __attribute__((amdgpu_waves_per_eu(PF ? 5 : PS_LM_WAVES, 8))) void k_landmark_pass_packed(
     int nwaves, const int32_t* __restrict__ lmw_first, const LmwRun* __restrict__ lmw_run, const int32_t* __restrict__ lm_ptr,
     const int32_t* __restrict__ lm_point,
     const LObs* __restrict__ lobs, const double* __restrict__ poses,
@@ -80,7 +80,7 @@
     const int32_t* __restrict__ gate = nullptr, double* __restrict__ cost_part = nullptr,
     long long* __restrict__ fail_word = nullptr, long long fail_tag = 0)
 {
-    __shared__ __attribute__((aligned(16))) double zst[4][64 * PS_ZROW];
+    __shared__ __attribute__((aligned(16))) double zst[4][64 * PS_ZST];
     __shared__ int32_t flags[4][64];
     __shared__ double csum[16];
     const int lane = threadIdx.x & 63;
@@ -124,7 +124,7 @@
             }
             const int g0 = __builtin_amdgcn_readfirstlane(grp);
             const ObsGroup g = obs_group_fetch(groups, g0);
-            reproj_eval_obs_fetched<true, true, WIDE>(T, pw, &o.u, groups, grp, g0, g, Sl, ev);
+            reproj_eval_obs_fetched<true, true, WIDE, COST>(T, pw, &o.u, groups, grp, g0, g, Sl, ev);
         }
         sg = lmw_segment_of(v0, nlm, rn.row0, rn.nrows, start, lane, flags[wv]);
     } else {
@@ -227,14 +227,17 @@
             z[9] = ev.pc[0]; z[10] = ev.pc[1]; z[11] = ev.pc[2];
             z[12] = (double)rid_of_obs;
         }
-        double2* dst = reinterpret_cast<double2*>(sm + PS_ZROW * lane);
-#pragma unroll
-        for (int k = 0; k < PS_ZROW / 2; ++k) dst[k] = make_double2(z[2 * k], z[2 * k + 1]);
+        double2* dst = reinterpret_cast<double2*>(sm + PS_ZST * lane);
+#pragma unroll
+        for (int k = 0; k < PS_ZST / 2; ++k) dst[k] = make_double2(z[2 * k], z[2 * k + 1]);
     }
     __builtin_amdgcn_wave_barrier();
     const double2* src = reinterpret_cast<const double2*>(sm);
     double2* out = reinterpret_cast<double2*>(Z + PS_ZROW * (size_t)sg.row0);
-    for (int k = lane; k < sg.nrows * (PS_ZROW / 2); k += 64) out[k] = src[k];
+    for (int k = lane; k < sg.nrows * (PS_ZROW / 2); k += 64) {
+        const int j = k & (PS_ZROW / 2 - 1);
+        out[k] = j < PS_ZST / 2 ? src[(k >> 3) * (PS_ZST / 2) + j] : make_double2(0.0, 0.0);
+    }
     }
     if (COST) {
         obs_cost = block_sum(obs_cost, csum);
diff --git a/pyslam_amd/csrc/ps_k_tail.h b/pyslam_amd/csrc/ps_k_tail.h
--- a/pyslam_amd/csrc/ps_k_tail.h
+++ b/pyslam_amd/csrc/ps_k_tail.h
@@ -510,46 +510,47 @@
     return ((a[0] + a[1]) + (a[2] + a[3])) + ((a[4] + a[5]) + (a[6] + a[7]));
 }
 
-__global__ __launch_bounds__(256) void k_reduce3(
-    int n0, const double* __restrict__ p0, double* __restrict__ o0,
-    int n1, const double* __restrict__ p1, double* __restrict__ o1,
-    int n2, const double* __restrict__ p2, double* __restrict__ o2, const int32_t* __restrict__ gate,
-    const int32_t* __restrict__ status, const double* __restrict__ scalars,
-    int32_t* __restrict__ hst, double* __restrict__ hsc,
-    int32_t* __restrict__ arrivals , long long* __restrict__ hseq, long long seq)
-{
-    __shared__ double lds[16];
-    const bool open = !(gate && gate[ST_PCG_DONE] != 1);
-    if (hst && blockIdx.x == 0) {
+PS_DEV void reduce3_block(const ReduceRide& rr, int b, double* lds) {
+    const bool open = !(rr.gate && rr.gate[ST_PCG_DONE] != 1);
+    if (rr.hst && b == 0) {
         const int t = threadIdx.x;
-        if (t < ST_NWORDS) hst[t] = status[t];
+        if (t < ST_NWORDS) rr.hst[t] = rr.status[t];
         else if (t < ST_NWORDS + SC_NWORDS) {
             const int k = t - ST_NWORDS;
-            if (!open || (o0 != scalars + k && o1 != scalars + k && o2 != scalars + k)) hsc[k] = scalars[k];
-        }
-    }
-    const int n = blockIdx.x == 0 ? n0 : (blockIdx.x == 1 ? n1 : n2);
-    const double* p = blockIdx.x == 0 ? p0 : (blockIdx.x == 1 ? p1 : p2);
-    double* o = blockIdx.x == 0 ? o0 : (blockIdx.x == 1 ? o1 : o2);
+            if (!open || (rr.o0 != rr.scalars + k && rr.o1 != rr.scalars + k && rr.o2 != rr.scalars + k)) rr.hsc[k] = rr.scalars[k];
+        }
+    }
+    const int n = b == 0 ? rr.n0 : (b == 1 ? rr.n1 : rr.n2);
+    const double* p = b == 0 ? rr.p0 : (b == 1 ? rr.p1 : rr.p2);
+    double* o = b == 0 ? rr.o0 : (b == 1 ? rr.o1 : rr.o2);
     if (open && o) {
         double s = strided_sum8(p, n);
         s = block_sum(s, lds);
         if (threadIdx.x == 0) {
             o[0] = s;
-            if (hsc && o >= scalars && o < scalars + SC_NWORDS) hsc[o - scalars] = s;
-        }
-    }
-    if (hseq) {
+            if (rr.hsc && o >= rr.scalars && o < rr.scalars + SC_NWORDS) rr.hsc[o - rr.scalars] = s;
+        }
+    }
+    if (rr.hseq) {
         __syncthreads();
         if (threadIdx.x == 0) {
             __threadfence_system();
-            if (atomicAdd(arrivals, 1) == (int)gridDim.x - 1) {
-                *arrivals = 0;
+            if (atomicAdd(rr.arrivals, 1) == 2) {
+                *rr.arrivals = 0;
+                if (rr.clear_status) {
+                    for (int k = 0; k < ST_NWORDS; ++k) rr.clear_status[k] = 0;
+                }
                 __threadfence_system();
-                *reinterpret_cast<volatile long long*>(hseq) = seq;
+                *reinterpret_cast<volatile long long*>(rr.hseq) = rr.seq;
             }
         }
     }
+}
+
+__global__ __launch_bounds__(256) void k_reduce3(ReduceRide rr)
+{
+    __shared__ double lds[16];
+    reduce3_block(rr, blockIdx.x, lds);
 }
 
 __global__ __launch_bounds__(64) void k_publish(
diff --git a/pyslam_amd/csrc/ps_math.h b/pyslam_amd/csrc/ps_math.h
--- a/pyslam_amd/csrc/ps_math.h
+++ b/pyslam_amd/csrc/ps_math.h
@@ -286,7 +286,7 @@
     double pc[3];
 };
 
-template <bool WITH_JP, bool WITH_JL>
+template <bool WITH_JP, bool WITH_JL, bool RHO_APART = false>
 PS_DEV void reproj_eval_s(const Se3& T, const double* __restrict__ pw, const double* __restrict__ uvd,
                           const ObsGroup& g, const double* __restrict__ Sv, ReprojEval& o) {
     double pc[3], rr[3], iz;
@@ -304,7 +304,11 @@
         for (int i = 0; i < 3; ++i) rr[i] = __builtin_fma(Sv[3 * i + 2], e2, __builtin_fma(Sv[3 * i + 1], e1, Sv[3 * i] * e0));
         o.cost = 0.0;
 #pragma unroll
-        for (int i = 0; i < 3; ++i) o.cost += ps_loss_rho(g.loss_id, g.loss_k, rr[i]);
+        for (int i = 0; i < 3; ++i) {
+            double k = g.loss_k;
+            if (RHO_APART) asm("" : "+v"(k), "+v"(rr[i]));
+            o.cost += ps_loss_rho(g.loss_id, k, rr[i]);
+        }
     }
     o.pc[0] = pc[0]; o.pc[1] = pc[1]; o.pc[2] = pc[2];
     double s[3];
@@ -386,7 +390,7 @@
     return g;
 }
 
-template <bool WITH_JP, bool WITH_JL, bool WIDE>
+template <bool WITH_JP, bool WITH_JL, bool WIDE, bool RHO_APART = false>
 PS_DEV void reproj_eval_obs_fetched(const Se3& T, const double* __restrict__ pw, const double* __restrict__ uvd,
                                     const ObsGroup* __restrict__ groups, int grp, int gfirst_id, const ObsGroup& gfirst,
                                     const double* __restrict__ Sl, ReprojEval& o) {
@@ -395,7 +399,7 @@
         if (grp == g0) {
             ObsGroup g = gfirst;
             if (g0 != gfirst_id) g = groups[g0];
-            reproj_eval_s<WITH_JP, WITH_JL>(T, pw, uvd, g, WIDE ? Sl : g.S, o);
+            reproj_eval_s<WITH_JP, WITH_JL, RHO_APART>(T, pw, uvd, g, WIDE ? Sl : g.S, o);
             break;
         }
     }
diff --git a/pyslam_amd/device.py b/pyslam_amd/device.py
--- a/pyslam_amd/device.py
+++ b/pyslam_amd/device.py
@@ -392,6 +392,13 @@
         nat.check(self._lib.ps_debug_pose_items(self._h, C.byref(ni), n, items.ctypes.data_as(C.POINTER(C.c_int32)), nat.f64p(partial)))
         return items, partial
 
+    def z_rows(self):
+        n = C.c_int64(0)
+        nat.check(self._lib.ps_debug_z_rows(self._h, C.byref(n), 0, None))
+        z = np.zeros((n.value, 16))
+        nat.check(self._lib.ps_debug_z_rows(self._h, C.byref(n), n.value, nat.f64p(z)))
+        return z
+
     def debug_reproj_blocks(self):
         n = self.lp.num_obs
         r, jp, jl = np.zeros((n, 3)), np.zeros((n, 3, 6)), np.zeros((n, 3, 3))
```
